# JiaweiXu8/AD-GS

Measured on AMD Instinct MI355X. Metric: fwd+bwd frames/s, higher is better.
Workload: dtype f32; 1 GPU; C3: 1000000 Gaussians, 1920x1280, SH deg 3, 8 dynamic objects, flow+semantic outputs, 1 camera/GPU/step; P=1000000, camera_pool=16 cameras / time stamps per GPU, cycled one per step (train.py:55-61), settle_steps=75, capacity_reruns=0, launch=eager, parallelism=single GPU, gradient_exchange=none, camera_streams=1

## Files before the change

### ad-gs_amd/csrc/api.hip

```cpp
#include "common.h"
#include "kernels.h"
#include "../../include/adgs_rasterizer.h"
#include "../../include/adgs_optim.h"

#include <atomic>
#include <chrono>
#include <mutex>
#include <vector>
#include <cstdlib>
#include <algorithm>
#include <cmath>
#include <cstring>

namespace adgs {

static thread_local std::string g_last_error;
struct FrameContext {
	adgs_frame_stats stats;
	size_t hint_cells, hint_fine;
	unsigned hint_max_cell_chunks;
	bool bucket_frame_pending;
	long long reruns;
	int last_order_hint;
	uint32_t* slab_bounds;
// ... 106 lines not shown
		s.tile_scanned = c.take<uint32_t>(ntiles);
		s.tile_batches = c.take<uint32_t>(ntiles);
		if (bytes) *bytes = c.size();
		return s;
	}
};
struct BinStateV2 {
	uint32_t* pool_cursor; uint32_t* pool;
	uint64_t* keys_unsorted; uint64_t* keys; uint32_t* list_unsorted; uint32_t* list; char* sort_temp;
	uint32_t* rec_key; uint2* rec_im; uint2* entries; uint32_t* slow_list;
	static size_t slab_grid(size_t R_cells, size_t ncells) { return std::max<size_t>(2 * R_cells / SLAB_TARGET_FOREIGN + ncells + 1, ncells << forced_lg()); }
	static int forced_lg() { const char* v = getenv("ADGS_SLABS_LG"); return (v && *v) ? std::min(std::max(atoi(v), 0), (int)MAX_SLAB_LG) : 0; }
	static size_t pool_chunks(size_t R_fine, size_t ntiles) { return R_fine / WAVE + (2 * (size_t)POOL_BLOCK + 1) * ntiles + 1; }
	static BinStateV2 carve_buckets(char* chunk, size_t R_cells, size_t R_fine, size_t ntiles, size_t* bytes, size_t ncells = 0) {
		Carver c(chunk); BinStateV2 b;
		b.pool_cursor = c.take<uint32_t>(64);
		b.pool = c.take<uint32_t>(pool_chunks(R_fine, ntiles) * CHUNK_WORDS);
		b.entries = c.take<uint2>(R_cells + 1);
		b.rec_im = c.take<uint2>(R_cells);
		b.rec_key = c.take<uint32_t>(R_cells);
		b.slow_list = c.take<uint32_t>(1 + slab_grid(R_cells, ncells));
		b.keys = nullptr; b.keys_unsorted = nullptr; b.sort_temp = nullptr; b.list = nullptr; b.list_unsorted = nullptr;
		if (bytes) *bytes = c.size();
		return b;
	}
	static BinStateV2 carve(char* chunk, size_t R_cells, size_t R_fine, size_t ntiles, size_t* bytes) {
		Carver c(chunk); BinStateV2 b;
		b.pool_cursor = c.take<uint32_t>(64);
		b.pool = c.take<uint32_t>(pool_chunks(R_fine, ntiles) * CHUNK_WORDS);
		b.list = c.take<uint32_t>(R_cells);
		b.list_unsorted = c.take<uint32_t>(R_cells);
		b.keys = c.take<uint64_t>(R_cells);
		b.keys_unsorted = c.take<uint64_t>(R_cells);
		b.sort_temp = c.take<char>(sort_temp_bytes(R_cells));
		b.rec_key = nullptr; b.rec_im = nullptr; b.entries = nullptr; b.slow_list = nullptr;
		if (bytes) *bytes = c.size();
		return b;
	}
};

static std::atomic<unsigned long long> g_env_reads{0};
static const char* env_str(const char* name) { g_env_reads.fetch_add(1, std::memory_order_relaxed); return getenv(name); }
static int env_int(const char* name, int dflt) {
	const char* v = env_str(name);
	return (v && *v) ? atoi(v) : dflt;
}
static bool use_v2(int D_S, bool env = true) {
	if (!env) return D_S <= (int)MAX_SEMANTIC;
	const char* m = env_str("ADGS_RASTER_MODE");
	if (m && std::string(m) == "classic") return false;
	return D_S <= std::min(env_int("ADGS_V2_MAX_SEMANTIC", 32), (int)MAX_SEMANTIC);
}

static bool v2_keys_fit(int gx, int gy, int c) { return 2 * c + (int)higher_msb((uint32_t)(((gx + c - 1) / c) * ((gy + c - 1) / c))) <= 32; }
static int v2_cell_tiles(int gx, int gy, bool fit_keys, bool env = true) {
	const size_t ntiles16 = (size_t)gx * gy;
	const int small = std::min(8, std::max(3, (int)std::lround(std::sqrt((double)ntiles16 / 110.0))));
	const int dflt = ntiles16 >= 4096 ? 12 : small;
	int c = std::max(1, env ? env_int("ADGS_CELL_TILES", dflt) : dflt);
	while (fit_keys && c > 1 && !v2_keys_fit(gx, gy, c)) c--;
	return c;
}
static int v2_pixels_per_lane(size_t ntiles16, bool env = true) {
	const int e = env ? env_int("ADGS_V2_PPL", 0) : 0;
	if (e == 1 || e == 2 || e == 4) return e;
	return ntiles16 < 4096 ? 2 : 4;
}


static const char* const kStageNames[ST_COUNT] = { "preprocess_fwd", "scan", "duplicate_keys", "radix_sort", "tile_ranges",
	"render_fwd", "render_bwd", "preprocess_bwd", "deform_fwd", "deform_bwd", "grad_expand" };
struct ProfRec { int stage; hipEvent_t a, b; };
static std::atomic<unsigned> g_prof_mask{0};
static std::mutex g_prof_mu;
static std::vector<ProfRec> g_prof_recs;
static std::vector<hipEvent_t> g_prof_pool;
static hipEvent_t prof_event() {
	std::lock_guard<std::mutex> lk(g_prof_mu);
	if (!g_prof_pool.empty()) { hipEvent_t e = g_prof_pool.back(); g_prof_pool.pop_back(); return e; }
	hipEvent_t e = nullptr; (void)hipEventCreate(&e); return e;
}
StageTimer::StageTimer(int stage_, hipStream_t stream) : on((g_prof_mask.load(std::memory_order_relaxed) >> stage_) & 1u), stage(stage_), a(nullptr), b(nullptr), s(stream) {
	if (on) { a = prof_event(); b = prof_event(); (void)hipEventRecord(a, s); }
}
StageTimer::~StageTimer() {
	if (on) { (void)hipEventRecord(b, s); std::lock_guard<std::mutex> lk(g_prof_mu); g_prof_recs.push_back(ProfRec{ stage, a, b }); }
}

static uint32_t* pinned_word() {
	static thread_local uint32_t* p = nullptr;
	if (!p) { if (hipHostMalloc((void**)&p, 1024, hipHostMallocDefault) != hipSuccess) p = nullptr; }
	return p;
}

struct MailboxRef { Mailbox* host; Mailbox* dev; uint32_t next_seq; size_t cap_cells, cap_fine;
	long long repaired; };
static MailboxRef* mailbox() {
	constexpr int MAX_DEV = 64;
	static thread_local MailboxRef boxes[MAX_DEV] = {};
	int dev = 0;
	if (hipGetDevice(&dev) != hipSuccess || dev < 0 || dev >= MAX_DEV) return nullptr;
	MailboxRef& m = boxes[dev];
	if (!m.host) {
		void* h = nullptr; void* d = nullptr;
		if (hipHostMalloc(&h, 256, hipHostMallocMapped | hipHostMallocCoherent | hipHostMallocPortable) != hipSuccess) return nullptr;
		if (hipHostGetDevicePointer(&d, h, 0) != hipSuccess) { (void)hipHostFree(h); return nullptr; }
		memset(h, 0, 256);
		m.host = (Mailbox*)h; m.dev = (Mailbox*)d; m.next_seq = 1; m.cap_cells = m.cap_fine = 0;
	}
	return &m;
}
struct OrderHints {
	struct Entry { const void* view; const void* proj; int W, H; size_t tiles; hipStream_t stream; bool captured; uint32_t* buf; unsigned long long used; bool written; size_t extra; };
	std::vector<Entry> entries;
	unsigned long long clock = 0, lookups = 0, hits = 0;
	hipStream_t service = nullptr;
	static constexpr size_t MAX_ENTRIES = 1024;
	Entry* find(const void* view, const void* proj, int W, int H, size_t tiles, hipStream_t stream, bool captured) {
		for (Entry& e : entries)
			if (e.view == view && e.proj == proj && e.W == W && e.H == H && e.tiles == tiles && e.captured == captured && (captured || e.stream == stream)) { e.used = ++clock; return &e; }
		return nullptr;
	}
	bool reset_signature(uint32_t* buf, size_t tiles, size_t extra) {
		if (!service && hipStreamCreateWithFlags(&service, hipStreamNonBlocking) != hipSuccess) { service = nullptr; return false; }
		return hipMemsetAsync(buf + tiles, 0, 16 * sizeof(uint32_t), service) == hipSuccess &&
		       (extra == 0 || hipMemsetAsync(buf + tiles + 16, 0xff, extra * sizeof(uint32_t), service) == hipSuccess) && hipStreamSynchronize(service) == hipSuccess;
	}
	Entry* create(const void* view, const void* proj, int W, int H, size_t tiles, hipStream_t stream, bool captured, size_t extra) {
		Entry* e = nullptr;
		if (entries.size() >= MAX_ENTRIES) {
			if (captured) return nullptr;
			for (Entry& c : entries) if (!c.captured && (!e || c.used < e->used)) e = &c;
			if (!e) return nullptr;
			(void)hipStreamSynchronize(e->stream);
			if (e->tiles != tiles || e->extra != extra) { (void)hipFree(e->buf); e->buf = nullptr; e->tiles = 0; e->view = nullptr; if (hipMalloc((void**)&e->buf, (tiles + 16 + extra) * sizeof(uint32_t)) != hipSuccess) { e->buf = nullptr; return nullptr; } }
		} else {
			Entry fresh{ nullptr, nullptr, 0, 0, 0, nullptr, false, nullptr, 0, false, 0 };
			if (hipMalloc((void**)&fresh.buf, (tiles + 16 + extra) * sizeof(uint32_t)) != hipSuccess) return nullptr;
			entries.push_back(fresh);
			e = &entries.back();
		}
		e->view = view; e->proj = proj; e->W = W; e->H = H; e->tiles = tiles; e->stream = stream; e->captured = captured; e->used = ++clock; e->written = false; e->extra = extra;
		if (!reset_signature(e->buf, tiles, extra)) { e->view = nullptr; e->tiles = 0; (void)hipFree(e->buf); e->buf = nullptr; return nullptr; }
		return e;
	}
};
static OrderHints* order_hints() {
	constexpr int MAX_DEV = 64;
	static thread_local OrderHints hints[MAX_DEV];
	int dev = 0;
	if (hipGetDevice(&dev) != hipSuccess || dev < 0 || dev >= MAX_DEV) return nullptr;
	return &hints[dev];
}
struct FrameCfg { int v2; int cell_tiles; int ppl; int tile_order = 1; int sh_staging = 1; int timeline = 0; int order_ready = 0; int backwards = 0; int antialiasing = 0; int published = 0; };
static uint32_t frame_cfg_word(const FrameCfg& c) {
	return 0xAD600000u | ((uint32_t)(c.v2 & 1) << 19) | ((uint32_t)(c.tile_order & 1) << 18) | ((uint32_t)(c.sh_staging & 1) << 17) | ((uint32_t)(c.timeline & 1) << 16) |
	       ((uint32_t)(c.order_ready & 1) << 15) | ((uint32_t)(c.antialiasing & 1) << 14) | ((uint32_t)(c.published & 1) << 13) |
	       ((uint32_t)(c.ppl & 0x1f) << 8) | (uint32_t)(c.cell_tiles & 0xff);
}
static bool frame_cfg_from_word(uint32_t w, FrameCfg* c) {
	if ((w & 0xFFF00000u) != 0xAD600000u) return false;
	*c = FrameCfg{ (int)((w >> 19) & 1u), (int)(w & 0xffu), (int)((w >> 8) & 0x1fu) };
	c->tile_order = (int)((w >> 18) & 1u); c->sh_staging = (int)((w >> 17) & 1u); c->timeline = (int)((w >> 16) & 1u); c->order_ready = (int)((w >> 15) & 1u);
	c->antialiasing = (int)((w >> 14) & 1u); c->published = (int)((w >> 13) & 1u);
	return c->cell_tiles >= 1 && (c->ppl == 1 || c->ppl == 2 || c->ppl == 4);
}
struct FrameKey {
	const void* img; const void* geom; int W, H, P;
	bool operator==(const FrameKey& o) const { return img == o.img && geom == o.geom && W == o.W && H == o.H && P == o.P; }
};
static std::mutex g_cfg_mu;
static std::vector<std::pair<FrameKey, FrameCfg>> g_cfg_table;
static void remember_frame(const FrameKey& k, const FrameCfg& c) {
	std::lock_guard<std::mutex> lk(g_cfg_mu);
	for (auto it = g_cfg_table.begin(); it != g_cfg_table.end();) it = (it->first.img == k.img || it->first.geom == k.geom) ? g_cfg_table.erase(it) : it + 1;
	if (g_cfg_table.size() >= 256) g_cfg_table.erase(g_cfg_table.begin());
	g_cfg_table.emplace_back(k, c);
}
static int note_backward(const FrameKey& k) {
	std::lock_guard<std::mutex> lk(g_cfg_mu);
	for (auto it = g_cfg_table.rbegin(); it != g_cfg_table.rend(); ++it) if (it->first == k) return it->second.backwards++;
	return -1;
}
static bool lookup_frame(const FrameKey& k, FrameCfg* c) {
	std::lock_guard<std::mutex> lk(g_cfg_mu);
	for (auto it = g_cfg_table.rbegin(); it != g_cfg_table.rend(); ++it) if (it->first == k) { *c = it->second; return true; }
	return false;
}
static bool lookup_frame_by_image(const void* img, int W, int H, FrameCfg* c) {
	std::lock_guard<std::mutex> lk(g_cfg_mu);
	for (auto it = g_cfg_table.rbegin(); it != g_cfg_table.rend(); ++it)
		if (it->first.img == img && it->first.W == W && it->first.H == H) { *c = it->second; return true; }
	return false;
}
__global__ void publish_counts_kernel(const uint32_t* __restrict__ total_cells, const unsigned long long* __restrict__ fine_slots, Mailbox* box, uint32_t seq,
	uint32_t cap_cells, unsigned long long cap_fine, uint32_t* __restrict__ overflow_flag) {
	unsigned long long f = threadIdx.x < SCAN_AUX_SLOTS ? fine_slots[threadIdx.x] : 0ull;
#pragma unroll
	for (int off = WAVE / 2; off > 0; off >>= 1) f += __shfl_xor(f, off, WAVE);
	if (threadIdx.x == 0) {
		const uint32_t total = *total_cells;
		const uint32_t over = (total > cap_cells || f > cap_fine) ? 1u : 0u;
		*overflow_flag = over;
		box->r_cells = total; box->r_fine = f; box->oversize = 0u; box->n_groups = 0u; box->overflow = over; box->max_cell_chunks = 0u;
		if (over) box->overflow_count = box->overflow_count + 1u;
		box->cap_cells = cap_cells; box->cap_fine = cap_fine;
		__threadfence_system();
		box->seq = seq;
	}
}
static int wait_mailbox(const MailboxRef* m, uint32_t seq, hipStream_t stream) {
	const auto t0 = std::chrono::steady_clock::now();
	for (unsigned spin = 0;; spin++) {
		if (m->host->seq == seq) return 0;
		if ((spin & 0xFFFF) == 0xFFFF && std::chrono::steady_clock::now() - t0 > std::chrono::seconds(10)) break;
	}
	ADGS_HIP_CHECK(hipStreamSynchronize(stream));
	if (m->host->seq == seq) return 0;
	set_error("the device never published the binning counts"); return -1;
}

}

using namespace adgs;

extern "C" const char* adgs_last_error(void) { return g_last_error.c_str(); }

extern "C" void adgs_get_frame_stats(adgs_frame_stats* out) { if (out) *out = frame_context()->stats; }

extern "C" int adgs_get_frame_status(adgs_frame_status* out) {
	if (!out) return -1;
	memset(out, 0, sizeof(*out));
	MailboxRef* mb = mailbox();
	if (!mb) { set_error("hipHostMalloc (mapped) failed"); return -1; }
	out->pairs = (int64_t)mb->host->r_cells; out->fine_pairs = (int64_t)mb->host->r_fine;
	out->capacity_pairs = mb->host->cap_cells == 0xffffffffu ? (int64_t)mb->host->r_cells : (int64_t)mb->host->cap_cells;
	out->capacity_fine_pairs = mb->host->cap_fine == ~0ull ? (int64_t)mb->host->r_fine : (int64_t)mb->host->cap_fine;
	out->overflow = (int32_t)mb->host->overflow; out->overflow_count = (int64_t)mb->host->overflow_count;
	out->eager_reruns = (int64_t)frame_context()->reruns;
	out->order_hint = frame_context()->last_order_hint;
	out->fullest_slab_units = (int64_t)mb->host->max_cell_chunks;
	if (OrderHints* oh = order_hints()) { out->order_hint_lookups = (int64_t)oh->lookups; out->order_hint_hits = (int64_t)oh->hits; }
	out->unrepaired_overflow_count = (int64_t)mb->host->overflow_count - (int64_t)mb->repaired;
	return 0;
}

extern "C" int adgs_raster_needs_zero_init(int D_S) { return use_v2(D_S) ? 0 : 1; }
extern "C" int adgs_raster_backward_needs_zero_init(const char* geom_buffer, const char* img_buffer, int width, int height, int P) {
	FrameCfg cfg;
	if (!lookup_frame(FrameKey{ img_buffer, geom_buffer, width, height, P }, &cfg)) return 1;
	return cfg.v2 ? 0 : 1;
}

extern "C" void adgs_profile_enable(int stage_mask) { g_prof_mask.store((unsigned)stage_mask); }
extern "C" int adgs_profile_reserve(int n_events) {
	std::vector<hipEvent_t> fresh;
	for (int i = 0; i < n_events; i++) { hipEvent_t e = nullptr; if (hipEventCreate(&e) != hipSuccess) break; fresh.push_back(e); }
	std::lock_guard<std::mutex> lk(g_prof_mu);
	g_prof_pool.insert(g_prof_pool.end(), fresh.begin(), fresh.end());
	return (int)fresh.size();
}
extern "C" int adgs_profile_num_stages(void) { return ST_COUNT; }
extern "C" const char* adgs_profile_stage_name(int i) { return (i >= 0 && i < ST_COUNT) ? kStageNames[i] : ""; }
extern "C" int adgs_profile_collect(double* total_ms, int64_t* counts) {
	std::lock_guard<std::mutex> lk(g_prof_mu);
	for (auto& r : g_prof_recs) {
		float ms = 0.f;
		if (hipEventElapsedTime(&ms, r.a, r.b) == hipSuccess) { total_ms[r.stage] += ms; counts[r.stage] += 1; }
		g_prof_pool.push_back(r.a); g_prof_pool.push_back(r.b);
	}
	g_prof_recs.clear();
	return 0;
}

extern "C" int adgs_device_check(void) {
	int n = 0;
	if (hipGetDeviceCount(&n) != hipSuccess || n == 0) { set_error("no HIP device"); return -1; }
	hipDeviceProp_t prop;
	int dev = 0;
	ADGS_HIP_CHECK(hipGetDevice(&dev));
	ADGS_HIP_CHECK(hipGetDeviceProperties(&prop, dev));
	if (std::string(prop.gcnArchName).find("gfx950") == std::string::npos) {
		set_error(std::string("device is ") + prop.gcnArchName + ", this library is built for gfx950 only");
		return -2;
	}
	return 0;
}

static int raster_forward_impl(const ShSource* sh_src, bool training, int antialiasing,
	adgs_alloc_fn geometryBuffer, void* geometryUser,
	adgs_alloc_fn binningBuffer, void* binningUser,
	adgs_alloc_fn imageBuffer, void* imageUser,
	int P, int D, int M, int D_S,
	const float* background, int width, int height,
	const float* means3D, const float* shs, const float* colors_precomp, const float* flow_points, const float* semantic,
	const float* opacities, const float* scales, float scale_modifier, const float* rotations, const float* cov3D_precomp,
	const float* viewmatrix, const float* projmatrix, const float* cam_pos, float tan_fovx, float tan_fovy, int prefiltered,
	float* out_color, float* out_depth, float* img_opacity, float* img_flow, float* img_semantic,
	int inv_depth, int* radii, int debug, void* stream_) {
	(void)prefiltered;
	hipStream_t stream = (hipStream_t)stream_;
	FrameContext* fc = frame_context();
	if (P <= 0) return 0;
	if (D_S > MAX_SEMANTIC) { set_error("D_S exceeds 32 semantic channels"); return -1; }
	if (!means3D || !opacities || (!cov3D_precomp && (!scales || !rotations)) || !radii) { set_error("missing required input pointer"); return -1; }
	const int gx = (width + TILE_X - 1) / TILE_X, gy = (height + TILE_Y - 1) / TILE_Y;
	const size_t ntiles = (size_t)gx * gy, npix = (size_t)width * height;
	if (gx > 65535 || gy > 65535) { set_error("image too large"); return -1; }
	if (ntiles * 4 * (2 * (size_t)POOL_BLOCK + 1) > 0xffffffffull) { set_error("image too large: chunk slots are 32-bit"); return -1; }

	if (D_S > 1) training = true;
	if (use_v2(D_S)) {
		int cell_tiles = v2_cell_tiles(gx, gy, false);
		int cgx = (gx + cell_tiles - 1) / cell_tiles, cgy = (gy + cell_tiles - 1) / cell_tiles;
		size_t ncells = (size_t)cgx * cgy;
		const char* binning_env = env_str("ADGS_BINNING");
		const std::string binning_mode = binning_env ? binning_env : "";
		{
			const MailboxRef* mbp = mailbox();
			const unsigned old_m = fc->hint_max_cell_chunks;
			const unsigned seen = (mbp && fc->bucket_frame_pending) ? mbp->host->max_cell_chunks : 0u;
			fc->hint_max_cell_chunks = std::max(seen, old_m - std::max(1u, old_m / 16) * (old_m ? 1u : 0u));
			fc->bucket_frame_pending = false;
		}
		bool buckets = ncells <= (size_t)MAX_CELLS && cell_tiles <= 16 && binning_mode != "sort" &&
			(binning_mode == "bucket" || (fc->hint_cells <= (size_t)std::max(1, env_int("ADGS_BUCKET_MAX_CHUNKS", 4)) * GS_NMAX * (ncells << MAX_SLAB_LG) &&
			                              fc->hint_max_cell_chunks <= (unsigned)std::max(1, env_int("ADGS_BUCKET_MAX_CELL_CHUNKS", 16))));
		if (!buckets && !v2_keys_fit(gx, gy, cell_tiles)) {
			cell_tiles = v2_cell_tiles(gx, gy, true);
			cgx = (gx + cell_tiles - 1) / cell_tiles; cgy = (gy + cell_tiles - 1) / cell_tiles; ncells = (size_t)cgx * cgy;
		}
		const bool sort_fallback_fits = v2_keys_fit(gx, gy, cell_tiles);
		size_t gb = 0, ib = 0;
		const size_t count_cells = buckets ? ncells : 0;
		const bool with_ddir = training && sh_src && M == 16;
		GeomStateV2::carve(nullptr, P, &gb, with_ddir, count_cells);
		char* gch = geometryBuffer(geometryUser, gb);
		const int ppl = v2_pixels_per_lane(ntiles), sub = TILE_Y / (4 * ppl);
		const int wgy = (height + 4 * ppl - 1) / (4 * ppl);
		const size_t wtiles = (size_t)gx * wgy;
		ImgStateV2::carve(nullptr, npix, wtiles, ncells, &ib);
		char* ich = imageBuffer(imageUser, ib);
		if (!gch || !ich) { set_error("buffer allocator returned NULL"); return -1; }
		GeomStateV2 geom = GeomStateV2::carve(gch, P, nullptr, with_ddir, count_cells);
		ImgStateV2 img = ImgStateV2::carve(ich, npix, wtiles, ncells, nullptr);
		uint32_t frame_word = 0; bool order_tiles = false;
		{
			FrameCfg fcfg{ 1, cell_tiles, ppl };
			fcfg.antialiasing = antialiasing ? 1 : 0;
			fcfg.tile_order = env_int("ADGS_TILE_ORDER", 1) != 0; fcfg.sh_staging = env_str("ADGS_NO_SH_STAGING") == nullptr; fcfg.timeline = env_int("ADGS_TIMELINE_BWD", 0) != 0;
			order_tiles = wtiles >= 2048 && fcfg.tile_order;
			if (!training) order_tiles = false;
			fcfg.order_ready = order_tiles ? 1 : 0;
			fcfg.published = (training && env_int("ADGS_PUBLISHED_MASK", 1) != 0) ? 1 : 0;
			if (training) remember_frame(FrameKey{ ich, gch, width, height, P }, fcfg);
			frame_word = frame_cfg_word(fcfg);
		}
		const int fwd_order_mode = env_int("ADGS_FWD_ORDER", 2);
		OrderHints::Entry* hint = nullptr;
		const uint32_t* hint_read = nullptr;
		const bool fwd_hint_wanted = wtiles >= 2048 && env_int("ADGS_TILE_ORDER", 1) != 0 && fwd_order_mode == 2;
		if (fwd_hint_wanted) {
			hipStreamCaptureStatus cs0 = hipStreamCaptureStatusNone;
			(void)hipStreamIsCapturing(stream, &cs0);
			if (OrderHints* oh = order_hints()) {
				const bool cap0 = cs0 == hipStreamCaptureStatusActive;
				hint = oh->find(viewmatrix, projmatrix, width, height, wtiles, stream, cap0);
				if (!hint && training) {
					hipStreamCaptureMode mode = hipStreamCaptureModeRelaxed;
					if (cap0) (void)hipThreadExchangeStreamCaptureMode(&mode);
					hint = oh->create(viewmatrix, projmatrix, width, height, wtiles, stream, cap0, std::min<size_t>(ncells, (size_t)MAX_CELLS) * SLAB_ROW);
					if (cap0) (void)hipThreadExchangeStreamCaptureMode(&mode);
					(void)hipGetLastError();
				}
				oh->lookups++;
				if (hint && hint->buf) { hint_read = hint->buf; if (hint->written) oh->hits++; fc->last_order_hint = hint->written ? 1 : 0; } else { hint = nullptr; fc->last_order_hint = 0; }
			}
		}

		PreprocessArgs pa;
		pa.P = P; pa.D = D; pa.M = M; pa.D_S = D_S;
		pa.means3D = means3D; pa.scales = scales; pa.scale_modifier = scale_modifier; pa.rotations = rotations;
		pa.opacities = opacities; pa.shs = shs; pa.cov3D_precomp = cov3D_precomp; pa.colors_precomp = colors_precomp;
		pa.flow_points = flow_points; pa.semantic = semantic;
		pa.view = viewmatrix; pa.proj = projmatrix; pa.campos = cam_pos;
		pa.W = width; pa.H = height; pa.gx = gx; pa.gy = gy;
		pa.tan_fovx = tan_fovx; pa.tan_fovy = tan_fovy;
		pa.focal_y = height / (2.0f * tan_fovy); pa.focal_x = width / (2.0f * tan_fovx);
		pa.inv_depth = inv_depth;
		pa.radii = radii; pa.splats = geom.splats; pa.cov3D = nullptr; pa.clamped = geom.clamped; pa.tiles_touched = geom.cells_touched;
		pa.v2 = 1; pa.dupinfo = geom.dupinfo; pa.fine_touched = geom.fine_touched; pa.cell_tiles = cell_tiles; pa.cgx = cgx; pa.cgy = cgy;
		memset(&pa.sh_src, 0, sizeof(pa.sh_src));
		pa.sh0 = geom.sh0; pa.gacc = training ? geom.gacc : nullptr; pa.fine_total = geom.fine_total;
		pa.bucket_count = nullptr;
		pa.cfg_word = img.header; pa.cfg_value = frame_word;
		pa.ddir = geom.ddir;
		pa.published = training ? geom.published : nullptr;
		pa.antialias = antialiasing ? 1 : 0;
		FramePrologue pro{ nullptr, 0, nullptr, nullptr, 0 };
		bool own_bounds = false, sample_bounds = false;
		if (buckets) {
			if (!fc->slab_bounds) {
				hipStreamCaptureStatus csb = hipStreamCaptureStatusNone;
				(void)hipStreamIsCapturing(stream, &csb);
				hipStreamCaptureMode mode = hipStreamCaptureModeRelaxed;
				if (csb == hipStreamCaptureStatusActive) (void)hipThreadExchangeStreamCaptureMode(&mode);
				bool ok = hipMalloc((void**)&fc->slab_bounds, (size_t)MAX_CELLS * SLAB_ROW * sizeof(uint32_t)) == hipSuccess;
				ok = ok && (fc->service || hipStreamCreateWithFlags(&fc->service, hipStreamNonBlocking) == hipSuccess);
				ok = ok && hipMemsetAsync(fc->slab_bounds, 0xff, (size_t)MAX_CELLS * SLAB_ROW * sizeof(uint32_t), fc->service) == hipSuccess && hipStreamSynchronize(fc->service) == hipSuccess;
				if (csb == hipStreamCaptureStatusActive) (void)hipThreadExchangeStreamCaptureMode(&mode);
				if (!ok) { if (fc->slab_bounds) (void)hipFree(fc->slab_bounds); fc->slab_bounds = nullptr; (void)hipGetLastError(); }
			}
			pro.zero = reinterpret_cast<uint32_t*>(geom.bucket_fine_total()); pro.n_zero = 2 * SCAN_AUX_SLOTS + 8;
			if (fc->slab_bounds) {
				const bool own = training && hint && (hint->written || hint->captured) && hint->extra >= ncells * SLAB_ROW;
				own_bounds = own;
				sample_bounds = !own && fwd_hint_wanted && env_int("ADGS_SLAB_SAMPLE", 1) != 0;
				pro.copy_dst = geom.bounds; pro.copy_src = own ? hint->buf + wtiles + 16 : fc->slab_bounds; pro.n_copy = (int)(ncells * SLAB_ROW);
			}
			if (!sh_src && launch_bin_prepare(pro, stream) != 0) return -1;
			pa.bucket_count = geom.counts; pa.fine_total = geom.bucket_fine_total();
		}
		if (sh_src) { pa.sh_src = *sh_src; StageTimer t(ST_PREPROCESS, stream); if (launch_sh0(P, *sh_src, geom.sh0, stream, buckets ? &pro : nullptr) != 0) return -1; }
		if (const int evict_mb = env_int("ADGS_DBG_EVICT_MB", 0)) {
			static thread_local void* scratch = nullptr; static thread_local size_t scratch_bytes = 0;
			const size_t want = (size_t)evict_mb << 20;
			if (scratch_bytes < want) { if (scratch) (void)hipFree(scratch); scratch = nullptr; scratch_bytes = 0; if (hipMalloc(&scratch, want) == hipSuccess) scratch_bytes = want; }
			if (scratch) ADGS_HIP_CHECK(hipMemsetAsync(scratch, 0, want, stream));
		}
		{ StageTimer t(ST_PREPROCESS, stream); if (launch_preprocess_fwd(pa, stream) != 0) return -1; }
		ADGS_LAUNCH_CHECK(debug, stream);
		MailboxRef* mb = mailbox();
		if (!mb) { set_error("hipHostMalloc (mapped) failed"); return -1; }
		const uint32_t seq = mb->next_seq++;
		hipStreamCaptureStatus cap_status = hipStreamCaptureStatusNone;
		(void)hipStreamIsCapturing(stream, &cap_status);
		const bool capturing = cap_status == hipStreamCaptureStatusActive;
		const bool speculate = capturing || env_int("ADGS_NO_SPECULATION", 0) == 0;
		const size_t cap_cells = std::min<size_t>(std::max<size_t>(fc->hint_cells, (size_t)P + 4096), 0x7fffffffu);
		const size_t cap_fine = std::max<size_t>(fc->hint_fine, (size_t)8 * P + 4096);
		mb->cap_cells = cap_cells; mb->cap_fine = cap_fine;
		uint32_t* overflow_flag = geom.d_counts() + 3;
		CellScanArgs sa;
		sa.cell_count = geom.cell_count(); sa.cell_start = geom.cell_start; sa.cell_ranges = img.cell_ranges; sa.ncells = (int)ncells;
		sa.max_chunks = (uint32_t)std::min(MAX_CHUNKS, std::max(1, env_int("ADGS_MAX_CHUNKS", MAX_CHUNKS))); sa.d_counts = geom.d_counts();
		sa.fine_total = geom.bucket_fine_total(); sa.cell_work = geom.cell_work; sa.force_lg = buckets ? env_int("ADGS_SLABS_LG", -1) : -1;
		sa.slab_target = own_bounds ? (uint32_t)SLAB_TARGET : (uint32_t)SLAB_TARGET_FOREIGN;
		sa.cap_cells = speculate ? (uint32_t)cap_cells : 0xffffffffu; sa.cap_fine = speculate ? (unsigned long long)cap_fine : ~0ull;
		sa.box = mb->dev; sa.seq = seq;
		if (buckets) {
			StageTimer t(ST_SCAN, stream);
			if (launch_cell_colscan(geom.counts, (P + 255) / 256, (int)ncells, geom.cell_count(), stream) != 0) return -1;
			if (launch_cell_scan(sa, stream) != 0) return -1;
		} else {
			{
				StageTimer t(ST_SCAN, stream);
				if (exclusive_scan_u32_sum(geom.cells_touched, geom.offsets, (size_t)P + 1, geom.scan_temp, geom.fine_touched, geom.fine_total, stream) != 0) return -1;
			}
			hipLaunchKernelGGL(publish_counts_kernel, dim3(1), dim3(WAVE), 0, stream, (const uint32_t*)(geom.offsets + P), (const unsigned long long*)geom.fine_total, mb->dev, seq,
				speculate ? (uint32_t)cap_cells : 0xffffffffu, speculate ? (unsigned long long)cap_fine : ~0ull, overflow_flag);
			ADGS_HIP_CHECK(hipGetLastError());
		}
		ADGS_LAUNCH_CHECK(debug, stream);
		const int bit = (int)higher_msb((uint32_t)ncells);
		BinStateV2 bin;
		const int mask_shift = 32 + bit;
		auto enqueue_binning = [&](size_t cells, size_t fine, const uint32_t* d_count) -> int {
			size_t bb = 0;
			if (buckets) {
				BinStateV2::carve_buckets(nullptr, cells, training ? fine * sub : 0, training ? wtiles : 0, &bb, ncells);
				char* bch = binningBuffer(binningUser, bb);
				if (!bch) { set_error("binning allocator returned NULL"); return -1; }
				bin = BinStateV2::carve_buckets(bch, cells, training ? fine * sub : 0, training ? wtiles : 0, nullptr, ncells);
				if (cells == 0) { ADGS_HIP_CHECK(hipMemsetAsync(bin.pool_cursor, 0, sizeof(uint32_t), stream)); return 0; }
				const uint32_t cap = (uint32_t)std::min<size_t>(cells, 0xffffffffu);
				{ StageTimer t(ST_DUPLICATE, stream);
				  if (launch_cell_scatter(P, geom.dupinfo, geom.cell_start, geom.counts, bin.rec_key, bin.rec_im, cap, cell_tiles, cgx, (int)ncells, bin.pool_cursor, bin.slow_list, stream) != 0) return -1; }
				ADGS_LAUNCH_CHECK(debug, stream);
				SlabSortArgs ga;
				ga.cell_ranges = img.cell_ranges; ga.ncells = (int)ncells; ga.cell_work = geom.cell_work; ga.grid = (uint32_t)BinStateV2::slab_grid(cells, ncells); ga.rec_key = bin.rec_key; ga.rec_im = bin.rec_im; ga.ent_f = bin.entries; ga.cap = cap;
				ga.bounds = geom.bounds; ga.bounds_out = fc->slab_bounds; ga.d_counts = geom.d_counts(); ga.slow_list = bin.slow_list;
				ga.bounds_out2 = (training && hint && hint->extra >= ncells * SLAB_ROW) ? hint->buf + wtiles + 16 : nullptr;
				ga.box = mb->dev;
				{ StageTimer t(ST_SORT, stream);
				  if (sample_bounds && launch_cell_sample(ga, geom.bounds, stream) != 0) return -1;
				  if (launch_slab_sort(ga, stream) != 0) return -1; }
				ADGS_LAUNCH_CHECK(debug, stream);
				return 0;
			}
			BinStateV2::carve(nullptr, cells, training ? fine * sub : 0, training ? wtiles : 0, &bb);
			char* bch = binningBuffer(binningUser, bb);
			if (!bch) { set_error("binning allocator returned NULL"); return -1; }
			bin = BinStateV2::carve(bch, cells, training ? fine * sub : 0, training ? wtiles : 0, nullptr);
			if (cells == 0) {
				ADGS_HIP_CHECK(hipMemsetAsync(img.cell_ranges, 0, ncells * sizeof(uint2), stream));
				ADGS_HIP_CHECK(hipMemsetAsync(bin.pool_cursor, 0, sizeof(uint32_t), stream));
				return 0;
			}
			{ StageTimer t(ST_DUPLICATE, stream);
			  if (launch_duplicate_cells(P, geom.dupinfo, geom.offsets, bin.keys_unsorted, bin.list_unsorted, (uint32_t)std::min<size_t>(cells, 0xffffffffu),
			        cell_tiles, cgx, img.cell_ranges, (int)ncells, bin.pool_cursor, mask_shift, stream) != 0) return -1; }
			ADGS_LAUNCH_CHECK(debug, stream);
			{ StageTimer t(ST_SORT, stream);
			  if (radix_sort_pairs_u64_dn(bin.keys_unsorted, bin.keys, bin.list_unsorted, bin.list, cells, d_count, 32 + bit, bin.sort_temp, stream) != 0) return -1; }
			ADGS_LAUNCH_CHECK(debug, stream);
			{ StageTimer t(ST_RANGES, stream);
			  if (launch_tile_ranges((int)cells, d_count, bin.keys, img.cell_ranges, bit >= 32 ? 0xffffffffu : ((1u << bit) - 1u), stream) != 0) return -1;
// ... 73 lines not shown
		fc->stats.num_rendered = (int64_t)R_cells; fc->stats.tiles = (int32_t)ntiles; fc->stats.sort_bits = buckets ? 32 : 32 + bit;
		fc->stats.sort_passes = buckets ? 4 : (32 + bit + 7) / 8;
		fc->stats.reserved = buckets ? 1 : 0; fc->stats.fine_pairs = (int64_t)R_fine;
		return (int)R_cells;
	}

	size_t gbytes = 0, ibytes = 0;
	GeomState::carve(nullptr, P, &gbytes);
	char* gchunk = geometryBuffer(geometryUser, gbytes);
	ImgState::carve(nullptr, npix, ntiles, &ibytes);
	char* ichunk = imageBuffer(imageUser, ibytes);
	if (!gchunk || !ichunk) { set_error("buffer allocator returned NULL"); return -1; }
	GeomState geom = GeomState::carve(gchunk, P, nullptr);
	ImgState img = ImgState::carve(ichunk, npix, ntiles, nullptr);
	uint32_t frame_word = 0;
	{
		FrameCfg fcfg{ 0, 1, 4 };
		fcfg.antialiasing = antialiasing ? 1 : 0;
		fcfg.sh_staging = env_str("ADGS_NO_SH_STAGING") == nullptr;
		remember_frame(FrameKey{ ichunk, gchunk, width, height, P }, fcfg);
		frame_word = frame_cfg_word(fcfg);
	}

	PreprocessArgs pa;
	pa.P = P; pa.D = D; pa.M = M; pa.D_S = D_S;
	pa.means3D = means3D; pa.scales = scales; pa.scale_modifier = scale_modifier; pa.rotations = rotations;
	pa.opacities = opacities; pa.shs = shs; pa.cov3D_precomp = cov3D_precomp; pa.colors_precomp = colors_precomp;
	pa.flow_points = flow_points; pa.semantic = semantic;
	pa.view = viewmatrix; pa.proj = projmatrix; pa.campos = cam_pos;
	pa.W = width; pa.H = height; pa.gx = gx; pa.gy = gy;
	pa.tan_fovx = tan_fovx; pa.tan_fovy = tan_fovy;
	pa.focal_y = height / (2.0f * tan_fovy);
	pa.focal_x = width / (2.0f * tan_fovx);
	pa.inv_depth = inv_depth;
	pa.radii = radii; pa.splats = geom.splats; pa.cov3D = geom.cov3D; pa.clamped = geom.clamped; pa.tiles_touched = geom.tiles_touched;
	pa.v2 = 0; pa.dupinfo = nullptr; pa.fine_touched = nullptr; pa.cell_tiles = 1; pa.cgx = gx; pa.cgy = gy;
	memset(&pa.sh_src, 0, sizeof(pa.sh_src)); pa.sh0 = nullptr; pa.gacc = nullptr; pa.fine_total = nullptr;
	pa.bucket_count = nullptr;
	pa.cfg_word = img.header; pa.cfg_value = frame_word; pa.ddir = nullptr; pa.published = nullptr;
	pa.antialias = antialiasing ? 1 : 0;
	if (sh_src) { set_error("the raw-SH entry points need the default (v2) pipeline (not ADGS_RASTER_MODE=classic, D_S <= ADGS_V2_MAX_SEMANTIC)"); return -1; }
	{ StageTimer t(ST_PREPROCESS, stream); if (launch_preprocess_fwd(pa, stream) != 0) return -1; }
	ADGS_LAUNCH_CHECK(debug, stream);

	{
		StageTimer t(ST_SCAN, stream);
		if (exclusive_scan_u32(geom.tiles_touched, geom.offsets, (size_t)P + 1, geom.scan_temp, stream) != 0) return -1;
	}
	ADGS_LAUNCH_CHECK(debug, stream);

	uint32_t* host_word = pinned_word();
	if (!host_word) { set_error("hipHostMalloc failed"); return -1; }
	ADGS_HIP_CHECK(hipMemcpyAsync(host_word, geom.offsets + P, sizeof(uint32_t), hipMemcpyDeviceToHost, stream));
	ADGS_HIP_CHECK(hipStreamSynchronize(stream));
	const int num_rendered = (int)*host_word;

	size_t bbytes = 0;
	BinState::carve(nullptr, (size_t)num_rendered, &bbytes);
	char* bchunk = binningBuffer(binningUser, bbytes);
	if (!bchunk) { set_error("binning allocator returned NULL"); return -1; }
	BinState bin = BinState::carve(bchunk, (size_t)num_rendered, nullptr);

	{ StageTimer t(ST_DUPLICATE, stream);
	  if (launch_duplicate_keys(P, geom.splats, geom.offsets, radii, bin.keys_unsorted, bin.list_unsorted, gx, gy, stream) != 0) return -1; }
	ADGS_LAUNCH_CHECK(debug, stream);
	const int bit = (int)higher_msb((uint32_t)ntiles);
	{ StageTimer t(ST_SORT, stream);
	  if (radix_sort_pairs_u64(bin.keys_unsorted, bin.keys, bin.list_unsorted, bin.list, (size_t)num_rendered, 32 + bit, bin.sort_temp, stream) != 0) return -1; }
	ADGS_LAUNCH_CHECK(debug, stream);
	{ StageTimer t(ST_RANGES, stream);
	  ADGS_HIP_CHECK(hipMemsetAsync(img.ranges, 0, ntiles * sizeof(uint2), stream));
	  if (launch_tile_ranges(num_rendered, nullptr, bin.keys, img.ranges, 0xffffffffu, stream) != 0) return -1; }
	ADGS_LAUNCH_CHECK(debug, stream);

	RenderFwdArgs ra;
	ra.ranges = img.ranges; ra.point_list = bin.list; ra.splats = geom.splats;
	ra.W = width; ra.H = height; ra.gx = gx; ra.gy = gy; ra.D_S = D_S;
	ra.has_color = (colors_precomp != nullptr) || (shs != nullptr);
	ra.has_flow = flow_points != nullptr; ra.has_sem = (semantic != nullptr) && D_S > 0; ra.inv_depth = inv_depth != 0;
	ra.semantic = semantic; ra.bg = background;
	ra.final_T = img_opacity; ra.n_contrib = img.n_contrib;
	ra.out_color = out_color; ra.out_depth = out_depth; ra.out_flow = img_flow; ra.out_semantic = img_semantic;
	{ StageTimer t(ST_RENDER_FWD, stream); if (launch_render_fwd(ra, stream) != 0) return -1; }
	ADGS_LAUNCH_CHECK(debug, stream);

	fc->stats.num_rendered = num_rendered; fc->stats.tiles = (int32_t)ntiles; fc->stats.sort_bits = 32 + bit; fc->stats.sort_passes = (32 + bit + 7) / 8;
	fc->stats.fine_pairs = num_rendered;
	return num_rendered;
}

static int raster_backward_impl(const ShSource* sh_src, const ShGradDst* sh_dst,
	int P, int D, int M, int R, int D_S,
	const float* background, int width, int height,
	const float* means3D, const float* shs, const float* colors_precomp, const float* flow_points, const float* semantic,
	const float* scales, float scale_modifier, const float* rotations, const float* cov3D_precomp,
	const float* viewmatrix, const float* projmatrix, const float* campos, float tan_fovx, float tan_fovy,
	const int* radii, char* geom_buffer, char* binning_buffer, char* img_buffer,
	const float* dL_dpix, const float* dL_dpix_depth, const float* dL_dpix_flow, const float* dL_dpix_semantic,
	float* dL_dmean2D, float* dL_dconic, float* dL_dopacity, float* dL_dcolor, float* dL_ddepth, float* dL_dmean3D,
	float* dL_dcov3D, float* dL_dsh, float* dL_dscale, float* dL_drot, float* dL_dflow, float* dL_dsemantic,
	const float* grad_img_opacity, const float* img_opacity, int inv_depth, int debug, void* stream_, float* dL_dmean2D_abs = nullptr) {
	hipStream_t stream = (hipStream_t)stream_;
	if (P <= 0) return 0;
	if (!geom_buffer || !img_buffer || (R > 0 && !binning_buffer)) { set_error("backward called without forward state buffers"); return -1; }
	if (dL_dmean2D_abs && dL_dpix_semantic && semantic && D_S > 1) {
		set_error("backward: dL_dmean2D_abs cannot be computed with D_S > 1 semantic channels and a semantic gradient (the extra channels are separate replays: "
		          "their per-pass absolute sums are not the absolute of the pair's term)");
		return -1;
	}
	const int gx = (width + TILE_X - 1) / TILE_X, gy = (height + TILE_Y - 1) / TILE_Y;
	const size_t ntiles = (size_t)gx * gy, npix = (size_t)width * height;
	FrameCfg cfg;
	const FrameKey fkey{ img_buffer, geom_buffer, width, height, P };
	if (!lookup_frame(fkey, &cfg)) {
		hipStreamCaptureStatus cs = hipStreamCaptureStatusNone;
		(void)hipStreamIsCapturing(stream, &cs);
		if (cs == hipStreamCaptureStatusActive) { set_error("backward over state buffers the captured forward did not allocate: their configuration cannot be read back inside a stream capture"); return -1; }
		uint32_t word = 0;
		ADGS_HIP_CHECK(hipMemcpyAsync(&word, img_buffer, sizeof(word), hipMemcpyDeviceToHost, stream));
		ADGS_HIP_CHECK(hipStreamSynchronize(stream));
		if (!frame_cfg_from_word(word, &cfg)) { set_error("backward: the image state buffer does not carry a forward's configuration word (not written by adgs_raster_forward?)"); return -1; }
	}
	if (dL_dmean2D_abs && !cfg.v2) {
		set_error("backward: dL_dmean2D_abs needs a forward of the default (v2) pipeline; this frame's forward ran the classic pipeline "
		          "(ADGS_RASTER_MODE=classic, or D_S above ADGS_V2_MAX_SEMANTIC), which does not form the absolute sums");
		return -1;
	}
	if (cfg.v2) {
		const int cell_tiles = cfg.cell_tiles;
		const size_t ncells = (size_t)((gx + cell_tiles - 1) / cell_tiles) * ((gy + cell_tiles - 1) / cell_tiles);
		GeomStateV2 geom = GeomStateV2::carve(geom_buffer, P, nullptr, sh_src && M == 16);
		const int ppl = cfg.ppl;
		const int wgy = (height + 4 * ppl - 1) / (4 * ppl);
		const size_t wtiles = (size_t)gx * wgy;
		ImgStateV2 img = ImgStateV2::carve(img_buffer, npix, wtiles, ncells, nullptr);
		BinStateV2 bin = BinStateV2::carve(binning_buffer, 0, 0, wtiles, nullptr);
		const bool has_color = (colors_precomp != nullptr) || (shs != nullptr) || (sh_src != nullptr);
		RenderV2BwdArgs ra;
		ra.splats = geom.splats; ra.pool = bin.pool; ra.tile_last_chunk = img.tile_last_chunk; ra.tile_consumed = img.tile_consumed;
		ra.W = width; ra.H = height; ra.gx = gx; ra.gy = wgy; ra.ppl = ppl;
		ra.bg = background; ra.final_T = img_opacity; ra.n_contrib = img.n_contrib;
		ra.bg_image = sh_src ? sh_src->bg_image : nullptr; ra.dL_dbg_image = (sh_src && sh_dst && ra.bg_image && dL_dpix) ? sh_dst->bg_image : nullptr;
		ra.dL_dpix = dL_dpix; ra.dL_dpix_depth = dL_dpix_depth; ra.dL_dpix_flow = dL_dpix_flow; ra.dL_dpix_sem = dL_dpix_semantic;
		ra.dL_dpix_opacity = grad_img_opacity;
		ra.do_color = dL_dpix && has_color;
		ra.do_flow = dL_dpix_flow && flow_points;
		ra.do_sem = dL_dpix_semantic && semantic && D_S > 0;
		ra.do_depth = dL_dpix_depth != nullptr;
		ra.do_opacity = grad_img_opacity != nullptr || (ra.bg_image != nullptr && ra.do_color);
		ra.absgrad = dL_dmean2D_abs != nullptr;
		ra.gacc = geom.gacc;
		ra.tile_order = nullptr;
		ra.tl_start = cfg.timeline ? img.tile_scanned : nullptr; ra.tl_end = img.tile_batches;
		{
			StageTimer t(ST_RENDER_BWD, stream);
			if (wtiles >= 2048 && cfg.tile_order) {
				if (!cfg.order_ready && launch_tile_order((int)wtiles, img.tile_consumed, img.tile_order, stream) != 0) return -1;
				ra.tile_order = img.tile_order;
			}
			if (note_backward(fkey) != 0) ADGS_HIP_CHECK(hipMemsetAsync(geom.gacc, 0, (size_t)P * GACC_STRIDE * sizeof(float), stream));
			ra.sem_src = nullptr; ra.sem_dst = nullptr; ra.sem_stride = 0;
			if (binning_buffer && launch_render_bwd_v2(ra, stream) != 0) return -1;
			if (binning_buffer && ra.do_sem && D_S > 1) {
				ADGS_HIP_CHECK(hipMemsetAsync(dL_dsemantic, 0, (size_t)P * D_S * sizeof(float), stream));
				RenderV2BwdArgs rc = ra;
				rc.do_color = rc.do_flow = rc.do_depth = rc.do_opacity = false; rc.do_sem = true; rc.absgrad = false;
				rc.dL_dpix = nullptr; rc.dL_dpix_depth = nullptr; rc.dL_dpix_flow = nullptr; rc.dL_dpix_opacity = nullptr;
				rc.bg_image = nullptr; rc.dL_dbg_image = nullptr; rc.sem_stride = D_S;
				for (int c = 1; c < D_S; c++) {
					rc.dL_dpix_sem = dL_dpix_semantic + (size_t)c * npix; rc.sem_src = semantic + c; rc.sem_dst = dL_dsemantic + c;
					if (launch_render_bwd_v2(rc, stream) != 0) return -1;
				}
			}
		}
		ADGS_LAUNCH_CHECK(debug, stream);
		PreprocessBwdArgs pa;
		pa.P = P; pa.D = D; pa.M = M;
		pa.means3D = means3D; pa.radii = radii; pa.shs = shs; pa.clamped = geom.clamped;
		pa.scales = scales; pa.rotations = rotations; pa.scale_modifier = scale_modifier;
		pa.cov3D = cov3D_precomp;
		pa.view = viewmatrix; pa.proj = projmatrix; pa.campos = campos;
		pa.focal_y = height / (2.0f * tan_fovy); pa.focal_x = width / (2.0f * tan_fovx);
		pa.tan_fovx = tan_fovx; pa.tan_fovy = tan_fovy; pa.inv_depth = inv_depth;
		pa.dL_dmean2D = nullptr; pa.dL_dconic = nullptr; pa.dL_dcolor = nullptr; pa.dL_ddepth = nullptr;
		pa.dL_dmean3D = dL_dmean3D; pa.dL_dcov3D = dL_dcov3D; pa.dL_dsh = dL_dsh; pa.dL_dscale = dL_dscale; pa.dL_drot = dL_drot;
		pa.gacc = geom.gacc; pa.splats = geom.splats; pa.W = width; pa.H = height;
		memset(&pa.sh_src, 0, sizeof(pa.sh_src)); pa.sh_dst = ShGradDst{};
		if (sh_src) { pa.sh_src = *sh_src; if (sh_dst) pa.sh_dst = *sh_dst; }
		pa.out_mean2D = dL_dmean2D; pa.out_conic = dL_dconic; pa.out_opacity = dL_dopacity; pa.out_color = dL_dcolor; pa.out_depth = dL_ddepth;
		pa.out_flow = ra.do_flow ? dL_dflow : nullptr; pa.out_sem = ra.do_sem ? dL_dsemantic : nullptr; pa.D_S = D_S;
		pa.out_mean2D_abs = dL_dmean2D_abs;
		pa.sh_staging = cfg.sh_staging;
		pa.ddir = geom.ddir;
		pa.antialias = cfg.antialiasing;
		pa.published = cfg.published ? geom.published : nullptr;
		{ StageTimer t(ST_PREPROCESS_BWD, stream); if (launch_preprocess_bwd(pa, stream) != 0) return -1; }
		ADGS_LAUNCH_CHECK(debug, stream);
		return 0;
	}
	GeomState geom = GeomState::carve(geom_buffer, P, nullptr);
	ImgState img = ImgState::carve(img_buffer, npix, ntiles, nullptr);
	BinState bin = BinState::carve(binning_buffer, (size_t)R, nullptr);

	const bool has_color = (colors_precomp != nullptr) || (shs != nullptr);
	RenderBwdArgs ra;
	ra.ranges = img.ranges; ra.point_list = bin.list; ra.splats = geom.splats;
	ra.W = width; ra.H = height; ra.gx = gx; ra.gy = gy; ra.D_S = D_S;
	ra.semantic = semantic; ra.bg = background;
	ra.final_T = img_opacity; ra.n_contrib = img.n_contrib;
	ra.dL_dpix = dL_dpix; ra.dL_dpix_depth = dL_dpix_depth; ra.dL_dpix_flow = dL_dpix_flow; ra.dL_dpix_sem = dL_dpix_semantic;
	ra.dL_dpix_opacity = grad_img_opacity;
	ra.do_color = dL_dpix && has_color;
	ra.do_flow = dL_dpix_flow && flow_points;
	ra.do_sem = dL_dpix_semantic && semantic && D_S > 0;
	ra.do_depth = dL_dpix_depth != nullptr;
	ra.do_opacity = grad_img_opacity != nullptr;
	ra.dL_dmean2D = dL_dmean2D; ra.dL_dconic = dL_dconic; ra.dL_dopacity = dL_dopacity; ra.dL_dcolor = dL_dcolor;
	ra.dL_ddepth = dL_ddepth; ra.dL_dflow = dL_dflow; ra.dL_dsem = dL_dsemantic;
	if (R > 0) {
		{ StageTimer t(ST_RENDER_BWD, stream); if (launch_render_bwd(ra, stream) != 0) return -1; }
		ADGS_LAUNCH_CHECK(debug, stream);
	}

	PreprocessBwdArgs pa;
	pa.P = P; pa.D = D; pa.M = M;
	pa.means3D = means3D; pa.radii = radii; pa.shs = shs; pa.clamped = geom.clamped;
	pa.scales = scales; pa.rotations = rotations; pa.scale_modifier = scale_modifier;
	pa.cov3D = cov3D_precomp ? cov3D_precomp : geom.cov3D;
	pa.view = viewmatrix; pa.proj = projmatrix; pa.campos = campos;
	pa.focal_y = height / (2.0f * tan_fovy); pa.focal_x = width / (2.0f * tan_fovx);
	pa.tan_fovx = tan_fovx; pa.tan_fovy = tan_fovy; pa.inv_depth = inv_depth;
	pa.dL_dmean2D = dL_dmean2D; pa.dL_dconic = dL_dconic; pa.dL_dcolor = dL_dcolor; pa.dL_ddepth = dL_ddepth;
	pa.dL_dmean3D = dL_dmean3D; pa.dL_dcov3D = dL_dcov3D; pa.dL_dsh = dL_dsh; pa.dL_dscale = dL_dscale; pa.dL_drot = dL_drot;
	if (sh_src) { set_error("the raw-SH entry points need the default (v2) pipeline (not ADGS_RASTER_MODE=classic, D_S <= ADGS_V2_MAX_SEMANTIC)"); return -1; }
	memset(&pa.sh_src, 0, sizeof(pa.sh_src)); pa.sh_dst = ShGradDst{};
	pa.gacc = nullptr; pa.splats = nullptr; pa.W = width; pa.H = height; pa.out_mean2D = nullptr; pa.out_conic = nullptr; pa.out_opacity = nullptr; pa.out_color = nullptr; pa.out_depth = nullptr;
	pa.out_flow = nullptr; pa.out_sem = nullptr; pa.D_S = D_S; pa.out_mean2D_abs = nullptr;
	pa.sh_staging = cfg.sh_staging; pa.ddir = nullptr; pa.published = nullptr;
	pa.antialias = cfg.antialiasing;
	if (cfg.antialiasing) { pa.out_opacity = dL_dopacity; pa.splats = geom.splats; }
	{ StageTimer t(ST_PREPROCESS_BWD, stream); if (launch_preprocess_bwd(pa, stream) != 0) return -1; }
	ADGS_LAUNCH_CHECK(debug, stream);
	return 0;
}

static int read_raster_options(const adgs_raster_options* o, const char* who, int* antialiasing) {
	*antialiasing = 0;
	if (!o) return 0;
	if (o->struct_bytes < offsetof(adgs_raster_options, antialiasing) + sizeof(int32_t) || o->struct_bytes > 4096) {
		set_error(std::string(who) + ": adgs_raster_options.struct_bytes must be sizeof(adgs_raster_options) of the caller's header"); return -1;
	}
	adgs_raster_options full;
	memset(&full, 0, sizeof(full));
	memcpy(&full, o, std::min<size_t>((size_t)o->struct_bytes, sizeof(full)));
	if (full.antialiasing != 0 && full.antialiasing != 1) { set_error(std::string(who) + ": adgs_raster_options.antialiasing must be 0 or 1"); return -1; }
	*antialiasing = full.antialiasing;
	return 0;
}

extern "C" int adgs_raster_forward_opts(
	adgs_alloc_fn geometryBuffer, void* geometryUser, adgs_alloc_fn binningBuffer, void* binningUser, adgs_alloc_fn imageBuffer, void* imageUser,
	int P, int D, int M, int D_S, const float* background, int width, int height,
	const float* means3D, const float* shs, const float* colors_precomp, const float* flow_points, const float* semantic,
	const float* opacities, const float* scales, float scale_modifier, const float* rotations, const float* cov3D_precomp,
	const float* viewmatrix, const float* projmatrix, const float* cam_pos, float tan_fovx, float tan_fovy, int prefiltered,
	float* out_color, float* out_depth, float* img_opacity, float* img_flow, float* img_semantic,
	int inv_depth, int* radii, int debug, void* stream, const adgs_raster_options* options) {
	int aa = 0;
	if (read_raster_options(options, "adgs_raster_forward_opts", &aa) != 0) return -1;
	return raster_forward_impl(nullptr, true, aa, geometryBuffer, geometryUser, binningBuffer, binningUser, imageBuffer, imageUser, P, D, M, D_S, background,
		width, height, means3D, shs, colors_precomp, flow_points, semantic, opacities, scales, scale_modifier, rotations, cov3D_precomp,
		viewmatrix, projmatrix, cam_pos, tan_fovx, tan_fovy, prefiltered, out_color, out_depth, img_opacity, img_flow, img_semantic,
		inv_depth, radii, debug, stream);
}

extern "C" int adgs_raster_forward(
	adgs_alloc_fn geometryBuffer, void* geometryUser, adgs_alloc_fn binningBuffer, void* binningUser, adgs_alloc_fn imageBuffer, void* imageUser,
	int P, int D, int M, int D_S, const float* background, int width, int height,
	const float* means3D, const float* shs, const float* colors_precomp, const float* flow_points, const float* semantic,
	const float* opacities, const float* scales, float scale_modifier, const float* rotations, const float* cov3D_precomp,
	const float* viewmatrix, const float* projmatrix, const float* cam_pos, float tan_fovx, float tan_fovy, int prefiltered,
	float* out_color, float* out_depth, float* img_opacity, float* img_flow, float* img_semantic,
	int inv_depth, int* radii, int debug, void* stream) {
	return adgs_raster_forward_opts(geometryBuffer, geometryUser, binningBuffer, binningUser, imageBuffer, imageUser, P, D, M, D_S, background, width, height, means3D, shs, colors_precomp, flow_points, semantic, opacities, scales, scale_modifier, rotations, cov3D_precomp, viewmatrix, projmatrix, cam_pos, tan_fovx, tan_fovy, prefiltered, out_color, out_depth, img_opacity, img_flow, img_semantic, inv_depth, radii, debug, stream, nullptr);
}

extern "C" int adgs_raster_render_opts(
	adgs_alloc_fn geometryBuffer, void* geometryUser, adgs_alloc_fn binningBuffer, void* binningUser, adgs_alloc_fn imageBuffer, void* imageUser,
	int P, int D, int M, int D_S, const float* background, int width, int height,
	const float* means3D, const float* shs, const float* colors_precomp, const float* flow_points, const float* semantic,
	const float* opacities, const float* scales, float scale_modifier, const float* rotations, const float* cov3D_precomp,
	const float* viewmatrix, const float* projmatrix, const float* cam_pos, float tan_fovx, float tan_fovy, int prefiltered,
	float* out_color, float* out_depth, float* img_opacity, float* img_flow, float* img_semantic,
	int inv_depth, int* radii, int debug, void* stream, const adgs_raster_options* options) {
	int aa = 0;
	if (read_raster_options(options, "adgs_raster_render_opts", &aa) != 0) return -1;
	return raster_forward_impl(nullptr, false, aa, geometryBuffer, geometryUser, binningBuffer, binningUser, imageBuffer, imageUser, P, D, M, D_S, background,
		width, height, means3D, shs, colors_precomp, flow_points, semantic, opacities, scales, scale_modifier, rotations, cov3D_precomp,
		viewmatrix, projmatrix, cam_pos, tan_fovx, tan_fovy, prefiltered, out_color, out_depth, img_opacity, img_flow, img_semantic,
		inv_depth, radii, debug, stream);
}

extern "C" int adgs_raster_render(
	adgs_alloc_fn geometryBuffer, void* geometryUser, adgs_alloc_fn binningBuffer, void* binningUser, adgs_alloc_fn imageBuffer, void* imageUser,
	int P, int D, int M, int D_S, const float* background, int width, int height,
	const float* means3D, const float* shs, const float* colors_precomp, const float* flow_points, const float* semantic,
	const float* opacities, const float* scales, float scale_modifier, const float* rotations, const float* cov3D_precomp,
	const float* viewmatrix, const float* projmatrix, const float* cam_pos, float tan_fovx, float tan_fovy, int prefiltered,
	float* out_color, float* out_depth, float* img_opacity, float* img_flow, float* img_semantic,
	int inv_depth, int* radii, int debug, void* stream) {
	return adgs_raster_render_opts(geometryBuffer, geometryUser, binningBuffer, binningUser, imageBuffer, imageUser, P, D, M, D_S, background, width, height, means3D, shs, colors_precomp, flow_points, semantic, opacities, scales, scale_modifier, rotations, cov3D_precomp, viewmatrix, projmatrix, cam_pos, tan_fovx, tan_fovy, prefiltered, out_color, out_depth, img_opacity, img_flow, img_semantic, inv_depth, radii, debug, stream, nullptr);
}

static int read_backward_options(const adgs_raster_backward_options* o, const char* who, float** dL_dmean2D_abs) {
	*dL_dmean2D_abs = nullptr;
	if (!o) return 0;
	if (o->struct_bytes < offsetof(adgs_raster_backward_options, dL_dmean2D_abs) + sizeof(float*) || o->struct_bytes > 4096) {
		set_error(std::string(who) + ": adgs_raster_backward_options.struct_bytes must be sizeof(adgs_raster_backward_options) of the caller's header"); return -1;
	}
	adgs_raster_backward_options full;
	memset(&full, 0, sizeof(full));
	memcpy(&full, o, std::min<size_t>((size_t)o->struct_bytes, sizeof(full)));
	*dL_dmean2D_abs = full.dL_dmean2D_abs;
	return 0;
}

extern "C" int adgs_raster_backward_opts(
	int P, int D, int M, int R, int D_S, const float* background, int width, int height,
	const float* means3D, const float* shs, const float* colors_precomp, const float* flow_points, const float* semantic,
	const float* scales, float scale_modifier, const float* rotations, const float* cov3D_precomp,
	const float* viewmatrix, const float* projmatrix, const float* campos, float tan_fovx, float tan_fovy,
	const int* radii, char* geom_buffer, char* binning_buffer, char* img_buffer,
	const float* dL_dpix, const float* dL_dpix_depth, const float* dL_dpix_flow, const float* dL_dpix_semantic,
	float* dL_dmean2D, float* dL_dconic, float* dL_dopacity, float* dL_dcolor, float* dL_ddepth, float* dL_dmean3D,
	float* dL_dcov3D, float* dL_dsh, float* dL_dscale, float* dL_drot, float* dL_dflow, float* dL_dsemantic,
	const float* grad_img_opacity, const float* img_opacity, int inv_depth, int debug, void* stream, const adgs_raster_backward_options* options) {
	float* abs_dst = nullptr;
	if (read_backward_options(options, "adgs_raster_backward_opts", &abs_dst) != 0) return -1;
	return raster_backward_impl(nullptr, nullptr, P, D, M, R, D_S, background, width, height, means3D, shs, colors_precomp, flow_points, semantic,
		scales, scale_modifier, rotations, cov3D_precomp, viewmatrix, projmatrix, campos, tan_fovx, tan_fovy, radii, geom_buffer, binning_buffer,
		img_buffer, dL_dpix, dL_dpix_depth, dL_dpix_flow, dL_dpix_semantic, dL_dmean2D, dL_dconic, dL_dopacity, dL_dcolor, dL_ddepth, dL_dmean3D,
		dL_dcov3D, dL_dsh, dL_dscale, dL_drot, dL_dflow, dL_dsemantic, grad_img_opacity, img_opacity, inv_depth, debug, stream, abs_dst);
}

extern "C" int adgs_raster_backward(
	int P, int D, int M, int R, int D_S, const float* background, int width, int height,
	const float* means3D, const float* shs, const float* colors_precomp, const float* flow_points, const float* semantic,
	const float* scales, float scale_modifier, const float* rotations, const float* cov3D_precomp,
	const float* viewmatrix, const float* projmatrix, const float* campos, float tan_fovx, float tan_fovy,
	const int* radii, char* geom_buffer, char* binning_buffer, char* img_buffer,
	const float* dL_dpix, const float* dL_dpix_depth, const float* dL_dpix_flow, const float* dL_dpix_semantic,
	float* dL_dmean2D, float* dL_dconic, float* dL_dopacity, float* dL_dcolor, float* dL_ddepth, float* dL_dmean3D,
	float* dL_dcov3D, float* dL_dsh, float* dL_dscale, float* dL_drot, float* dL_dflow, float* dL_dsemantic,
	const float* grad_img_opacity, const float* img_opacity, int inv_depth, int debug, void* stream) {
	return adgs_raster_backward_opts(P, D, M, R, D_S, background, width, height, means3D, shs, colors_precomp, flow_points, semantic,
		scales, scale_modifier, rotations, cov3D_precomp, viewmatrix, projmatrix, campos, tan_fovx, tan_fovy, radii, geom_buffer, binning_buffer,
		img_buffer, dL_dpix, dL_dpix_depth, dL_dpix_flow, dL_dpix_semantic, dL_dmean2D, dL_dconic, dL_dopacity, dL_dcolor, dL_ddepth, dL_dmean3D,
		dL_dcov3D, dL_dsh, dL_dscale, dL_drot, dL_dflow, dL_dsemantic, grad_img_opacity, img_opacity, inv_depth, debug, stream, nullptr);
}

static ShSource to_sh_source(const adgs_sh_source* s) {
	ShSource r;
	r.Ns = s->Ns; r.scene_dc = s->scene_dc; r.obj_dc = s->obj_dc; r.scene_rest = s->scene_rest; r.obj_rest = s->obj_rest;
	r.scene_sp = s->scene_deform; r.obj_sp = s->obj_deform; r.f = s->f;
	const bool raw_geo = s->Ns > 0 && s->scene_xyz && s->scene_scaling && s->scene_rotation && s->scene_opacity;
	r.scene_xyz = raw_geo ? s->scene_xyz : nullptr; r.scene_scaling = raw_geo ? s->scene_scaling : nullptr;
	r.scene_rotation = raw_geo ? s->scene_rotation : nullptr; r.scene_opacity = raw_geo ? s->scene_opacity : nullptr;
	r.bg_image = s->bg_image;
	if (!r.scene_dc) { r.scene_dc = r.obj_dc; r.scene_rest = r.obj_rest; }
	if (!r.obj_dc) { r.obj_dc = r.scene_dc; r.obj_rest = r.scene_rest; }
	return r;
}
static int check_sh_source(const adgs_sh_source* sh, int P, int M, const char* who) {
	const bool need_scene = sh && sh->Ns > 0, need_obj = sh && sh->Ns < P;
	if (sh && (sh->scene_xyz || sh->scene_scaling || sh->scene_rotation || sh->scene_opacity) &&
	    !(sh->scene_xyz && sh->scene_scaling && sh->scene_rotation && sh->scene_opacity)) {
		set_error(std::string(who) + ": raw scene geometry needs all four tensors"); return -1;
	}
	if (!sh || sh->Ns < 0 || sh->Ns > P || (need_scene && (!sh->scene_dc || (M > 1 && !sh->scene_rest))) || (need_obj && (!sh->obj_dc || (M > 1 && !sh->obj_rest)))) {
		set_error(std::string(who) + ": incomplete SH source"); return -1;
	}
	return 0;
}

extern "C" int adgs_raster_forward_rawsh_opts(
	adgs_alloc_fn geometryBuffer, void* geometryUser, adgs_alloc_fn binningBuffer, void* binningUser, adgs_alloc_fn imageBuffer, void* imageUser,
	int P, int D, int M, int D_S, const float* background, int width, int height,
	const float* means3D, const adgs_sh_source* sh, const float* flow_points, const float* semantic,
	const float* opacities, const float* scales, float scale_modifier, const float* rotations,
	const float* viewmatrix, const float* projmatrix, const float* cam_pos, float tan_fovx, float tan_fovy,
	float* out_color, float* out_depth, float* img_opacity, float* img_flow, float* img_semantic,
// ... 279 lines not shown
```

### ad-gs_amd/csrc/deform_sh.hip

```cpp
#include "common.h"
#include "kernels.h"
#include <cstring>

namespace adgs {
namespace {

struct ShsFwdArgs {
	int Ns, N, M;
	const float *scene_dc, *obj_dc, *scene_rest, *obj_rest, *sp_scene, *sp_obj;
	adgs_func_eval fs;
	float* out;
};
__global__ void __launch_bounds__(256) deform_shs_fwd_kernel(ShsFwdArgs a) {
	const size_t i = (size_t)blockIdx.x * blockDim.x + threadIdx.x;
	const int row = a.M * 3;
	const size_t total = (size_t)a.N * row;
	const size_t e0 = i * 4;
	if (e0 >= total) return;
	float v[4];
#pragma unroll
	for (int k = 0; k < 4; k++) {
		const size_t e = e0 + k;
		if (e >= total) { v[k] = 0.f; continue; }
		const int n = (int)(e / row), c = (int)(e % row);
		const bool is_obj = n >= a.Ns;
		const int m = is_obj ? n - a.Ns : n;
		if (c < 3) {
			float x = (is_obj ? a.obj_dc : a.scene_dc)[3 * (size_t)m + c];
			const float* sp = is_obj ? a.sp_obj : a.sp_scene;
			if (sp && has_lin(a.fs)) x = x + lin_eval(sp + ((size_t)m * 3 + c) * a.fs.n_params, a.fs);
			v[k] = x;
		} else {
			v[k] = (is_obj ? a.obj_rest : a.scene_rest)[(size_t)m * (row - 3) + (c - 3)];
		}
	}
	if (e0 + 4 <= total && (row & 3) == 0) *reinterpret_cast<float4*>(a.out + e0) = make_float4(v[0], v[1], v[2], v[3]);
	else { for (int k = 0; k < 4; k++) if (e0 + k < total) a.out[e0 + k] = v[k]; }
}

__global__ void __launch_bounds__(256) shs_rest_interleave_kernel(int Ns, int N, const float* __restrict__ scene_rest, const float* __restrict__ obj_rest, float* __restrict__ out) {
	const size_t i = (size_t)blockIdx.x * blockDim.x + threadIdx.x;
	if (i >= (size_t)N * 12) return;
	const int n = (int)(i / 12), q = (int)(i - (size_t)n * 12);
	const bool is_obj = n >= Ns;
	const float* r = (is_obj ? obj_rest : scene_rest) + (size_t)(is_obj ? n - Ns : n) * 45;
	float* o = out + (size_t)n * 48 + 4 * q;
	if (q == 0) { o[3] = r[0]; return; }
	const float a = r[4 * q - 3], b = r[4 * q - 2], c = r[4 * q - 1], d = r[4 * q];
	*reinterpret_cast<float4*>(o) = make_float4(a, b, c, d);
}
__global__ void __launch_bounds__(256) shs_grad_split_kernel(int Ns, int N, const float* __restrict__ g, float* __restrict__ g_scene_dc, float* __restrict__ g_obj_dc,
	float* __restrict__ g_scene_rest, float* __restrict__ g_obj_rest) {
	const size_t i = (size_t)blockIdx.x * blockDim.x + threadIdx.x;
	if (i >= (size_t)N * 12) return;
	const int n = (int)(i / 12), q = (int)(i - (size_t)n * 12);
	const bool is_obj = n >= Ns;
	const size_t m = is_obj ? n - Ns : n;
	const float4 v = *reinterpret_cast<const float4*>(g + (size_t)n * 48 + 4 * q);
	float* rest = is_obj ? g_obj_rest : g_scene_rest;
	if (q == 0) {
		float* dc = is_obj ? g_obj_dc : g_scene_dc;
		if (dc) { dc[3 * m] = v.x; dc[3 * m + 1] = v.y; dc[3 * m + 2] = v.z; }
		if (rest) rest[m * 45] = v.w;
		return;
	}
	if (rest) { float* r = rest + m * 45 + 4 * q - 3; r[0] = v.x; r[1] = v.y; r[2] = v.z; r[3] = v.w; }
}

struct ShsBwdArgs {
	int Ns, N, M;
	const float* g;
	float *g_scene_dc, *g_obj_dc, *g_scene_rest, *g_obj_rest;
};
__global__ void __launch_bounds__(256) deform_shs_bwd_copy_kernel(ShsBwdArgs a) {
	const size_t e = (size_t)blockIdx.x * blockDim.x + threadIdx.x;
	const int row = a.M * 3;
	if (e >= (size_t)a.N * row) return;
	const int n = (int)(e / row), c = (int)(e % row);
	const bool is_obj = n >= a.Ns;
	const int m = is_obj ? n - a.Ns : n;
	const float v = a.g[e];
	if (c < 3) { float* d = is_obj ? a.g_obj_dc : a.g_scene_dc; if (d) d[3 * (size_t)m + c] = v; }
	else { float* d = is_obj ? a.g_obj_rest : a.g_scene_rest; if (d) d[(size_t)m * (row - 3) + (c - 3)] = v; }
}
struct ParamGradArgs {
	int count, D, gstride;
	const float* g;
	float* out;
	adgs_func_eval f;
	int nb0, count_b; const float* g_b; float* out_b;
	AdamSlot adam = { nullptr, nullptr, nullptr, 0.f, 0.f }, adam_b = { nullptr, nullptr, nullptr, 0.f, 0.f };
	float beta1 = 0.f, beta2 = 0.f, eps = 0.f;
};
constexpr int PG_ITEMS = 8;
template <bool ADAM>
__global__ void __launch_bounds__(256) deform_lin_param_grad_kernel(ParamGradArgs a) {
	extern __shared__ float s_w[];
	const int np = a.f.n_params;
	const bool second = a.nb0 > 0 && (int)blockIdx.x >= a.nb0;
	const int seg_count = second ? a.count_b : a.count;
	const float* __restrict__ seg_g = second ? a.g_b : a.g;
	float* __restrict__ seg_out = second ? a.out_b : a.out;
	const size_t tot = (size_t)seg_count * a.D * np;
	const size_t blk0 = (size_t)(blockIdx.x - (second ? a.nb0 : 0)) * 256 * PG_ITEMS;
	constexpr int HALVES = PG_ITEMS / 4;
	size_t e0[HALVES], m0[HALVES]; int k0[HALVES], d0[HALVES]; float gv0[HALVES];
#pragma unroll
	for (int half = 0; half < HALVES; half++) {
		e0[half] = blk0 + ((size_t)half * 256 + threadIdx.x) * 4;
		const size_t e = min(e0[half], tot - 1);
		size_t row;
		if (tot <= 0xffffffffull) { const uint32_t r32 = (uint32_t)e / (uint32_t)np; row = r32; k0[half] = (int)((uint32_t)e - r32 * (uint32_t)np); }
		else { row = e / np; k0[half] = (int)(e - row * np); }
		m0[half] = row / a.D; d0[half] = (int)(row - m0[half] * a.D);
		gv0[half] = seg_g[m0[half] * (size_t)a.gstride + d0[half]];
	}
	float* const ad_p = ADAM ? (second ? a.adam_b.p : a.adam.p) : nullptr;
	float* const ad_m = ADAM ? (second ? a.adam_b.m : a.adam.m) : nullptr;
	float* const ad_v = ADAM ? (second ? a.adam_b.v : a.adam.v) : nullptr;
	const float ad_step = ADAM ? (second ? a.adam_b.step_size : a.adam.step_size) : 0.f, ad_ibc2 = ADAM ? (second ? a.adam_b.inv_bc2_sqrt : a.adam.inv_bc2_sqrt) : 0.f;
	float4 p4[HALVES], m4[HALVES], v4[HALVES];
	if (ADAM && ad_p) {
		const size_t last4 = tot >= 4 ? (tot - 4) & ~(size_t)3 : 0;
#pragma unroll
		for (int half = 0; half < HALVES; half++) {
			const size_t e = tot >= 4 ? min(e0[half], last4) : 0;
			if (tot >= 4) { p4[half] = ld_stream4(reinterpret_cast<const float4*>(ad_p + e)); m4[half] = ld_stream4(reinterpret_cast<const float4*>(ad_m + e)); v4[half] = ld_stream4(reinterpret_cast<const float4*>(ad_v + e)); }
		}
	}
	for (int k = threadIdx.x; k < np; k += blockDim.x) s_w[k] = 0.f;
	__syncthreads();
	const int total = a.f.n_terms[0] + a.f.n_terms[1] + a.f.n_terms[2];
	for (int i = threadIdx.x; i < total; i += blockDim.x) s_w[a.f.index[i]] = a.f.weight[i];
	__syncthreads();
#pragma unroll
	for (int half = 0; half < HALVES; half++) {
		if (e0[half] >= tot) return;
		size_t m = m0[half]; int k = k0[half], d = d0[half];
		float gv = gv0[half];
		float v[4];
#pragma unroll
		for (int it = 0; it < 4; it++) {
			v[it] = __fmul_rn(s_w[k], gv);
			if (++k == np) {
				k = 0;
				if (++d == a.D) { d = 0; m++; }
				if (e0[half] + it + 1 < tot) gv = seg_g[m * (size_t)a.gstride + d];
			}
		}
		if (ADAM && ad_p) {
			if (e0[half] + 4 <= tot) {
				adam_update4(p4[half], m4[half], v4[half], make_float4(v[0], v[1], v[2], v[3]), a.beta1, a.beta2, a.eps, ad_step, ad_ibc2);
				st_stream4(reinterpret_cast<float4*>(ad_p + e0[half]), p4[half]); st_stream4(reinterpret_cast<float4*>(ad_m + e0[half]), m4[half]); st_stream4(reinterpret_cast<float4*>(ad_v + e0[half]), v4[half]);
			} else for (int it = 0; it < 4 && e0[half] + it < tot; it++) {
				const size_t e = e0[half] + it;
				float pp = ad_p[e], mm = ad_m[e], vv = ad_v[e];
				adam_update(pp, mm, vv, v[it], a.beta1, a.beta2, a.eps, ad_step, ad_ibc2);
				ad_p[e] = pp; ad_m[e] = mm; ad_v[e] = vv;
			}
			continue;
		}
		if (e0[half] + 4 <= tot) st_stream4(reinterpret_cast<float4*>(seg_out + e0[half]), make_float4(v[0], v[1], v[2], v[3]));
		else for (int it = 0; it < 4 && e0[half] + it < tot; it++) seg_out[e0[half] + it] = v[it];
	}
}

template <int NV4>
__global__ void __launch_bounds__(256) sh0_rows_kernel(int N, ShSource s, float* __restrict__ out, FramePrologue pro, int ostride) {
	__shared__ float s_w[NV4 * 4];
	run_frame_prologue(pro);
	__shared__ float s_part[256 * NV4 + 4];
	const int e0 = blockIdx.x * 256;
	const int rows = min(256, N * 3 - e0);
	const int split = 3 * s.Ns;
	const bool one_side = (e0 >= split) || (e0 + rows <= split);
	const bool ob = e0 >= split;
	const float* sp = ob ? s.obj_sp : s.scene_sp;
	const bool fast = rows > 0 && one_side && sp != nullptr;
	const size_t r0 = ob ? (size_t)e0 - split : (size_t)e0;
	float4 q[NV4];
	float dc = 0.f;
	if (fast) {
		const float4* src = reinterpret_cast<const float4*>(sp + r0 * (NV4 * 4));
		const int words = rows * NV4;
#pragma unroll
		for (int k = 0; k < NV4; k++) { const int wd = k * 256 + threadIdx.x; q[k] = ld_stream4(src + min(wd, words - 1)); }
		dc = (ob ? s.obj_dc : s.scene_dc)[r0 + min((int)threadIdx.x, rows - 1)];
	}
	for (int k = threadIdx.x; k < NV4 * 4; k += 256) s_w[k] = 0.f;
	__syncthreads();
	const int total = s.f.n_terms[0] + s.f.n_terms[1] + s.f.n_terms[2];
	for (int i = threadIdx.x; i < total; i += 256) s_w[s.f.index[i]] = s.f.weight[i];
	__syncthreads();
	if (rows <= 0) return;
	if (fast) {
#pragma unroll
		for (int k = 0; k < NV4; k++) {
			const int wd = k * 256 + threadIdx.x, part = wd % NV4;
			s_part[wd] = q[k].x * s_w[4 * part] + q[k].y * s_w[4 * part + 1] + q[k].z * s_w[4 * part + 2] + q[k].w * s_w[4 * part + 3];
		}
		__syncthreads();
		if ((int)threadIdx.x < rows) {
			float acc = 0.f;
#pragma unroll
			for (int k = 0; k < NV4; k++) acc += s_part[threadIdx.x * NV4 + k];
			const int e = e0 + threadIdx.x, n = e / 3;
			out[(size_t)n * ostride + (e - 3 * n)] = dc + acc;
		}
		return;
	}
	const int e = e0 + threadIdx.x;
	if (e >= N * 3) return;
	const int n = e / 3;
	const bool tob = n >= s.Ns;
	const size_t r = tob ? (size_t)e - 3 * (size_t)s.Ns : (size_t)e;
	float v = (tob ? s.obj_dc : s.scene_dc)[r];
	const float* tsp = tob ? s.obj_sp : s.scene_sp;
	if (tsp) {
		const float4* row = reinterpret_cast<const float4*>(tsp + r * (NV4 * 4));
		float4 q[NV4];
#pragma unroll
		for (int k = 0; k < NV4; k++) q[k] = row[k];
		float acc = 0.f;
#pragma unroll
		for (int k = 0; k < NV4; k++) acc += q[k].x * s_w[4 * k] + q[k].y * s_w[4 * k + 1] + q[k].z * s_w[4 * k + 2] + q[k].w * s_w[4 * k + 3];
		v = v + acc;
	}
	out[(size_t)n * ostride + (e - 3 * n)] = v;
}
__global__ void __launch_bounds__(256) sh0_kernel(int N, ShSource s, float* __restrict__ out, FramePrologue pro, int ostride) {
	extern __shared__ float s_rows[];
	run_frame_prologue(pro);
	const int tid = threadIdx.x, B = blockDim.x, base = blockIdx.x * B, count = min(B, N - base);
	const int np = s.f.n_params, L = 3 * np, stride = L | 1;
	const bool lin = (s.scene_sp || s.obj_sp) && has_lin(s.f);
	if (lin) {
		stage_rows<true>(s_rows, stride, L, base, count, s.Ns, s.scene_sp, s.obj_sp, tid, B);
		__syncthreads();
	}
	if (tid >= count) return;
	const int n = base + tid;
	const bool ob = n >= s.Ns;
	const size_t m = ob ? n - s.Ns : n;
	const float* dc = (ob ? s.obj_dc : s.scene_dc) + 3 * m;
	const bool has_row = lin && (ob ? s.obj_sp : s.scene_sp) != nullptr;
#pragma unroll
	for (int c = 0; c < 3; c++) {
		float v = dc[c];
		if (has_row) v = v + lin_eval(s_rows + tid * stride + c * np, s.f);
		out[(size_t)ostride * n + c] = v;
	}
}
}

int launch_sh0(int N, const ShSource& s, float* out, hipStream_t stream, const FramePrologue* prologue, int ostride) {
	if (N <= 0) return 0;
	const FramePrologue pro = prologue ? *prologue : FramePrologue{ nullptr, 0, nullptr, nullptr, 0 };
	const int np = s.f.n_params;
	const bool lin = (s.scene_sp || s.obj_sp) && (s.f.n_terms[0] + s.f.n_terms[1] + s.f.n_terms[2]) > 0 && np > 0;
	const bool aligned = ((reinterpret_cast<uintptr_t>(s.scene_sp) | reinterpret_cast<uintptr_t>(s.obj_sp)) & 15) == 0;
	if (lin && np % 4 == 0 && np <= 32 && aligned) {
		using RowsKernel = void (*)(int, ShSource, float*, FramePrologue, int);
		static const RowsKernel rows[8] = { sh0_rows_kernel<1>, sh0_rows_kernel<2>, sh0_rows_kernel<3>, sh0_rows_kernel<4>,
			sh0_rows_kernel<5>, sh0_rows_kernel<6>, sh0_rows_kernel<7>, sh0_rows_kernel<8> };
		hipLaunchKernelGGL(rows[np / 4 - 1], dim3((unsigned)(((size_t)N * 3 + 255) / 256)), dim3(256), 0, stream, N, s, out, pro, ostride);
		ADGS_HIP_CHECK(hipGetLastError());
		return 0;
	}
	size_t lds = 0;
	const int B = pick_block((3 * np) | 1, &lds);
	if (lds > MAX_STAGING_LDS) { set_error("launch_sh0: SH deformation rows too large for the LDS staging buffer (more than 207 parameters per channel)"); return -1; }
	if (lds > 48 * 1024) ADGS_HIP_CHECK(hipFuncSetAttribute(reinterpret_cast<const void*>(&sh0_kernel), hipFuncAttributeMaxDynamicSharedMemorySize, (int)lds));
	hipLaunchKernelGGL(sh0_kernel, dim3((unsigned)((N + B - 1) / B)), dim3(B), lds, stream, N, s, out, pro, ostride);
	ADGS_HIP_CHECK(hipGetLastError());
	return 0;
}
int launch_lin_param_grad2(int count_a, const float* g_a, float* out_a, int count_b, const float* g_b, float* out_b, int D, int gstride,
	const adgs_func_eval& f, hipStream_t stream, const AdamSlot* adam_a, const AdamSlot* adam_b, float beta1, float beta2, float eps) {
	if (f.n_params <= 0) return 0;
	const AdamSlot off = { nullptr, nullptr, nullptr, 0.f, 0.f };
	const AdamSlot sa = adam_a ? *adam_a : off, sb = adam_b ? *adam_b : off;
	const bool on_a = (out_a || sa.p) && count_a > 0, on_b = (out_b || sb.p) && count_b > 0;
	if (!on_a && !on_b) return 0;
	if ((on_a && !g_a) || (on_b && !g_b)) { set_error("launch_lin_param_grad2: NULL gradient buffer"); return -1; }
	if ((on_a && out_a && sa.p) || (on_b && out_b && sb.p)) { set_error("launch_lin_param_grad2: a side takes the gradient store OR the Adam step"); return -1; }
	ParamGradArgs pg;
	pg.D = D; pg.gstride = gstride; pg.f = f; pg.beta1 = beta1; pg.beta2 = beta2; pg.eps = eps;
	const size_t per_block = (size_t)256 * PG_ITEMS;
	const size_t nb_a = on_a ? ((size_t)count_a * D * f.n_params + per_block - 1) / per_block : 0, nb_b = on_b ? ((size_t)count_b * D * f.n_params + per_block - 1) / per_block : 0;
	const bool two = on_a && on_b;
	pg.count = on_a ? count_a : count_b; pg.g = on_a ? g_a : g_b; pg.out = on_a ? out_a : out_b; pg.adam = on_a ? sa : sb;
	pg.nb0 = two ? (int)nb_a : 0; pg.count_b = two ? count_b : 0; pg.g_b = two ? g_b : nullptr; pg.out_b = two ? out_b : nullptr; pg.adam_b = two ? sb : off;
	if (sa.p || sb.p) hipLaunchKernelGGL(deform_lin_param_grad_kernel<true>, dim3((unsigned)(nb_a + nb_b)), dim3(256), f.n_params * sizeof(float), stream, pg);
	else hipLaunchKernelGGL(deform_lin_param_grad_kernel<false>, dim3((unsigned)(nb_a + nb_b)), dim3(256), f.n_params * sizeof(float), stream, pg);
	ADGS_HIP_CHECK(hipGetLastError());
	return 0;
}
int launch_lin_param_grad(int count, int D, const float* g, int gstride, float* out, const adgs_func_eval& f, hipStream_t stream) {
	if (count <= 0 || f.n_params <= 0) return 0;
	if (!g || !out) { set_error("launch_lin_param_grad: NULL gradient buffer"); return -1; }
	return launch_lin_param_grad2(count, g, out, 0, nullptr, nullptr, D, gstride, f, stream, nullptr, nullptr, 0.f, 0.f, 0.f);
}

int launch_deform_shs_fwd(const adgs_deform_params& p, const adgs_func_eval& fs, float* shs_out, hipStream_t stream) {
	const int N = p.Ns + p.No;
	if (p.sh_coeffs == 16 && (reinterpret_cast<uintptr_t>(shs_out) & 15) == 0 && (p.scene_shs_dc || p.obj_shs_dc)) {
		ShSource src;
		memset(&src, 0, sizeof(src));
		src.Ns = p.Ns; src.scene_dc = p.scene_shs_dc ? p.scene_shs_dc : p.obj_shs_dc; src.obj_dc = p.obj_shs_dc ? p.obj_shs_dc : p.scene_shs_dc;
		src.scene_sp = p.shs_deform_param_scene; src.obj_sp = p.shs_deform_param_obj; src.f = fs;
		if (launch_sh0(N, src, shs_out, stream, nullptr, 48) != 0) return -1;
		hipLaunchKernelGGL(shs_rest_interleave_kernel, dim3((unsigned)(((size_t)N * 12 + 255) / 256)), dim3(256), 0, stream, p.Ns, N, p.scene_shs_rest, p.obj_shs_rest, shs_out);
	} else {
		const ShsFwdArgs sa = { p.Ns, N, p.sh_coeffs, p.scene_shs_dc, p.obj_shs_dc, p.scene_shs_rest, p.obj_shs_rest, p.shs_deform_param_scene, p.shs_deform_param_obj, fs, shs_out };
		const size_t quads = ((size_t)N * p.sh_coeffs * 3 + 3) / 4;
		hipLaunchKernelGGL(deform_shs_fwd_kernel, dim3((unsigned)((quads + 255) / 256)), dim3(256), 0, stream, sa);
	}
	ADGS_HIP_CHECK(hipGetLastError());
	return 0;
}
int launch_deform_shs_bwd(const adgs_deform_params& p, const adgs_func_eval& fs, const float* dL_dshs, const adgs_deform_grads& grads, hipStream_t stream) {
	const int N = p.Ns + p.No, M = p.sh_coeffs;
	const ShsBwdArgs sb = { p.Ns, N, M, dL_dshs, grads.scene_shs_dc, grads.obj_shs_dc, grads.scene_shs_rest, grads.obj_shs_rest };
	if (M == 16 && (reinterpret_cast<uintptr_t>(dL_dshs) & 15) == 0)
		hipLaunchKernelGGL(shs_grad_split_kernel, dim3((unsigned)(((size_t)N * 12 + 255) / 256)), dim3(256), 0, stream, sb.Ns, N, dL_dshs, sb.g_scene_dc, sb.g_obj_dc, sb.g_scene_rest, sb.g_obj_rest);
	else
		hipLaunchKernelGGL(deform_shs_bwd_copy_kernel, dim3((unsigned)(((size_t)N * M * 3 + 255) / 256)), dim3(256), 0, stream, sb);
	ADGS_HIP_CHECK(hipGetLastError());
	return launch_lin_param_grad2(p.Ns, dL_dshs, grads.shs_deform_param_scene, p.No, dL_dshs + (size_t)p.Ns * M * 3, grads.shs_deform_param_obj,
		3, M * 3, fs, stream);
}
}
```

### ad-gs_amd/csrc/kernels.h

```cpp
#pragma once
#include "common.h"
#include "func_eval.h"

namespace adgs {

struct PreprocessArgs {
	int P, D, M, D_S;
	const float* means3D; const float* scales; float scale_modifier; const float* rotations;
	const float* opacities; const float* shs; const float* cov3D_precomp; const float* colors_precomp;
	const float* flow_points; const float* semantic;
	const float* view; const float* proj; const float* campos;
	int W, H, gx, gy;
	float tan_fovx, tan_fovy, focal_x, focal_y;
	int inv_depth;
	int* radii; Splat* splats; float* cov3D; uint8_t* clamped; uint32_t* tiles_touched;
	int v2;
	uint32_t* fine_touched;
	uint4* dupinfo;
	int cell_tiles, cgx, cgy;
	ShSource sh_src;
	const float* sh0;
	float* gacc;
	unsigned long long* fine_total;
	uint32_t* bucket_count;
	uint32_t* cfg_word; uint32_t cfg_value;
	float* ddir;
	int antialias;
	uint8_t* published;
};

int launch_preprocess_fwd(const PreprocessArgs& a, hipStream_t stream);
int launch_mark_visible(int P, const float* means, const float* view, uint8_t* present, hipStream_t stream);
int launch_duplicate_keys(int P, const Splat* splats, const uint32_t* offsets, const int* radii, uint64_t* keys, uint32_t* vals,
	int gx, int gy, hipStream_t stream);
int launch_tile_ranges(int L, const uint32_t* d_L, const uint64_t* keys, uint2* ranges, uint32_t id_mask, hipStream_t stream);

struct RenderFwdArgs {
	const uint2* ranges; const uint32_t* point_list; const Splat* splats;
	int W, H, gx, gy, D_S;
	bool has_color, has_flow, has_sem, inv_depth;
	const float* semantic;
	const float* bg;
	float* final_T;
	uint32_t* n_contrib;
	float* out_color; float* out_depth; float* out_flow; float* out_semantic;
	int order_mode;
};
int launch_render_fwd(const RenderFwdArgs& a, hipStream_t stream);

struct RenderBwdArgs {
	const uint2* ranges; const uint32_t* point_list; const Splat* splats;
	int W, H, gx, gy, D_S;
	const float* semantic; const float* bg;
	const float* final_T; const uint32_t* n_contrib;
	const float* dL_dpix; const float* dL_dpix_depth; const float* dL_dpix_flow; const float* dL_dpix_sem; const float* dL_dpix_opacity;
	bool do_color, do_flow, do_sem, do_depth, do_opacity;
	float* dL_dmean2D;
	float* dL_dconic;
	float* dL_dopacity;
	float* dL_dcolor;
	float* dL_ddepth;
	float* dL_dflow;
	float* dL_dsem;
};
int launch_render_bwd(const RenderBwdArgs& a, hipStream_t stream);

struct PreprocessBwdArgs {
	int P, D, M;
	const float* means3D; const int* radii; const float* shs; const uint8_t* clamped;
	const float* scales; const float* rotations; float scale_modifier;
	const float* cov3D;
	const float* view; const float* proj; const float* campos;
	float focal_x, focal_y, tan_fovx, tan_fovy;
	int inv_depth;
	const float* dL_dmean2D; const float* dL_dconic; const float* dL_dcolor; const float* dL_ddepth;
	float* dL_dmean3D; float* dL_dcov3D; float* dL_dsh; float* dL_dscale; float* dL_drot;
	float* gacc; const Splat* splats; int W, H;
	ShSource sh_src; ShGradDst sh_dst;
	float* out_mean2D; float* out_conic; float* out_opacity; float* out_color; float* out_depth; float* out_flow; float* out_sem;
	float* out_mean2D_abs;
	int D_S;
	int sh_staging;
	const float* ddir;
	int antialias;
	const uint8_t* published;
};
int launch_preprocess_bwd(const PreprocessBwdArgs& a, hipStream_t stream);

constexpr int CHUNK_WORDS = 2 + WAVE;
constexpr int CHUNK_PREV = WAVE, CHUNK_COUNT = WAVE + 1;
constexpr int POOL_BLOCK = 4;
constexpr int GACC_STRIDE = 16;
constexpr int GACC_USED = 14;

constexpr int MAX_CELLS = 1024;
constexpr int SLAB_ROW = 128;
constexpr int MAX_SLAB_LG = 7;
constexpr int SLAB_TARGET = 3072;
constexpr int SLAB_TARGET_FOREIGN = 2048;
constexpr int GS_NMAX = 4096;
constexpr int MAX_CHUNKS = 16384;
constexpr size_t count_row_stride(int nblocks) { return ((size_t)nblocks + 3u) & ~(size_t)3u; }
struct Mailbox { volatile uint32_t seq; uint32_t r_cells; unsigned long long r_fine; uint32_t oversize, n_groups, overflow, overflow_count, max_cell_chunks;
	uint32_t cap_cells; unsigned long long cap_fine; };
int launch_bin_prepare(const FramePrologue& p, hipStream_t stream);
struct CellScanArgs {
	const uint32_t* cell_count;
	uint32_t* cell_start;
	uint2* cell_ranges; int ncells;
	uint32_t max_chunks;
	uint2* cell_work;
	int force_lg;
	uint32_t slab_target;
	uint32_t* d_counts;
	const unsigned long long* fine_total;
	uint32_t cap_cells; unsigned long long cap_fine;
	Mailbox* box; uint32_t seq;
};
int launch_cell_scan(const CellScanArgs& a, hipStream_t stream);
int launch_cell_colscan(uint32_t* counts , int nblocks, int ncells, uint32_t* cell_count, hipStream_t stream);
int launch_cell_scatter(int P, const uint4* dupinfo, const uint32_t* cell_start, const uint32_t* counts, uint32_t* rec_key, uint2* rec_im, uint32_t cap,
	int cell_tiles, int cgx, int ncells, uint32_t* pool_cursor, uint32_t* slow_list, hipStream_t stream);
struct SlabSortArgs {
	const uint2* cell_ranges; int ncells;
	const uint2* cell_work;
	uint32_t grid;
	const uint32_t* rec_key; const uint2* rec_im;
	uint2* ent_f;
	uint32_t cap;
	const uint32_t* bounds;
	uint32_t* bounds_out;
	uint32_t* bounds_out2;
	uint32_t* slow_list;
	uint32_t* d_counts;
	Mailbox* box;
};
int launch_slab_sort(const SlabSortArgs& a, hipStream_t stream);
int launch_cell_sample(const SlabSortArgs& a, uint32_t* bounds, hipStream_t stream);
int launch_bounds_from_sorted(const uint64_t* keys, const uint2* cell_ranges, int ncells, const uint32_t* d_total, uint32_t cap, uint32_t* bounds_out, hipStream_t stream);

int launch_duplicate_cells(int P, const uint4* dupinfo, const uint32_t* offsets, uint64_t* keys, uint32_t* vals,
	uint32_t cap, int cell_tiles, int cgx, uint2* cell_ranges, int ncells, uint32_t* pool_cursor, int mask_shift, hipStream_t stream);

struct RenderV2FwdArgs {
	const uint2* cell_ranges; const uint32_t* cell_list; const Splat* splats;
	const uint64_t* cell_keys; int mask_shift;
	const uint2* cell_entries;
	int W, H, gx, gy, cell_tiles, cgx;
	int ppl;
	bool has_color, has_flow, has_sem;
	const float* bg;
	const float* bg_image;
	uint32_t* pool; uint32_t* pool_cursor; uint32_t* tile_last_chunk; uint32_t* tile_consumed; uint32_t* tile_scanned; uint32_t* tile_batches;
	float* final_T; uint32_t* n_contrib;
	float* out_color; float* out_depth; float* out_flow; float* out_semantic;
	int order_mode;
	const uint32_t* fwd_order;
	const float* fwd_view; const float* fwd_sig;
	const uint32_t* overflow_flag;
	bool publish;
	uint8_t* published;
};
int launch_render_fwd_v2(const RenderV2FwdArgs& a, hipStream_t stream);

struct RenderV2BwdArgs {
	const Splat* splats; const uint32_t* pool; const uint32_t* tile_last_chunk; const uint32_t* tile_consumed;
	int W, H, gx, gy, ppl;
	const float* bg; const float* final_T; const uint32_t* n_contrib;
	const float* bg_image; float* dL_dbg_image;
	const float* dL_dpix; const float* dL_dpix_depth; const float* dL_dpix_flow; const float* dL_dpix_sem; const float* dL_dpix_opacity;
	bool do_color, do_flow, do_sem, do_depth, do_opacity;
	bool absgrad;
	float* gacc;
	const uint32_t* tile_order;
	uint32_t* tl_start; uint32_t* tl_end;
	const float* sem_src; float* sem_dst; int sem_stride;
};
int launch_render_bwd_v2(const RenderV2BwdArgs& a, hipStream_t stream);

struct RenderV2SemFwdArgs {
	const Splat* splats; const uint32_t* pool; const uint32_t* tile_last_chunk; const uint32_t* tile_consumed; const uint32_t* n_contrib;
	int W, H, gx, gy, ppl;
	const float* semantic; int D_S, c0, nch;
	float* out_semantic;
};
int launch_render_sem_fwd_v2(const RenderV2SemFwdArgs& a, hipStream_t stream);
int launch_tile_order(int ntiles, const uint32_t* tile_consumed, uint32_t* order, hipStream_t stream, uint32_t* order_copy = nullptr, const float* view = nullptr);

constexpr size_t MAX_STAGING_LDS = 156 * 1024;
inline int pick_block(int row_floats, size_t* lds) {
	int B = 256;
	while (B > 64 && (size_t)B * row_floats * sizeof(float) > 48 * 1024) B >>= 1;
	*lds = (size_t)B * row_floats * sizeof(float);
	return B;
}
int launch_deform_shs_fwd(const adgs_deform_params& p, const adgs_func_eval& fs, float* shs_out, hipStream_t stream);
int launch_deform_shs_bwd(const adgs_deform_params& p, const adgs_func_eval& fs, const float* dL_dshs, const adgs_deform_grads& grads, hipStream_t stream);
int launch_lin_param_grad(int count, int D, const float* g, int gstride, float* out, const adgs_func_eval& f, hipStream_t stream);
int launch_lin_param_grad2(int count_a, const float* g_a, float* out_a, int count_b, const float* g_b, float* out_b, int D, int gstride,
	const adgs_func_eval& f, hipStream_t stream, const AdamSlot* adam_a = nullptr, const AdamSlot* adam_b = nullptr, float beta1 = 0.f, float beta2 = 0.f,
	float eps = 0.f);
void adam_bias_terms(float lr, int step, float beta1, float beta2, float* step_size, float* inv_bc2_sqrt);
int launch_sh0(int N, const ShSource& s, float* out, hipStream_t stream, const FramePrologue* prologue = nullptr, int ostride = 3);
inline bool has_lin_host(const adgs_func_eval& f) { return (f.n_terms[0] + f.n_terms[1] + f.n_terms[2]) > 0 && f.n_params > 0; }

int knn_run(int P, const float* points, float* meanDists, char* workspace, hipStream_t stream);
size_t knn_workspace_bytes(int P);

}
```

### ad-gs_amd/csrc/preprocess_bwd.hip

```cpp
#include "common.h"
#include "kernels.h"
#include "geom.h"
#include "func_eval.h"
#include <cstdlib>

#ifndef ADGS_PREB_STAGE_U4
#define ADGS_PREB_STAGE_U4 12
#endif
namespace adgs {
namespace {

struct M3 { float v[3][3]; };
__device__ __forceinline__ M3 m3mul(const M3& a, const M3& b) {
	M3 r;
#pragma unroll
	for (int c = 0; c < 3; c++)
#pragma unroll
		for (int rr = 0; rr < 3; rr++)
			r.v[c][rr] = a.v[0][rr] * b.v[c][0] + a.v[1][rr] * b.v[c][1] + a.v[2][rr] * b.v[c][2];
	return r;
}
__device__ __forceinline__ M3 m3t(const M3& a) {
	M3 r;
#pragma unroll
	for (int c = 0; c < 3; c++)
#pragma unroll
		for (int rr = 0; rr < 3; rr++) r.v[c][rr] = a.v[rr][c];
	return r;
}

constexpr int BW_THREADS = 256;
constexpr int SH_ROW_FULL = 48, SH_ROW_FULL_LDS = 49, SH_ROW_REST = 45;

struct PreBIn { alignas(16) float q[4]; float4 u0, u1, u2, u3, s0, s1; float p[3], s[3], op; int radius; uint8_t clamped; float dd[9]; };
__device__ __forceinline__ PreBIn load_preb_in(const PreprocessBwdArgs& a, const int idx, const bool gate, const bool pub) {
	PreBIn in;
	const size_t i = (size_t)min(idx, a.P - 1);
	const bool rs = a.sh_src.scene_xyz != nullptr && (int)i < a.sh_src.Ns;
	in.radius = gate ? 0 : a.radii[i];
	if (!pub) return in;
	const float* pos = rs ? a.sh_src.scene_xyz : a.means3D;
	in.p[0] = pos[3 * i]; in.p[1] = pos[3 * i + 1]; in.p[2] = pos[3 * i + 2];
	const float* sc = rs ? a.sh_src.scene_scaling : a.scales;
	const float* rt = rs ? a.sh_src.scene_rotation : a.rotations;
	in.s[0] = sc[3 * i]; in.s[1] = sc[3 * i + 1]; in.s[2] = sc[3 * i + 2];
	const float4 r = *reinterpret_cast<const float4*>(rt + 4 * i);
	in.q[0] = r.x; in.q[1] = r.y; in.q[2] = r.z; in.q[3] = r.w;
	in.op = rs ? a.sh_src.scene_opacity[i] : 0.f;
	const float4* ga = reinterpret_cast<const float4*>(a.gacc + i * GACC_STRIDE);
	in.u0 = ld_stream4(ga); in.u1 = ld_stream4(ga + 1); in.u2 = ld_stream4(ga + 2); in.u3 = ld_stream4(ga + 3);
	const float4* sp = reinterpret_cast<const float4*>(a.splats + i);
	in.s0 = ld_stream4(sp); in.s1 = ld_stream4(sp + 1);
	in.clamped = a.clamped[i];
	if (a.ddir) {
#pragma unroll
		for (int k = 0; k < 9; k++) in.dd[k] = ld_stream(a.ddir + (size_t)k * a.P + i);
	}
	return in;
}

template <bool STAGED, bool AA>
__global__ void __launch_bounds__(BW_THREADS) preprocess_bwd_kernel(PreprocessBwdArgs a) {
	extern __shared__ float s_sh[];
	const int tid = threadIdx.x;
	const int base = blockIdx.x * BW_THREADS;
	const int idx = base + tid;
	const bool raw = a.sh_src.scene_dc != nullptr;
	const int nvalid = min(BW_THREADS, a.P - base);
	const bool pf = STAGED && a.gacc != nullptr && a.cov3D == nullptr && a.scales != nullptr && a.rotations != nullptr;
	const bool adam_rest = STAGED && raw && (a.sh_dst.adam.scene_rest.p != nullptr || a.sh_dst.adam.obj_rest.p != nullptr);
	const bool gate = a.gacc != nullptr && a.published != nullptr;
	bool pub = true;
	if (gate) pub = idx < a.P && a.published[idx] != 0;
	PreBIn in;
	const bool have_ddir = STAGED && raw && pf && a.ddir != nullptr && a.D == 3;
	if (STAGED) {
		if (raw && have_ddir) {
			in = load_preb_in(a, idx, gate, pub);
		} else if (raw) {
			stage_rows<true, ADGS_PREB_STAGE_U4>(s_sh, SH_ROW_REST, SH_ROW_REST, base, nvalid, a.sh_src.Ns, a.sh_src.scene_rest, a.sh_src.obj_rest, tid, BW_THREADS,
				[&]() { if (pf) in = load_preb_in(a, idx, gate, pub); });
		} else {
			const float4* src = reinterpret_cast<const float4*>(a.shs + (size_t)base * SH_ROW_FULL);
			constexpr int NQ4 = SH_ROW_FULL / 4;
			const int total4 = nvalid * NQ4;
			float4 v[NQ4];
#pragma unroll
			for (int u = 0; u < NQ4; u++) v[u] = ld_stream4(src + min(tid + u * BW_THREADS, total4 - 1));
			if (pf) in = load_preb_in(a, idx, gate, pub);
#pragma unroll
			for (int u = 0; u < NQ4; u++) {
				const int q = tid + u * BW_THREADS;
				if (q < total4) {
					const int g = q / NQ4, c = (q - g * NQ4) * 4;
					float* d = s_sh + g * SH_ROW_FULL_LDS + c;
					d[0] = v[u].x; d[1] = v[u].y; d[2] = v[u].z; d[3] = v[u].w;
				}
			}
		}
		if (!have_ddir) __syncthreads();
	}
	const bool valid = idx < a.P;
	const bool vis = valid && (gate ? pub : (pf ? in.radius : a.radii[idx]) > 0);
	const bool rs = a.sh_src.scene_xyz != nullptr && idx < a.sh_src.Ns;
	if (valid && !vis) {
		if (a.gacc) {
			a.out_mean2D[3 * (size_t)idx] = 0.f; a.out_mean2D[3 * (size_t)idx + 1] = 0.f; a.out_mean2D[3 * (size_t)idx + 2] = 0.f;
			if (a.out_mean2D_abs) { a.out_mean2D_abs[3 * (size_t)idx] = 0.f; a.out_mean2D_abs[3 * (size_t)idx + 1] = 0.f; a.out_mean2D_abs[3 * (size_t)idx + 2] = 0.f; }
			if (a.out_conic) *reinterpret_cast<float4*>(a.out_conic + 4 * (size_t)idx) = make_float4(0.f, 0.f, 0.f, 0.f);
			if (!rs) a.out_opacity[idx] = 0.f;
			if (a.out_depth) a.out_depth[idx] = 0.f;
			if (a.out_color) { a.out_color[3 * (size_t)idx] = 0.f; a.out_color[3 * (size_t)idx + 1] = 0.f; a.out_color[3 * (size_t)idx + 2] = 0.f; }
			if (a.out_flow && !rs) { a.out_flow[3 * (size_t)idx] = 0.f; a.out_flow[3 * (size_t)idx + 1] = 0.f; a.out_flow[3 * (size_t)idx + 2] = 0.f; }
			if (a.out_sem && a.D_S >= 1) a.out_sem[(size_t)idx * a.D_S] = 0.f;
			if (rs) {
				float* gx = a.sh_dst.scene_xyz + 3 * (size_t)idx; gx[0] = 0.f; gx[1] = 0.f; gx[2] = 0.f;
				float* gs = a.sh_dst.scene_scaling + 3 * (size_t)idx; gs[0] = 0.f; gs[1] = 0.f; gs[2] = 0.f;
				*reinterpret_cast<float4*>(a.sh_dst.scene_rotation + 4 * (size_t)idx) = make_float4(0.f, 0.f, 0.f, 0.f);
				a.sh_dst.scene_opacity[idx] = 0.f;
			} else {
				a.dL_dmean3D[3 * (size_t)idx] = 0.f; a.dL_dmean3D[3 * (size_t)idx + 1] = 0.f; a.dL_dmean3D[3 * (size_t)idx + 2] = 0.f;
			}
			if (a.dL_dcov3D) for (int i = 0; i < 6; i++) a.dL_dcov3D[6 * (size_t)idx + i] = 0.f;
			if (raw) {
				const bool is_obj = idx >= a.sh_src.Ns;
				const size_t m = is_obj ? idx - a.sh_src.Ns : idx;
				float* gdc = (is_obj ? a.sh_dst.obj_dc : a.sh_dst.scene_dc);
				float* gre = (is_obj ? a.sh_dst.obj_rest : a.sh_dst.scene_rest);
				if (gdc) { gdc[3 * m] = 0.f; gdc[3 * m + 1] = 0.f; gdc[3 * m + 2] = 0.f; }
				if (a.sh_dst.rgb_factor) { float* rf = a.sh_dst.rgb_factor + 3 * (size_t)idx; rf[0] = 0.f; rf[1] = 0.f; rf[2] = 0.f; }
				if (STAGED) { if (gre || adam_rest) for (int i = 0; i < SH_ROW_REST; i++) s_sh[tid * SH_ROW_REST + i] = 0.f; }
				else if (gre) for (int i = 0; i < (a.M - 1) * 3; i++) gre[m * (size_t)(a.M - 1) * 3 + i] = 0.f;
			} else if (a.shs) {
				if (STAGED) { for (int i = 0; i < SH_ROW_FULL; i++) s_sh[tid * SH_ROW_FULL_LDS + i] = 0.f; }
				else { float* dsh = a.dL_dsh + (size_t)idx * a.M * 3; for (int i = 0; i < a.M * 3; i++) dsh[i] = 0.f; }
			}
			if (a.scales && !rs) {
				a.dL_dscale[3 * (size_t)idx] = 0.f; a.dL_dscale[3 * (size_t)idx + 1] = 0.f; a.dL_dscale[3 * (size_t)idx + 2] = 0.f;
				*reinterpret_cast<float4*>(a.dL_drot + 4 * (size_t)idx) = make_float4(0.f, 0.f, 0.f, 0.f);
			}
		}
	}
	if (vis) {
	const float* V = a.view; const float* PJ = a.proj;
	const float* pos = rs ? a.sh_src.scene_xyz : a.means3D;
	const float mx = pf ? in.p[0] : pos[3 * (size_t)idx], my = pf ? in.p[1] : pos[3 * (size_t)idx + 1], mz = pf ? in.p[2] : pos[3 * (size_t)idx + 2];
	SceneAct act;
	if (rs) act = pf ? scene_activations(in.s, in.q, &in.op, (size_t)0)
	                 : scene_activations(a.sh_src.scene_scaling, a.sh_src.scene_rotation, a.sh_src.scene_opacity, (size_t)idx);
	float gflow[3] = { 0.f, 0.f, 0.f };

	float dcon_x, dcon_y, dcon_z, g2x, g2y, gd, gcol[3];
	float aa_g = 0.f, aa_op = 0.f;
	if (a.gacc) {
		const float4* ga = reinterpret_cast<const float4*>(a.gacc + (size_t)idx * GACC_STRIDE);
		const float4 u0 = pf ? in.u0 : ga[0], u1 = pf ? in.u1 : ga[1], u2 = pf ? in.u2 : ga[2], u3 = pf ? in.u3 : ga[3];
		const float4* sp = reinterpret_cast<const float4*>(a.splats + idx);
		const float4 s0 = pf ? in.s0 : sp[0], s1 = pf ? in.s1 : sp[1];
		const float op = s1.y, qa = s0.z, qb = s0.w, qc = s1.x;
		g2x = -op * (qa * u0.y + qb * u0.z) * (float)(0.5 * a.W);
		g2y = -op * (qc * u0.z + qb * u0.y) * (float)(0.5 * a.H);
		dcon_x = -0.5f * op * u0.w; dcon_y = -0.5f * op * u1.x; dcon_z = -0.5f * op * u1.y;
		gcol[0] = u1.z; gcol[1] = u1.w; gcol[2] = u2.x; gd = u2.y;
		st_stream(a.out_mean2D + 3 * (size_t)idx, g2x); st_stream(a.out_mean2D + 3 * (size_t)idx + 1, g2y); st_stream(a.out_mean2D + 3 * (size_t)idx + 2, 0.f);
		if (a.out_mean2D_abs) {
			st_stream(a.out_mean2D_abs + 3 * (size_t)idx, op * (float)(0.5 * a.W) * u3.z); st_stream(a.out_mean2D_abs + 3 * (size_t)idx + 1, op * (float)(0.5 * a.H) * u3.w);
			st_stream(a.out_mean2D_abs + 3 * (size_t)idx + 2, 0.f);
		}
		if (a.out_conic) *reinterpret_cast<float4*>(a.out_conic + 4 * (size_t)idx) = make_float4(dcon_x, dcon_y, 0.f, dcon_z);
		if (AA) { aa_g = u0.x; aa_op = op; }
		else if (rs) st_stream(a.sh_dst.scene_opacity + idx, u0.x * act.op * (1.f - act.op));
		else st_stream(a.out_opacity + idx, u0.x);
		if (a.out_color) { a.out_color[3 * (size_t)idx] = gcol[0]; a.out_color[3 * (size_t)idx + 1] = gcol[1]; a.out_color[3 * (size_t)idx + 2] = gcol[2]; }
		if (a.out_depth) a.out_depth[idx] = gd;
		if (a.out_flow && rs) { gflow[0] = u2.z; gflow[1] = u2.w; gflow[2] = u3.x; }
		else if (a.out_flow) { a.out_flow[3 * (size_t)idx] = u2.z; a.out_flow[3 * (size_t)idx + 1] = u2.w; a.out_flow[3 * (size_t)idx + 2] = u3.x; }
		if (a.out_sem && a.D_S >= 1) a.out_sem[(size_t)idx * a.D_S] = u3.y;
	} else {
		dcon_x = a.dL_dconic[4 * (size_t)idx]; dcon_y = a.dL_dconic[4 * (size_t)idx + 1]; dcon_z = a.dL_dconic[4 * (size_t)idx + 3];
		g2x = a.dL_dmean2D[3 * (size_t)idx]; g2y = a.dL_dmean2D[3 * (size_t)idx + 1];
		gd = a.dL_ddepth[idx];
		gcol[0] = a.dL_dcolor[3 * (size_t)idx]; gcol[1] = a.dL_dcolor[3 * (size_t)idx + 1]; gcol[2] = a.dL_dcolor[3 * (size_t)idx + 2];
		if (AA) { aa_g = a.out_opacity[idx]; aa_op = a.splats[idx].opacity; }
	}
	float c3[6];
	if (a.cov3D) {
#pragma unroll
		for (int i = 0; i < 6; i++) c3[i] = a.cov3D[6 * (size_t)idx + i];
	} else if (rs) {
		cov3d_from_values(act.s[0], act.s[1], act.s[2], a.scale_modifier, act.q[0], act.q[1], act.q[2], act.q[3], c3);
	} else if (pf) {
		cov3d_from_scale_rot(in.s, a.scale_modifier, in.q, c3);
	} else {
		cov3d_from_scale_rot(a.scales + 3 * (size_t)idx, a.scale_modifier, a.rotations + 4 * (size_t)idx, c3);
	}
	float tx = V[0] * mx + V[4] * my + V[8] * mz + V[12];
	float ty = V[1] * mx + V[5] * my + V[9] * mz + V[13];
	const float tz = V[2] * mx + V[6] * my + V[10] * mz + V[14];
	const float h_x = a.focal_x, h_y = a.focal_y;
	const float limx = 1.3f * a.tan_fovx, limy = 1.3f * a.tan_fovy;
	const float txtz = tx / tz, tytz = ty / tz;
	tx = fminf(limx, fmaxf(-limx, txtz)) * tz;
	ty = fminf(limy, fmaxf(-limy, tytz)) * tz;
	const float x_grad_mul = (txtz < -limx || txtz > limx) ? 0.f : 1.f;
	const float y_grad_mul = (tytz < -limy || tytz > limy) ? 0.f : 1.f;
	M3 J = { { { h_x / tz, 0.0f, -(h_x * tx) / (tz * tz) }, { 0.0f, h_y / tz, -(h_y * ty) / (tz * tz) }, { 0.f, 0.f, 0.f } } };
	M3 Wm = { { { V[0], V[4], V[8] }, { V[1], V[5], V[9] }, { V[2], V[6], V[10] } } };
	M3 Vrk = { { { c3[0], c3[1], c3[2] }, { c3[1], c3[3], c3[4] }, { c3[2], c3[4], c3[5] } } };
	M3 T = m3mul(Wm, J);
	M3 cov2D = m3mul(m3mul(m3t(T), m3t(Vrk)), T);
	const float ca = cov2D.v[0][0] + 0.3f, cb = cov2D.v[0][1], cc = cov2D.v[1][1] + 0.3f;
	const float denom = ca * cc - cb * cb;
	float dL_da = 0.f, dL_db = 0.f, dL_dc = 0.f;
	float aa_drho = 0.f;
	if (AA) {
		const float rho = (cov2D.v[0][0] * cov2D.v[1][1] - cb * cb) / denom;
		const float k = sqrtf(fmaxf(rho, 2.5e-5f));
		const float op_in = rs ? act.op : aa_op / k;
		aa_drho = rho > 2.5e-5f ? aa_g * op_in / (2.f * k) : 0.f;
		if (rs) st_stream(a.sh_dst.scene_opacity + idx, aa_g * k * act.op * (1.f - act.op));
		else if (a.gacc) st_stream(a.out_opacity + idx, aa_g * k);
		else a.out_opacity[idx] = aa_g * k;
	}
	const float denom2inv = 1.0f / ((denom * denom) + 0.0000001f);
	float dcov[6];
	if (denom2inv != 0) {
		dL_da = denom2inv * (-cc * cc * dcon_x + 2 * cb * cc * dcon_y + (denom - ca * cc) * dcon_z);
		dL_dc = denom2inv * (-ca * ca * dcon_z + 2 * ca * cb * dcon_y + (denom - ca * cc) * dcon_x);
		dL_db = denom2inv * 2 * (cb * cc * dcon_x - (denom + 2 * cb * cb) * dcon_y + ca * cb * dcon_z);
		if (AA) {
			const float q = aa_drho * 0.3f / (denom * denom);
			dL_da += q * (cov2D.v[1][1] * cc + cb * cb);
			dL_dc += q * (cov2D.v[0][0] * ca + cb * cb);
			dL_db += q * (-2.f * cb * (ca + cov2D.v[1][1]));
		}
		dcov[0] = (T.v[0][0] * T.v[0][0] * dL_da + T.v[0][0] * T.v[1][0] * dL_db + T.v[1][0] * T.v[1][0] * dL_dc);
		dcov[3] = (T.v[0][1] * T.v[0][1] * dL_da + T.v[0][1] * T.v[1][1] * dL_db + T.v[1][1] * T.v[1][1] * dL_dc);
		dcov[5] = (T.v[0][2] * T.v[0][2] * dL_da + T.v[0][2] * T.v[1][2] * dL_db + T.v[1][2] * T.v[1][2] * dL_dc);
		dcov[1] = 2 * T.v[0][0] * T.v[0][1] * dL_da + (T.v[0][0] * T.v[1][1] + T.v[0][1] * T.v[1][0]) * dL_db + 2 * T.v[1][0] * T.v[1][1] * dL_dc;
		dcov[2] = 2 * T.v[0][0] * T.v[0][2] * dL_da + (T.v[0][0] * T.v[1][2] + T.v[0][2] * T.v[1][0]) * dL_db + 2 * T.v[1][0] * T.v[1][2] * dL_dc;
		dcov[4] = 2 * T.v[0][2] * T.v[0][1] * dL_da + (T.v[0][1] * T.v[1][2] + T.v[0][2] * T.v[1][1]) * dL_db + 2 * T.v[1][1] * T.v[1][2] * dL_dc;
	} else {
#pragma unroll
		for (int i = 0; i < 6; i++) dcov[i] = 0.f;
	}
	if (a.dL_dcov3D) {
#pragma unroll
		for (int i = 0; i < 6; i++) a.dL_dcov3D[6 * (size_t)idx + i] = dcov[i];
	}

	const float tv0 = T.v[0][0] * Vrk.v[0][0] + T.v[0][1] * Vrk.v[0][1] + T.v[0][2] * Vrk.v[0][2];
	const float tv1 = T.v[0][0] * Vrk.v[1][0] + T.v[0][1] * Vrk.v[1][1] + T.v[0][2] * Vrk.v[1][2];
	const float tv2 = T.v[0][0] * Vrk.v[2][0] + T.v[0][1] * Vrk.v[2][1] + T.v[0][2] * Vrk.v[2][2];
	const float uv0 = T.v[1][0] * Vrk.v[0][0] + T.v[1][1] * Vrk.v[0][1] + T.v[1][2] * Vrk.v[0][2];
	const float uv1 = T.v[1][0] * Vrk.v[1][0] + T.v[1][1] * Vrk.v[1][1] + T.v[1][2] * Vrk.v[1][2];
	const float uv2 = T.v[1][0] * Vrk.v[2][0] + T.v[1][1] * Vrk.v[2][1] + T.v[1][2] * Vrk.v[2][2];
	const float dL_dT00 = 2 * tv0 * dL_da + uv0 * dL_db;
	const float dL_dT01 = 2 * tv1 * dL_da + uv1 * dL_db;
// ... 13 lines not shown
	float gmy = V[4] * dL_dtx + V[5] * dL_dty + V[6] * dL_dtz;
	float gmz = V[8] * dL_dtx + V[9] * dL_dty + V[10] * dL_dtz;

	{
		const float hw = PJ[3] * mx + PJ[7] * my + PJ[11] * mz + PJ[15];
		const float m_w = 1.0f / (hw + 0.0000001f);
		const float mul1 = (PJ[0] * mx + PJ[4] * my + PJ[8] * mz + PJ[12]) * m_w * m_w;
		const float mul2 = (PJ[1] * mx + PJ[5] * my + PJ[9] * mz + PJ[13]) * m_w * m_w;
		gmx += (PJ[0] * m_w - PJ[3] * mul1) * g2x + (PJ[1] * m_w - PJ[3] * mul2) * g2y;
		gmy += (PJ[4] * m_w - PJ[7] * mul1) * g2x + (PJ[5] * m_w - PJ[7] * mul2) * g2y;
		gmz += (PJ[8] * m_w - PJ[11] * mul1) * g2x + (PJ[9] * m_w - PJ[11] * mul2) * g2y;
	}
	{
		const float mul3 = V[2] * mx + V[6] * my + V[10] * mz + V[14];
		const float demon = a.inv_depth ? (-1.0f / (mul3 * mul3 + 0.0000001f)) : 1.0f;
		gmx += (V[2] - V[3] * mul3) * gd * demon;
		gmy += (V[6] - V[7] * mul3) * gd * demon;
		gmz += (V[10] - V[11] * mul3) * gd * demon;
	}
	if (a.shs || a.sh_src.scene_dc) {
		const float ox = mx - a.campos[0], oy = my - a.campos[1], oz = mz - a.campos[2];
		const float len = sqrtf(ox * ox + oy * oy + oz * oz);
		const float x = ox / len, y = oy / len, z = oz / len;
		const float* sh; float* dsh; float* dsh0;
		bool want_rows = true;
		if (raw) {
			const bool is_obj = idx >= a.sh_src.Ns;
			const size_t m = is_obj ? idx - a.sh_src.Ns : idx;
			float* gdc = is_obj ? a.sh_dst.obj_dc : a.sh_dst.scene_dc;
			float* gre = is_obj ? a.sh_dst.obj_rest : a.sh_dst.scene_rest;
			dsh0 = gdc ? gdc + 3 * m : nullptr;
			want_rows = gre != nullptr || adam_rest;
			if (STAGED) { dsh = s_sh + tid * SH_ROW_REST - 3; sh = dsh; }
			else {
				sh = (is_obj ? a.sh_src.obj_rest : a.sh_src.scene_rest) + m * (size_t)(a.M - 1) * 3 - 3;
				dsh = gre + m * (size_t)(a.M - 1) * 3 - 3;
			}
		} else if (STAGED) {
			dsh = s_sh + tid * SH_ROW_FULL_LDS; sh = dsh; dsh0 = dsh;
		} else {
			sh = a.shs + (size_t)idx * a.M * 3;
			dsh = a.dL_dsh + (size_t)idx * a.M * 3;
			dsh0 = dsh;
		}
		const uint8_t cl = pf ? in.clamped : a.clamped[idx];
		float g[3];
#pragma unroll
		for (int c = 0; c < 3; c++) g[c] = ((cl >> c) & 1) ? 0.f : gcol[c];
		float dx3[3] = { 0.f, 0.f, 0.f }, dy3[3] = { 0.f, 0.f, 0.f }, dz3[3] = { 0.f, 0.f, 0.f };
		const float C0 = 0.28209479177387814f, C1 = 0.4886025119029199f;
		const float C2[5] = { 1.0925484305920792f, -1.0925484305920792f, 0.31539156525252005f, -1.0925484305920792f, 0.5462742152960396f };
		const float C3[7] = { -0.5900435899266435f, 2.890611442640554f, -0.4570457994644658f, 0.3731763325901154f,
			-0.4570457994644658f, 1.445305721320277f, -0.5900435899266435f };
		const int deg = a.D;
		float xx = 0.f, yy = 0.f, zz = 0.f, xy = 0.f, yz = 0.f, xz = 0.f;
		if (have_ddir) {
#pragma unroll
			for (int c = 0; c < 3; c++) { dx3[c] = in.dd[3 * c]; dy3[c] = in.dd[3 * c + 1]; dz3[c] = in.dd[3 * c + 2]; }
		} else if (deg > 0) {
#pragma unroll
			for (int c = 0; c < 3; c++) { dx3[c] = -C1 * sh[3 * 3 + c]; dy3[c] = -C1 * sh[1 * 3 + c]; dz3[c] = C1 * sh[2 * 3 + c]; }
			if (deg > 1) {
				xx = x * x; yy = y * y; zz = z * z; xy = x * y; yz = y * z; xz = x * z;
#pragma unroll
				for (int c = 0; c < 3; c++) {
					dx3[c] += C2[0] * y * sh[4 * 3 + c] + C2[2] * 2.f * -x * sh[6 * 3 + c] + C2[3] * z * sh[7 * 3 + c] + C2[4] * 2.f * x * sh[8 * 3 + c];
					dy3[c] += C2[0] * x * sh[4 * 3 + c] + C2[1] * z * sh[5 * 3 + c] + C2[2] * 2.f * -y * sh[6 * 3 + c] + C2[4] * 2.f * -y * sh[8 * 3 + c];
					dz3[c] += C2[1] * y * sh[5 * 3 + c] + C2[2] * 2.f * 2.f * z * sh[6 * 3 + c] + C2[3] * x * sh[7 * 3 + c];
				}
				if (deg > 2) {
#pragma unroll
					for (int c = 0; c < 3; c++) {
						dx3[c] += (C3[0] * sh[9 * 3 + c] * 3.f * 2.f * xy + C3[1] * sh[10 * 3 + c] * yz + C3[2] * sh[11 * 3 + c] * -2.f * xy +
							C3[3] * sh[12 * 3 + c] * -3.f * 2.f * xz + C3[4] * sh[13 * 3 + c] * (-3.f * xx + 4.f * zz - yy) +
							C3[5] * sh[14 * 3 + c] * 2.f * xz + C3[6] * sh[15 * 3 + c] * 3.f * (xx - yy));
						dy3[c] += (C3[0] * sh[9 * 3 + c] * 3.f * (xx - yy) + C3[1] * sh[10 * 3 + c] * xz + C3[2] * sh[11 * 3 + c] * (-3.f * yy + 4.f * zz - xx) +
							C3[3] * sh[12 * 3 + c] * -3.f * 2.f * yz + C3[4] * sh[13 * 3 + c] * -2.f * xy + C3[5] * sh[14 * 3 + c] * -2.f * yz +
							C3[6] * sh[15 * 3 + c] * -3.f * 2.f * xy);
						dz3[c] += (C3[1] * sh[10 * 3 + c] * xy + C3[2] * sh[11 * 3 + c] * 4.f * 2.f * yz + C3[3] * sh[12 * 3 + c] * 3.f * (2.f * zz - xx - yy) +
							C3[4] * sh[13 * 3 + c] * 4.f * 2.f * xz + C3[5] * sh[14 * 3 + c] * (xx - yy));
					}
				}
			}
		}
		if (dsh0) { dsh0[0] = C0 * g[0]; dsh0[1] = C0 * g[1]; dsh0[2] = C0 * g[2]; }
		if (raw && a.sh_dst.rgb_factor) { float* rf = a.sh_dst.rgb_factor + 3 * (size_t)idx; rf[0] = g[0]; rf[1] = g[1]; rf[2] = g[2]; }
		if (want_rows) {
			float coef[16];
			sh_coef_factors(deg, x, y, z, coef);
#pragma unroll
			for (int k = 1; k < 16; k++)
				if (k < a.M) { dsh[k * 3] = coef[k] * g[0]; dsh[k * 3 + 1] = coef[k] * g[1]; dsh[k * 3 + 2] = coef[k] * g[2]; }
		}
		const float ddx = dx3[0] * g[0] + dx3[1] * g[1] + dx3[2] * g[2];
		const float ddy = dy3[0] * g[0] + dy3[1] * g[1] + dy3[2] * g[2];
		const float ddz = dz3[0] * g[0] + dz3[1] * g[1] + dz3[2] * g[2];
		const float sum2 = ox * ox + oy * oy + oz * oz;
		const float invsum32 = 1.0f / sqrtf(sum2 * sum2 * sum2);
		gmx += ((+sum2 - ox * ox) * ddx - oy * ox * ddy - oz * ox * ddz) * invsum32;
		gmy += (-ox * oy * ddx + (sum2 - oy * oy) * ddy - oz * oy * ddz) * invsum32;
		gmz += (-ox * oz * ddx - oy * oz * ddy + (sum2 - oz * oz) * ddz) * invsum32;
	}
	if (rs) { float* gx = a.sh_dst.scene_xyz + 3 * (size_t)idx; st_stream(gx, gmx + gflow[0]); st_stream(gx + 1, gmy + gflow[1]); st_stream(gx + 2, gmz + gflow[2]); }
	else { st_stream(a.dL_dmean3D + 3 * (size_t)idx, gmx); st_stream(a.dL_dmean3D + 3 * (size_t)idx + 1, gmy); st_stream(a.dL_dmean3D + 3 * (size_t)idx + 2, gmz); }

	if (a.scales) {
		float r, x, y, z;
		if (rs) { r = act.q[0]; x = act.q[1]; y = act.q[2]; z = act.q[3]; }
		else if (pf) { r = in.q[0]; x = in.q[1]; y = in.q[2]; z = in.q[3]; }
		else { const float* q = a.rotations + 4 * (size_t)idx; r = q[0]; x = q[1]; y = q[2]; z = q[3]; }
		const float sc0 = rs ? act.s[0] : (pf ? in.s[0] : a.scales[3 * (size_t)idx]), sc1 = rs ? act.s[1] : (pf ? in.s[1] : a.scales[3 * (size_t)idx + 1]),
			sc2 = rs ? act.s[2] : (pf ? in.s[2] : a.scales[3 * (size_t)idx + 2]);
		M3 R = { { { 1.f - 2.f * (y * y + z * z), 2.f * (x * y - r * z), 2.f * (x * z + r * y) },
		           { 2.f * (x * y + r * z), 1.f - 2.f * (x * x + z * z), 2.f * (y * z - r * x) },
		           { 2.f * (x * z - r * y), 2.f * (y * z + r * x), 1.f - 2.f * (x * x + y * y) } } };
		const float s0 = a.scale_modifier * sc0, s1 = a.scale_modifier * sc1, s2 = a.scale_modifier * sc2;
		M3 S = { { { s0, 0.f, 0.f }, { 0.f, s1, 0.f }, { 0.f, 0.f, s2 } } };
		M3 Mm = m3mul(S, R);
		M3 dSig = { { { dcov[0], 0.5f * dcov[1], 0.5f * dcov[2] }, { 0.5f * dcov[1], dcov[3], 0.5f * dcov[4] }, { 0.5f * dcov[2], 0.5f * dcov[4], dcov[5] } } };
		M3 twoM;
#pragma unroll
		for (int c = 0; c < 3; c++)
#pragma unroll
			for (int rr = 0; rr < 3; rr++) twoM.v[c][rr] = Mm.v[c][rr] * 2.0f;
		M3 dL_dM = m3mul(twoM, dSig);
		M3 Rt = m3t(R);
		M3 dMt = m3t(dL_dM);
		const float ds0 = Rt.v[0][0] * dMt.v[0][0] + Rt.v[0][1] * dMt.v[0][1] + Rt.v[0][2] * dMt.v[0][2];
		const float ds1 = Rt.v[1][0] * dMt.v[1][0] + Rt.v[1][1] * dMt.v[1][1] + Rt.v[1][2] * dMt.v[1][2];
		const float ds2 = Rt.v[2][0] * dMt.v[2][0] + Rt.v[2][1] * dMt.v[2][1] + Rt.v[2][2] * dMt.v[2][2];
		if (rs) { float* gs = a.sh_dst.scene_scaling + 3 * (size_t)idx; st_stream(gs, ds0 * sc0); st_stream(gs + 1, ds1 * sc1); st_stream(gs + 2, ds2 * sc2); }
		else { st_stream(a.dL_dscale + 3 * (size_t)idx + 0, ds0); st_stream(a.dL_dscale + 3 * (size_t)idx + 1, ds1); st_stream(a.dL_dscale + 3 * (size_t)idx + 2, ds2); }
#pragma unroll
		for (int k = 0; k < 3; k++) { dMt.v[0][k] *= s0; dMt.v[1][k] *= s1; dMt.v[2][k] *= s2; }
#define MT(i, j) dMt.v[i][j]
		float4 dq;
		dq.x = 2 * z * (MT(0, 1) - MT(1, 0)) + 2 * y * (MT(2, 0) - MT(0, 2)) + 2 * x * (MT(1, 2) - MT(2, 1));
		dq.y = 2 * y * (MT(1, 0) + MT(0, 1)) + 2 * z * (MT(2, 0) + MT(0, 2)) + 2 * r * (MT(1, 2) - MT(2, 1)) - 4 * x * (MT(2, 2) + MT(1, 1));
		dq.z = 2 * x * (MT(1, 0) + MT(0, 1)) + 2 * r * (MT(2, 0) - MT(0, 2)) + 2 * z * (MT(1, 2) + MT(2, 1)) - 4 * y * (MT(2, 2) + MT(0, 0));
		dq.w = 2 * r * (MT(0, 1) - MT(1, 0)) + 2 * x * (MT(2, 0) + MT(0, 2)) + 2 * y * (MT(1, 2) + MT(2, 1)) - 4 * z * (MT(1, 1) + MT(0, 0));
#undef MT
		if (rs) {
			const float qg = r * dq.x + x * dq.y + y * dq.z + z * dq.w;
			st_stream4(reinterpret_cast<float4*>(a.sh_dst.scene_rotation + 4 * (size_t)idx),
				make_float4((dq.x - r * qg) * act.inv_norm, (dq.y - x * qg) * act.inv_norm, (dq.z - y * qg) * act.inv_norm, (dq.w - z * qg) * act.inv_norm));
		} else st_stream4(reinterpret_cast<float4*>(a.dL_drot + 4 * (size_t)idx), dq);
	}
	}
	if (STAGED) {
		__syncthreads();
		if (raw && adam_rest) {
			adam_rows<4>(s_sh, SH_ROW_REST, SH_ROW_REST, base, nvalid, a.sh_src.Ns, a.sh_dst.adam.scene_rest, a.sh_dst.adam.obj_rest, a.sh_dst.adam.beta1, a.sh_dst.adam.beta2, a.sh_dst.adam.eps,
				tid, BW_THREADS);
		} else if (raw) {
			stage_rows<false>(s_sh, SH_ROW_REST, SH_ROW_REST, base, nvalid, a.sh_src.Ns, a.sh_dst.scene_rest, a.sh_dst.obj_rest, tid, BW_THREADS);
		} else {
			float4* dst = reinterpret_cast<float4*>(a.dL_dsh + (size_t)base * SH_ROW_FULL);
			for (int q = tid; q < nvalid * (SH_ROW_FULL / 4); q += BW_THREADS) {
				const int g = q / (SH_ROW_FULL / 4), c = (q - g * (SH_ROW_FULL / 4)) * 4;
				const float* s = s_sh + g * SH_ROW_FULL_LDS + c;
				st_stream4(dst + q, make_float4(s[0], s[1], s[2], s[3]));
			}
		}
	}
}

}

int launch_preprocess_bwd(const PreprocessBwdArgs& a, hipStream_t stream) {
	if (a.P == 0) return 0;
	const bool raw = a.sh_src.scene_dc != nullptr;
	const bool staged = a.M == 16 && (raw || a.shs) && a.gacc != nullptr && a.sh_staging != 0;
	const unsigned grid = (unsigned)((a.P + BW_THREADS - 1) / BW_THREADS);
	const bool adam_rest = a.sh_dst.adam.scene_rest.p || a.sh_dst.adam.obj_rest.p, adam_sp = a.sh_dst.adam.scene_sp.p || a.sh_dst.adam.obj_sp.p;
	if ((adam_rest || adam_sp) && !raw) { set_error("preprocess backward: the in-backward Adam step needs the raw-SH path"); return -1; }
	if (adam_rest && !staged) {
		set_error("preprocess backward: the in-backward Adam step of the SH `rest` tensors needs 16 SH coefficients and the LDS row staging "
		          "(the frame's forward ran with ADGS_NO_SH_STAGING, or M != 16)");
		return -1;
	}
	if (a.out_mean2D_abs && !a.gacc) { set_error("preprocess backward: the absolute mean2D gradient needs the default (v2) pipeline's accumulator lines"); return -1; }
	if (a.antialias && (!a.out_opacity || (!a.gacc && !a.splats))) { set_error("preprocess backward: the anti-aliased frame's opacity gradient has no destination"); return -1; }
	if (staged) {
		const size_t lds = (size_t)BW_THREADS * (raw ? SH_ROW_REST : SH_ROW_FULL_LDS) * sizeof(float);
		if (a.antialias) hipLaunchKernelGGL((preprocess_bwd_kernel<true, true>), dim3(grid), dim3(BW_THREADS), lds, stream, a);
		else hipLaunchKernelGGL((preprocess_bwd_kernel<true, false>), dim3(grid), dim3(BW_THREADS), lds, stream, a);
	} else {
		if (a.antialias) hipLaunchKernelGGL((preprocess_bwd_kernel<false, true>), dim3(grid), dim3(BW_THREADS), 0, stream, a);
		else hipLaunchKernelGGL((preprocess_bwd_kernel<false, false>), dim3(grid), dim3(BW_THREADS), 0, stream, a);
	}
	ADGS_HIP_CHECK(hipGetLastError());
	if (raw && has_lin_host(a.sh_src.f)) {
		const int No = a.P - a.sh_src.Ns;
		if (launch_lin_param_grad2(a.sh_src.Ns, a.sh_dst.scene_dc, a.sh_dst.scene_sp, No, a.sh_dst.obj_dc, a.sh_dst.obj_sp, 3, 3, a.sh_src.f, stream,
		                           &a.sh_dst.adam.scene_sp, &a.sh_dst.adam.obj_sp, a.sh_dst.adam.beta1, a.sh_dst.adam.beta2, a.sh_dst.adam.eps) != 0) return -1;
	}
	return 0;
}

}
```

### ad-gs_amd/csrc/render_v2.hip

```cpp
#include "common.h"
#include "kernels.h"
#include "blend_instrument.h"
#include <cstdlib>

namespace adgs {
namespace {

constexpr float ALPHA_MAX = 0.99f;
constexpr float ALPHA_MIN = 1.0f / 255.0f;
constexpr float T_STOP = 0.0001f;
constexpr float PIXEL_DONE = 3.0e38f;
constexpr uint32_t NO_CHUNK = 0xFFFFFFFFu;
constexpr int SPLAT_ROW = 5;

#ifndef ADGS_PRECISE_EXP
#define ADGS_EXP2(x) __builtin_amdgcn_exp2f(x)
#else
#define ADGS_EXP2(x) exp2f(x)
#endif
constexpr float LOG2E = 1.4426950408889634f;

__device__ __forceinline__ bool tile_may_contribute(const float4 q0, float C, float tau, uint32_t tx, uint32_t row0, int rows) {
	const float A = q0.z, B = q0.w;
	const float x0 = (float)(tx * TILE_X) - q0.x, x1 = x0 + (float)(TILE_X - 1);
// ... 239 lines not shown
		for (uint64_t todo = pm; todo != 0ull; todo &= todo - 1ull) {
			const uint32_t j = (uint32_t)__builtin_ctzll(todo);
			const float4 q0 = s_splat[j * SPLAT_ROW + 0];
			const float4 q1 = s_splat[j * SPLAT_ROW + 1];
			const EntryGeom eg = entry_geom(q0, q1, q0.x - pxf);
			PROBE_EVAL();
			float alpha[PPL]; uint64_t actm[PPL];
			const uint64_t any_m = ((lean_m >> j) & 1ull) ? eval_entry_fwd<true, PPL>(eg, pyf, alpha, actm) : eval_entry_fwd<false, PPL>(eg, pyf, alpha, actm);
			if (any_m == 0ull) continue;

			PROBE_LIVE(actm, PPL);
			uint32_t position = 0u;
			if (PUBLISH) {
				position = consumed + (uint32_t)__popcll(live) + 1u;
				asm volatile("" : "+v"(position));
			}
			live |= 1ull << j;
			const float4 q2 = s_splat[j * SPLAT_ROW + 2];
			const float4 q3 = s_splat[j * SPLAT_ROW + 3];
#pragma unroll
			for (int k = 0; k < PPL; k++) {
				if (actm[k] == 0ull) continue;
				const float test_T = T[k] * (1.f - alpha[k]);
				const uint64_t stopm = actm[k] & __builtin_amdgcn_ballot_w64(test_T < T_STOP);
				const bool stop = __builtin_amdgcn_inverse_ballot_w64(stopm);
				const bool up = __builtin_amdgcn_inverse_ballot_w64(actm[k] & ~stopm);
				pyf[k] = stop ? PIXEL_DONE : pyf[k];
				const float w = up ? alpha[k] * T[k] : 0.f;
				C0[k] = fmaf(q1.z, w, C0[k]); C1[k] = fmaf(q1.w, w, C1[k]); C2[k] = fmaf(q2.x, w, C2[k]);
				F0[k] = fmaf(q2.z, w, F0[k]); F1[k] = fmaf(q2.w, w, F1[k]); F2[k] = fmaf(q3.x, w, F2[k]);
				Dp[k] = fmaf(q2.y, w, Dp[k]); S0[k] = fmaf(q3.y, w, S0[k]);
				T[k] = up ? test_T : T[k];
				if (PUBLISH) last_contrib[k] = up ? position : last_contrib[k];
			}
		}
		PT(t_b1); PT_ACC(3, t_b0, t_b1);
		const uint32_t nlive = (uint32_t)__popcll(live);
		if (PUBLISH) {
			if ((live >> lane) & 1ull) s_pub[pub_n + (uint32_t)__popcll(live & lt_mask)] = myid;
			pub_n += nlive;
		}
		consumed += nlive;
		if (PUBLISH && pub_n >= (uint32_t)WAVE) flush_chunk(WAVE);
	}
	if (PUBLISH && pub_n > 0) flush_chunk(pub_n);

	if (PUBLISH && lane == 0) { a.tile_last_chunk[tile] = prev_chunk; a.tile_consumed[tile] = consumed; a.tile_scanned[tile] = min(pos, range.y) - range.x; a.tile_batches[tile] = entries_in; }
	TL_STORE(lane, a.tile_scanned, a.tile_batches, tile);
	PROBE_FLUSH(0, lane);
	{ PT(t_wave1); PT_ACC(4, t_wave0, t_wave1); PT_ADD(5, 1ull); PT_FLUSH(0, 10, lane); }
	const size_t HW = (size_t)a.H * a.W;
#pragma unroll
	for (int k = 0; k < PPL; k++) {
		if (inside[k]) {
			const size_t pix_id = (size_t)a.W * (py0 + 4 * k) + px;
			a.final_T[pix_id] = (float)(1.0 - (double)T[k]);
			if (PUBLISH) a.n_contrib[pix_id] = last_contrib[k];
			if (a.has_color) {
				const float b0 = a.bg[0] + (a.bg_image ? a.bg_image[0 * HW + pix_id] : 0.f), b1 = a.bg[1] + (a.bg_image ? a.bg_image[1 * HW + pix_id] : 0.f),
					b2 = a.bg[2] + (a.bg_image ? a.bg_image[2 * HW + pix_id] : 0.f);
				st_stream(a.out_color + 0 * HW + pix_id, C0[k] + T[k] * b0);
				st_stream(a.out_color + 1 * HW + pix_id, C1[k] + T[k] * b1);
				st_stream(a.out_color + 2 * HW + pix_id, C2[k] + T[k] * b2);
			}
			if (a.has_flow) { st_stream(a.out_flow + 0 * HW + pix_id, F0[k]); st_stream(a.out_flow + 1 * HW + pix_id, F1[k]); st_stream(a.out_flow + 2 * HW + pix_id, F2[k]); }
			if (a.has_sem) st_stream(a.out_semantic + pix_id, S0[k]);
			st_stream(a.out_depth + pix_id, Dp[k]);
		}
	}
}

constexpr int RED_ROWS = 14, RED_ROWS_ABS = 16, RED_STRIDE = WAVE;
struct RedAddr { const float4* r[4]; };
template <int ROWS>
__device__ __forceinline__ RedAddr red_addresses(const float* s_red, int lane) {
	const int row = (lane >> 2) < ROWS ? (lane >> 2) : (lane >> 2) - 4;
	RedAddr ra;
#pragma unroll
	for (int i = 0; i < 4; i++) ra.r[i] = reinterpret_cast<const float4*>(s_red + row * RED_STRIDE + (lane & 3) * 16 + 4 * ((i + row) & 3));
	return ra;
}
template <bool ABS>
__device__ __forceinline__ float wave_sum14_lds(float* s_red, const RedAddr& ra, int lane, float x0, float x1, float x2, float x3, float x4, float x5, float x6,
	float x7, float x8, float x9, float x10, float x11, float x12, float x13, float x14, float x15) {
	float* w = s_red + lane;
	w[0 * RED_STRIDE] = x0; w[1 * RED_STRIDE] = x1; w[2 * RED_STRIDE] = x2; w[3 * RED_STRIDE] = x3; w[4 * RED_STRIDE] = x4;
	w[5 * RED_STRIDE] = x5; w[6 * RED_STRIDE] = x6; w[7 * RED_STRIDE] = x7; w[8 * RED_STRIDE] = x8; w[9 * RED_STRIDE] = x9;
	w[10 * RED_STRIDE] = x10; w[11 * RED_STRIDE] = x11; w[12 * RED_STRIDE] = x12; w[13 * RED_STRIDE] = x13;
	if (ABS) { w[14 * RED_STRIDE] = x14; w[15 * RED_STRIDE] = x15; }
	const float4 a = *ra.r[0], b = *ra.r[1], c = *ra.r[2], d = *ra.r[3];
	float v = ((a.x + a.y) + (a.z + a.w)) + ((b.x + b.y) + (b.z + b.w));
	v += ((c.x + c.y) + (c.z + c.w)) + ((d.x + d.y) + (d.z + d.w));
	int x = __float_as_int(v);
	v += __int_as_float(__builtin_amdgcn_update_dpp(0, x, 0xB1, 0xF, 0xF, false)); x = __float_as_int(v);
	v += __int_as_float(__builtin_amdgcn_update_dpp(0, x, 0x4E, 0xF, 0xF, false));
	return v;
}

struct BwdSums { float op, mx, my, ca, cb, cc, c0, c1, c2, d, f0, f1, f2, s, ax, ay; };
struct BwdEntry { float r, g, b, dval, fx, fy, fz, sem, dx, adx, bdx, qb, qc; };
struct BwdPixel { float gC0, gC1, gC2, gD, gF0, gF1, gF2, gS, tfo, tfb; };
template <bool INIT>
__device__ __forceinline__ void bwd_acc(float& s, float a, float b) { s = INIT ? a * b : fmaf(a, b, s); }
template <bool INIT, bool ABS>
__device__ __forceinline__ void bwd_strip(BwdSums& v, const BwdEntry& e, const BwdPixel& p, float al, float G, float dy, float& T, float& Bsum,
	bool do_color, bool do_flow, bool do_sem, bool do_depth, bool do_opacity) {
	const float rinv = __builtin_amdgcn_rcpf(1.f - al);
	T = T * rinv;
	const float dch = al * T;
	float cg = 0.f;
	if (do_color) {
		cg += e.r * p.gC0; cg += e.g * p.gC1; cg += e.b * p.gC2;
		bwd_acc<INIT>(v.c0, dch, p.gC0); bwd_acc<INIT>(v.c1, dch, p.gC1); bwd_acc<INIT>(v.c2, dch, p.gC2);
	} else if (INIT) { v.c0 = v.c1 = v.c2 = 0.f; }
	if (do_flow) {
		cg += e.fx * p.gF0; cg += e.fy * p.gF1; cg += e.fz * p.gF2;
		bwd_acc<INIT>(v.f0, dch, p.gF0); bwd_acc<INIT>(v.f1, dch, p.gF1); bwd_acc<INIT>(v.f2, dch, p.gF2);
	} else if (INIT) { v.f0 = v.f1 = v.f2 = 0.f; }
	if (do_sem) { cg += e.sem * p.gS; bwd_acc<INIT>(v.s, dch, p.gS); } else if (INIT) { v.s = 0.f; }
	if (do_depth) { cg += e.dval * p.gD; bwd_acc<INIT>(v.d, dch, p.gD); } else if (INIT) { v.d = 0.f; }
	float dL_dalpha = cg - Bsum;
	Bsum += al * dL_dalpha;
	if (do_opacity) dL_dalpha += p.tfo * rinv;
	dL_dalpha = dL_dalpha * T - p.tfb * rinv;
	const float L = G * dL_dalpha;
	const float Ly = L * dy;
	bwd_acc<INIT>(v.op, G, dL_dalpha); bwd_acc<INIT>(v.my, L, dy); bwd_acc<INIT>(v.cc, Ly, dy);
	if (ABS) {
		const float aL = fabsf(L);
		bwd_acc<INIT>(v.ax, aL, fabsf(fmaf(e.qb, dy, e.adx))); bwd_acc<INIT>(v.ay, aL, fabsf(fmaf(e.qc, dy, e.bdx)));
	}
}
__device__ __forceinline__ void bwd_finish_moments(BwdSums& v, float dx) {
	v.mx = dx * v.op; v.ca = dx * v.mx; v.cb = dx * v.my;
}

template <bool LEAN, int PPL>
__device__ __forceinline__ uint64_t eval_entry_bwd(const EntryGeom& eg, float pyf0, int contributor, const int (&last_contributor)[PPL],
	float (&alpha)[PPL], float (&G)[PPL], float (&dy)[PPL], uint64_t (&actm)[PPL]) {
	uint64_t any_m = 0ull;
#pragma unroll
	for (int k = 0; k < PPL; k++) {
		float power;
		eval_pixel<LEAN>(eg, pyf0 + (float)(4 * k), dy[k], power, G[k], alpha[k]);
		actm[k] = LEAN ? __builtin_amdgcn_ballot_w64(!(alpha[k] < ALPHA_MIN))
		               : (__builtin_amdgcn_ballot_w64(contributor < last_contributor[k]) & __builtin_amdgcn_ballot_w64(!(power > 0.0f)) &
		                  __builtin_amdgcn_ballot_w64(!(alpha[k] < ALPHA_MIN)));
		any_m |= actm[k];
	}
	return any_m;
}

template <int PPL, bool FULL, bool ABS>
__global__ void __launch_bounds__(WAVE) render_bwd_v2_kernel(RenderV2BwdArgs a) {
	constexpr int ROWS = 4 * PPL;
	const bool do_color = FULL || a.do_color, do_flow = FULL || a.do_flow, do_sem = FULL || a.do_sem, do_depth = FULL || a.do_depth, do_opacity = FULL || a.do_opacity;
	constexpr int BROW = PPL == 4 ? SPLAT_ROW : 4;
	__shared__ float4 s_splat[WAVE * BROW];
	constexpr int RROWS = ABS ? RED_ROWS_ABS : RED_ROWS;
	__shared__ __attribute__((aligned(16))) float s_red[RROWS * RED_STRIDE];
	const int lane = threadIdx.x;
	const uint32_t tile = a.tile_order ? a.tile_order[blockIdx.x] : blockIdx.x;
	const uint32_t tx = tile % a.gx, ty = tile / a.gx;
	const uint32_t px = tx * TILE_X + (lane & 15);
	const uint32_t py0 = ty * ROWS + (lane >> 4);
	const float pxf = (float)px;
	const size_t HW = (size_t)a.H * a.W;
	bool inside[PPL];
	const float pyf0 = (float)py0;
	float T[PPL], tfo[PPL], tfb[PPL];
	int last_contributor[PPL];
	float Bsum[PPL];
	float gC0[PPL], gC1[PPL], gC2[PPL], gF0[PPL], gF1[PPL], gF2[PPL], gD[PPL], gS[PPL];
	int max_contrib = 0, min_contrib = 0x7fffffff;
	const int slot = lane >> 2;
	const RedAddr red = red_addresses<RROWS>(s_red, lane);
	const bool writer = (lane & 3) == 0 && slot < (ABS ? GACC_STRIDE : GACC_USED);
#pragma unroll
	for (int k = 0; k < PPL; k++) {
		const uint32_t py = py0 + 4 * k;
		inside[k] = px < (uint32_t)a.W && py < (uint32_t)a.H;
		const size_t pix_id = (size_t)a.W * py + px;
		const float T_final = inside[k] ? (float)(1.0 - (double)a.final_T[pix_id]) : 0.f;
		float gO = 0.f;
		T[k] = T_final;
		last_contributor[k] = inside[k] ? (int)a.n_contrib[pix_id] : 0;
		max_contrib = max(max_contrib, last_contributor[k]);
		min_contrib = min(min_contrib, last_contributor[k]);
		Bsum[k] = 0.f;
		gC0[k] = gC1[k] = gC2[k] = gF0[k] = gF1[k] = gF2[k] = gD[k] = gS[k] = 0.f;
		if (inside[k]) {
			if (do_color) { gC0[k] = ld_stream(a.dL_dpix + 0 * HW + pix_id); gC1[k] = ld_stream(a.dL_dpix + 1 * HW + pix_id); gC2[k] = ld_stream(a.dL_dpix + 2 * HW + pix_id); }
			if (do_flow) { gF0[k] = ld_stream(a.dL_dpix_flow + 0 * HW + pix_id); gF1[k] = ld_stream(a.dL_dpix_flow + 1 * HW + pix_id); gF2[k] = ld_stream(a.dL_dpix_flow + 2 * HW + pix_id); }
			if (do_sem) gS[k] = ld_stream(a.dL_dpix_sem + pix_id);
			if (do_depth) gD[k] = ld_stream(a.dL_dpix_depth + pix_id);
			if (do_opacity && a.dL_dpix_opacity) gO = ld_stream(a.dL_dpix_opacity + pix_id);
		}
		float b = 0.f;
		b += a.bg[0] * gC0[k]; b += a.bg[1] * gC1[k]; b += a.bg[2] * gC2[k];
		if (a.bg_image && inside[k]) {
			gO -= a.bg_image[0 * HW + pix_id] * gC0[k] + a.bg_image[1 * HW + pix_id] * gC1[k] + a.bg_image[2 * HW + pix_id] * gC2[k];
			if (a.dL_dbg_image) {
				st_stream(a.dL_dbg_image + 0 * HW + pix_id, T_final * gC0[k]); st_stream(a.dL_dbg_image + 1 * HW + pix_id, T_final * gC1[k]); st_stream(a.dL_dbg_image + 2 * HW + pix_id, T_final * gC2[k]);
			}
		}
		tfo[k] = gO * T_final; tfb[k] = T_final * b;
	}
#pragma unroll
	for (int off = WAVE / 2; off > 0; off >>= 1) {
		max_contrib = max(max_contrib, __shfl_xor(max_contrib, off, WAVE));
		min_contrib = min(min_contrib, __shfl_xor(min_contrib, off, WAVE));
	}
	max_contrib = __builtin_amdgcn_readfirstlane(max_contrib);
	min_contrib = __builtin_amdgcn_readfirstlane(min_contrib);
	uint32_t chunk = a.tile_last_chunk[tile];
	int base = (int)a.tile_consumed[tile];
	TL_DECL; PROBE_DECL;
	PT_DECL(9); PT(t_wave0);
	{
		float pt_probe = gC0[0] + T[0];
		(void)pt_probe;
#ifdef ADGS_PHASE_TIMING
		asm volatile("s_waitcnt vmcnt(0)" : "+v"(pt_probe) :: "memory");
#endif
		PT(t_p1); PT_ACC(8, t_wave0, t_p1);
	}
	uint32_t my_id = 0, link = 0;
	uint32_t nx_id = 0, nx_link = 0;
	float4 nx0, nx1, nx2, nx3;
	nx0 = nx1 = nx2 = nx3 = make_float4(0.f, 0.f, 0.f, 0.f);
	auto request_rows = [&](uint32_t id, int cnt, float4& r0, float4& r1, float4& r2, float4& r3) {
		if (lane < cnt) {
			const float4* src = reinterpret_cast<const float4*>(a.splats + id);
			r0 = src[0]; r1 = src[1]; r2 = src[2]; r3 = src[3];
			if (!FULL && a.sem_src) r3.y = a.sem_src[(size_t)id * a.sem_stride];
		}
	};
	if (chunk != NO_CHUNK) {
		const uint32_t* c = a.pool + (size_t)chunk * CHUNK_WORDS;
		my_id = c[lane]; link = c[CHUNK_PREV + (lane & 1)];
	}
	bool rows_ready = false;
	while (chunk != NO_CHUNK) {
		PT(t_c0);
		__builtin_amdgcn_s_setprio(2);
		const uint32_t prev = (uint32_t)__builtin_amdgcn_readlane((int)link, 0);
		const int n = __builtin_amdgcn_readlane((int)link, 1);
#ifdef ADGS_PHASE_TIMING
		asm volatile("s_waitcnt vmcnt(0) lgkmcnt(0)" ::: "memory");
#endif
		PT(t_c1); PT_ACC(0, t_c0, t_c1); PT_ADD(6, 1ull);
		base -= n;
		const uint32_t cur_id = my_id;
		float4 c0, c1, c2, c3;
		if (rows_ready) { c0 = nx0; c1 = nx1; c2 = nx2; c3 = nx3; }
		else {
			if (prev != NO_CHUNK) { const uint32_t* cn = a.pool + (size_t)prev * CHUNK_WORDS; nx_id = cn[lane]; nx_link = cn[CHUNK_PREV + (lane & 1)]; }
			c0 = c1 = c2 = c3 = make_float4(0.f, 0.f, 0.f, 0.f);
			request_rows(cur_id, n, c0, c1, c2, c3);
		}
		{
			__syncthreads();
			bool my_lean = false;
			if (lane < n) {
				s_splat[lane * BROW + 0] = c0; s_splat[lane * BROW + 1] = c1; s_splat[lane * BROW + 2] = c2; s_splat[lane * BROW + 3] = c3;
				my_lean = c3.w != 0.f;
			}
			uint32_t nn_id = 0, nn_link = 0;
			if (prev != NO_CHUNK) {
				{
					const uint32_t pprev = (uint32_t)__builtin_amdgcn_readlane((int)nx_link, 0);
					request_rows(nx_id, __builtin_amdgcn_readlane((int)nx_link, 1), nx0, nx1, nx2, nx3);
					if (pprev != NO_CHUNK) { const uint32_t* cp = a.pool + (size_t)pprev * CHUNK_WORDS; nn_id = cp[lane]; nn_link = cp[CHUNK_PREV + (lane & 1)]; }
					rows_ready = true;
				}
			}
			my_id = nx_id; link = nx_link; nx_id = nn_id; nx_link = nn_link;
			const int n_before = min_contrib - base;
			const uint64_t lean_m = __builtin_amdgcn_ballot_w64(my_lean) & (n_before >= WAVE ? ~0ull : n_before <= 0 ? 0ull : ((1ull << n_before) - 1ull));
			__syncthreads();
			__builtin_amdgcn_s_setprio(0);
			PT(t_g1); PT_ACC(1, t_c1, t_g1);
			const int j_first = min(n - 1, max_contrib - base - 1);
			for (int j = j_first; j >= 0; j--) {
				const int contributor = base + j;
				PT_ADD(7, 1ull);
				const float4 q0 = s_splat[j * BROW + 0], q1 = s_splat[j * BROW + 1];
				const float dx = q0.x - pxf;
				const EntryGeom eg = entry_geom(q0, q1, dx);
				const uint32_t gid = (uint32_t)__builtin_amdgcn_readlane((int)cur_id, j);
				PROBE_EVAL();
				float alpha[PPL], G[PPL], dy[PPL]; uint64_t actm[PPL];
				const uint64_t any_m = ((lean_m >> j) & 1ull) ? eval_entry_bwd<true, PPL>(eg, pyf0, contributor, last_contributor, alpha, G, dy, actm)
				                            : eval_entry_bwd<false, PPL>(eg, pyf0, contributor, last_contributor, alpha, G, dy, actm);
				if (any_m == 0ull) continue;
				const float4 q2 = s_splat[j * BROW + 2];
				const float4 q3 = s_splat[j * BROW + 3];
				PROBE_LIVE(actm, PPL);
				BwdSums v;
				const BwdEntry be = { q1.z, q1.w, q2.x, q2.y, q2.z, q2.w, q3.x, q3.y, dx, ABS ? q0.z * dx : 0.f, ABS ? q0.w * dx : 0.f, q0.w, q1.x };
#define ADGS_BWD_PIXEL(k) const BwdPixel bp = { gC0[k], gC1[k], gC2[k], gD[k], gF0[k], gF1[k], gF2[k], gS[k], tfo[k], tfb[k] }
#define ADGS_BWD_INITK(k) { ADGS_BWD_PIXEL(k); const bool act = __builtin_amdgcn_inverse_ballot_w64(actm[k]); \
	bwd_strip<true, ABS>(v, be, bp, act ? alpha[k] : 0.f, act ? G[k] : 0.f, dy[k], T[k], Bsum[k], do_color, do_flow, do_sem, do_depth, do_opacity); }
#define ADGS_BWD_ACCK(k) if (__builtin_amdgcn_inverse_ballot_w64(actm[k])) { ADGS_BWD_PIXEL(k); \
	bwd_strip<false, ABS>(v, be, bp, alpha[k], G[k], dy[k], T[k], Bsum[k], do_color, do_flow, do_sem, do_depth, do_opacity); }
				if (actm[0] != 0ull) { ADGS_BWD_INITK(0) }
				else v.op = v.my = v.cc = v.c0 = v.c1 = v.c2 = v.d = v.f0 = v.f1 = v.f2 = v.s = v.ax = v.ay = 0.f;
#pragma unroll
				for (int k = 1; k < PPL; k++) { ADGS_BWD_ACCK(k) }
				bwd_finish_moments(v, dx);
#undef ADGS_BWD_PIXEL
#undef ADGS_BWD_INITK
#undef ADGS_BWD_ACCK
				PT(t_r0);
				const float out = wave_sum14_lds<ABS>(s_red, red, lane, v.op, v.mx, v.my, v.ca, v.cb, v.cc, v.c0, v.c1, v.c2, v.d, v.f0, v.f1, v.f2, v.s, v.ax, v.ay);
				if (!FULL && a.sem_dst) {
					if (writer && (slot < 6 || slot == GACC_USED - 1)) atomicAdd(slot == GACC_USED - 1 ? a.sem_dst + (size_t)gid * a.sem_stride : a.gacc + (size_t)gid * GACC_STRIDE + slot, out);
				} else if (writer) atomicAdd(a.gacc + (size_t)gid * GACC_STRIDE + slot, out);
				PT(t_r1); PT_ACC(3, t_r0, t_r1);
			}
			PT(t_e1); PT_ACC(2, t_g1, t_e1);
		}
		chunk = prev;
	}
	__builtin_amdgcn_s_setprio(0);
	{ PT(t_wave1); PT_ACC(4, t_wave0, t_wave1); PT_ADD(5, 1ull); PT_FLUSH(16, 9, lane); }
	TL_STORE(lane, a.tl_start, a.tl_end, tile);
	PROBE_FLUSH(8, lane);
}

template <int PPL>
__global__ void __launch_bounds__(WAVE, 8) render_sem_fwd_v2_kernel(RenderV2SemFwdArgs a) {
	constexpr int ROWS = 4 * PPL, NCH = 4;
	__shared__ float4 s_geo[WAVE * 2];
	__shared__ float4 s_sem[WAVE];
	const int lane = threadIdx.x;
	const uint32_t tile = blockIdx.x;
	const uint32_t tx = tile % a.gx, ty = tile / a.gx;
	const uint32_t px = tx * TILE_X + (lane & 15);
	const uint32_t py0 = ty * ROWS + (lane >> 4);
	const float pxf = (float)px, pyf0 = (float)py0;
	const size_t HW = (size_t)a.H * a.W;
	bool inside[PPL]; int last_contributor[PPL]; float S[PPL][NCH];
	int max_contrib = 0;
#pragma unroll
	for (int k = 0; k < PPL; k++) {
		const uint32_t py = py0 + 4 * k;
		inside[k] = px < (uint32_t)a.W && py < (uint32_t)a.H;
		last_contributor[k] = inside[k] ? (int)a.n_contrib[(size_t)a.W * py + px] : 0;
		max_contrib = max(max_contrib, last_contributor[k]);
#pragma unroll
		for (int i = 0; i < NCH; i++) S[k][i] = 0.f;
	}
#pragma unroll
	for (int off = WAVE / 2; off > 0; off >>= 1) max_contrib = max(max_contrib, __shfl_xor(max_contrib, off, WAVE));
	uint32_t chunk = a.tile_last_chunk[tile];
	int base = (int)a.tile_consumed[tile];
	while (chunk != NO_CHUNK) {
		const uint32_t* c = a.pool + (size_t)chunk * CHUNK_WORDS;
		const uint32_t prev = c[CHUNK_PREV];
		const int n = (int)c[CHUNK_COUNT];
		base -= n;
		if (base < max_contrib) {
			__syncthreads();
			if (lane < n) {
				const uint32_t id = c[lane];
				const float4* src = reinterpret_cast<const float4*>(a.splats + id);
				s_geo[lane * 2 + 0] = src[0];
				s_geo[lane * 2 + 1] = src[1];
				const float* sv = a.semantic + (size_t)id * a.D_S + a.c0;
				float4 q = make_float4(sv[0], 0.f, 0.f, 0.f);
				if (a.nch > 1) q.y = sv[1];
				if (a.nch > 2) q.z = sv[2];
				if (a.nch > 3) q.w = sv[3];
				s_sem[lane] = q;
			}
			__syncthreads();
			for (int j = n - 1; j >= 0; j--) {
				const int contributor = base + j;
				if (contributor >= max_contrib) continue;
				const float4 q0 = s_geo[j * 2 + 0], q1 = s_geo[j * 2 + 1];
				const EntryGeom eg = entry_geom(q0, q1, q0.x - pxf);
				const float4 sv = s_sem[j];
#pragma unroll
				for (int k = 0; k < PPL; k++) {
					float dy, power, G, alpha;
					eval_pixel<false>(eg, pyf0 + (float)(4 * k), dy, power, G, alpha);
					const bool act = contributor < last_contributor[k] && !(power > 0.0f) && !(alpha < ALPHA_MIN);
					const float al = act ? alpha : 0.f;
					S[k][0] = fmaf(al, sv.x - S[k][0], S[k][0]); S[k][1] = fmaf(al, sv.y - S[k][1], S[k][1]);
					S[k][2] = fmaf(al, sv.z - S[k][2], S[k][2]); S[k][3] = fmaf(al, sv.w - S[k][3], S[k][3]);
				}
			}
		}
		chunk = prev;
	}
#pragma unroll
	for (int k = 0; k < PPL; k++) {
		if (!inside[k]) continue;
		const size_t pix_id = (size_t)a.W * (py0 + 4 * k) + px;
#pragma unroll
		for (int i = 0; i < NCH; i++) if (i < a.nch) a.out_semantic[(size_t)(a.c0 + i) * HW + pix_id] = S[k][i];
	}
}

__global__ void __launch_bounds__(256) reset_tiles_kernel(uint32_t T, uint32_t* last_chunk, uint32_t* consumed, uint32_t* cursor) {
	const uint32_t i = blockIdx.x * blockDim.x + threadIdx.x;
	if (i < T) { last_chunk[i] = NO_CHUNK; consumed[i] = 0; }
	if (i == 0) *cursor = 0;
}

}

int launch_render_fwd_v2(const RenderV2FwdArgs& a, hipStream_t stream) {
	const uint32_t T = (uint32_t)a.gx * a.gy;
	if (!a.publish) {
		if (a.ppl == 1) hipLaunchKernelGGL((render_fwd_v2_kernel<1, false>), dim3(T), dim3(WAVE), 0, stream, a);
		else if (a.ppl == 2) hipLaunchKernelGGL((render_fwd_v2_kernel<2, false>), dim3(T), dim3(WAVE), 0, stream, a);
		else hipLaunchKernelGGL((render_fwd_v2_kernel<4, false>), dim3(T), dim3(WAVE), 0, stream, a);
	} else if (a.ppl == 1) hipLaunchKernelGGL((render_fwd_v2_kernel<1, true>), dim3(T), dim3(WAVE), 0, stream, a);
	else if (a.ppl == 2) hipLaunchKernelGGL((render_fwd_v2_kernel<2, true>), dim3(T), dim3(WAVE), 0, stream, a);
	else hipLaunchKernelGGL((render_fwd_v2_kernel<4, true>), dim3(T), dim3(WAVE), 0, stream, a);
	ADGS_HIP_CHECK(hipGetLastError());
	return 0;
}
namespace {
constexpr int TO_THREADS = 256;
__global__ void __launch_bounds__(TO_THREADS) tile_order_kernel(int T, int K, const uint32_t* __restrict__ consumed, uint32_t* __restrict__ order, uint32_t* __restrict__ order_copy,
	const float* __restrict__ view) {
	__shared__ __attribute__((aligned(16))) uint32_t s_key[TO_THREADS];
	const int w = blockIdx.x, tid = threadIdx.x;
	if (w == 0 && order_copy && view && tid < 16) reinterpret_cast<float*>(order_copy + T)[tid] = view[tid];
	const int n = (T - w + K - 1) / K;
	const int t = w + tid * K;
	const uint32_t mine = tid < n ? (min(consumed[t], 0xffffffu) << 8) | (uint32_t)(TO_THREADS - 1 - tid) : 0u;
	s_key[tid] = mine;
	__syncthreads();
	if (tid >= n) return;
	uint32_t rank = 0;
#pragma unroll 4
	for (int j = 0; j < TO_THREADS / 4; j++) {
		const uint4 o = reinterpret_cast<const uint4*>(s_key)[j];
		rank += (o.x > mine ? 1u : 0u) + (o.y > mine ? 1u : 0u) + (o.z > mine ? 1u : 0u) + (o.w > mine ? 1u : 0u);
	}
	const uint32_t at = rank * (uint32_t)K + (uint32_t)w;
	order[at] = (uint32_t)t;
	if (order_copy) order_copy[at] = (uint32_t)t;
}
}
int launch_tile_order(int ntiles, const uint32_t* tile_consumed, uint32_t* order, hipStream_t stream, uint32_t* order_copy, const float* view) {
	if (ntiles <= 0) return 0;
	const int K = (ntiles + TO_THREADS - 1) / TO_THREADS;
	hipLaunchKernelGGL(tile_order_kernel, dim3(K), dim3(TO_THREADS), 0, stream, ntiles, K, tile_consumed, order, order_copy, view);
	ADGS_HIP_CHECK(hipGetLastError());
	return 0;
}

int launch_render_sem_fwd_v2(const RenderV2SemFwdArgs& a, hipStream_t stream) {
	const uint32_t T = (uint32_t)a.gx * a.gy;
	if (a.ppl == 1) hipLaunchKernelGGL(render_sem_fwd_v2_kernel<1>, dim3(T), dim3(WAVE), 0, stream, a);
	else if (a.ppl == 2) hipLaunchKernelGGL(render_sem_fwd_v2_kernel<2>, dim3(T), dim3(WAVE), 0, stream, a);
	else hipLaunchKernelGGL(render_sem_fwd_v2_kernel<4>, dim3(T), dim3(WAVE), 0, stream, a);
	ADGS_HIP_CHECK(hipGetLastError());
	return 0;
}

namespace {
template <bool ABS>
void launch_render_bwd_v2_t(const RenderV2BwdArgs& a, uint32_t T, bool full, hipStream_t stream) {
	if (a.ppl == 1) {
		if (full) hipLaunchKernelGGL((render_bwd_v2_kernel<1, true, ABS>), dim3(T), dim3(WAVE), 0, stream, a);
		else hipLaunchKernelGGL((render_bwd_v2_kernel<1, false, ABS>), dim3(T), dim3(WAVE), 0, stream, a);
	} else if (a.ppl == 2) {
		if (full) hipLaunchKernelGGL((render_bwd_v2_kernel<2, true, ABS>), dim3(T), dim3(WAVE), 0, stream, a);
		else hipLaunchKernelGGL((render_bwd_v2_kernel<2, false, ABS>), dim3(T), dim3(WAVE), 0, stream, a);
	} else {
		if (full) hipLaunchKernelGGL((render_bwd_v2_kernel<4, true, ABS>), dim3(T), dim3(WAVE), 0, stream, a);
		else hipLaunchKernelGGL((render_bwd_v2_kernel<4, false, ABS>), dim3(T), dim3(WAVE), 0, stream, a);
	}
}
}
int launch_render_bwd_v2(const RenderV2BwdArgs& a, hipStream_t stream) {
	const uint32_t T = (uint32_t)a.gx * a.gy;
	const bool full = a.do_color && a.do_flow && a.do_sem && a.do_depth && a.do_opacity && a.dL_dpix_opacity != nullptr && !a.sem_src && !a.sem_dst;
	if (a.absgrad && (a.sem_src || a.sem_dst)) { set_error("blend backward: absolute gradient sums cannot be formed by the extra semantic channel replays"); return -1; }
	if (a.absgrad) launch_render_bwd_v2_t<true>(a, T, full, stream);
	else launch_render_bwd_v2_t<false>(a, T, full, stream);
	ADGS_HIP_CHECK(hipGetLastError());
	return 0;
}

}
```

Baseline: 1098 frames/s.

## Prefill zero gradients for unpublished Gaussians inside the render backward grid

Adds a fill plan that zeroes per-Gaussian gradient outputs for sparse groups, meaning groups where fewer than half of the Gaussians were published. These zero-fill workgroups are appended to the render-backward launch grid, so the fill overlaps with the tail of tile rendering. Preprocess-backward then writes only the visible rows for sparse groups, and the linear parameter gradient gets a row-masked variant. The intent is to remove dense zero-writing from the later kernels and hide it behind render-backward. The cost is more complex grid indexing, a large FillPlan passed by value as a kernel argument, and correctness that depends on the fill and the preprocess paths agreeing on which groups are sparse.

After: 1132 frames/s (median of 6 runs). +3.1%, better.

```diff
diff --git a/ad-gs_amd/csrc/api.hip b/ad-gs_amd/csrc/api.hip
--- a/ad-gs_amd/csrc/api.hip
+++ b/ad-gs_amd/csrc/api.hip
@@ -282,17 +282,17 @@
 	if (hipGetDevice(&dev) != hipSuccess || dev < 0 || dev >= MAX_DEV) return nullptr;
 	return &hints[dev];
 }
-struct FrameCfg { int v2; int cell_tiles; int ppl; int tile_order = 1; int sh_staging = 1; int timeline = 0; int order_ready = 0; int backwards = 0; int antialiasing = 0; int published = 0; };
+struct FrameCfg { int v2; int cell_tiles; int ppl; int tile_order = 1; int sh_staging = 1; int timeline = 0; int order_ready = 0; int backwards = 0; int antialiasing = 0; int published = 0; int prefill = 0; };
 static uint32_t frame_cfg_word(const FrameCfg& c) {
 	return 0xAD600000u | ((uint32_t)(c.v2 & 1) << 19) | ((uint32_t)(c.tile_order & 1) << 18) | ((uint32_t)(c.sh_staging & 1) << 17) | ((uint32_t)(c.timeline & 1) << 16) |
 	       ((uint32_t)(c.order_ready & 1) << 15) | ((uint32_t)(c.antialiasing & 1) << 14) | ((uint32_t)(c.published & 1) << 13) |
-	       ((uint32_t)(c.ppl & 0x1f) << 8) | (uint32_t)(c.cell_tiles & 0xff);
+	       ((uint32_t)(c.prefill & 1) << 12) | ((uint32_t)(c.ppl & 0x7) << 8) | (uint32_t)(c.cell_tiles & 0xff);
 }
 static bool frame_cfg_from_word(uint32_t w, FrameCfg* c) {
 	if ((w & 0xFFF00000u) != 0xAD600000u) return false;
-	*c = FrameCfg{ (int)((w >> 19) & 1u), (int)(w & 0xffu), (int)((w >> 8) & 0x1fu) };
+	*c = FrameCfg{ (int)((w >> 19) & 1u), (int)(w & 0xffu), (int)((w >> 8) & 0x7u) };
 	c->tile_order = (int)((w >> 18) & 1u); c->sh_staging = (int)((w >> 17) & 1u); c->timeline = (int)((w >> 16) & 1u); c->order_ready = (int)((w >> 15) & 1u);
-	c->antialiasing = (int)((w >> 14) & 1u); c->published = (int)((w >> 13) & 1u);
+	c->antialiasing = (int)((w >> 14) & 1u); c->published = (int)((w >> 13) & 1u); c->prefill = (int)((w >> 12) & 1u) & c->published;
 	return c->cell_tiles >= 1 && (c->ppl == 1 || c->ppl == 2 || c->ppl == 4);
 }
 struct FrameKey {
@@ -483,6 +483,7 @@
 			if (!training) order_tiles = false;
 			fcfg.order_ready = order_tiles ? 1 : 0;
 			fcfg.published = (training && env_int("ADGS_PUBLISHED_MASK", 1) != 0) ? 1 : 0;
+			fcfg.prefill = (fcfg.published && env_int("ADGS_GRAD_PREFILL", 1) != 0) ? 1 : 0;
 			if (training) remember_frame(FrameKey{ ich, gch, width, height, P }, fcfg);
 			frame_word = frame_cfg_word(fcfg);
 		}
@@ -862,28 +863,6 @@
 		ra.gacc = geom.gacc;
 		ra.tile_order = nullptr;
 		ra.tl_start = cfg.timeline ? img.tile_scanned : nullptr; ra.tl_end = img.tile_batches;
-		{
-			StageTimer t(ST_RENDER_BWD, stream);
-			if (wtiles >= 2048 && cfg.tile_order) {
-				if (!cfg.order_ready && launch_tile_order((int)wtiles, img.tile_consumed, img.tile_order, stream) != 0) return -1;
-				ra.tile_order = img.tile_order;
-			}
-			if (note_backward(fkey) != 0) ADGS_HIP_CHECK(hipMemsetAsync(geom.gacc, 0, (size_t)P * GACC_STRIDE * sizeof(float), stream));
-			ra.sem_src = nullptr; ra.sem_dst = nullptr; ra.sem_stride = 0;
-			if (binning_buffer && launch_render_bwd_v2(ra, stream) != 0) return -1;
-			if (binning_buffer && ra.do_sem && D_S > 1) {
-				ADGS_HIP_CHECK(hipMemsetAsync(dL_dsemantic, 0, (size_t)P * D_S * sizeof(float), stream));
-				RenderV2BwdArgs rc = ra;
-				rc.do_color = rc.do_flow = rc.do_depth = rc.do_opacity = false; rc.do_sem = true; rc.absgrad = false;
-				rc.dL_dpix = nullptr; rc.dL_dpix_depth = nullptr; rc.dL_dpix_flow = nullptr; rc.dL_dpix_opacity = nullptr;
-				rc.bg_image = nullptr; rc.dL_dbg_image = nullptr; rc.sem_stride = D_S;
-				for (int c = 1; c < D_S; c++) {
-					rc.dL_dpix_sem = dL_dpix_semantic + (size_t)c * npix; rc.sem_src = semantic + c; rc.sem_dst = dL_dsemantic + c;
-					if (launch_render_bwd_v2(rc, stream) != 0) return -1;
-				}
-			}
-		}
-		ADGS_LAUNCH_CHECK(debug, stream);
 		PreprocessBwdArgs pa;
 		pa.P = P; pa.D = D; pa.M = M;
 		pa.means3D = means3D; pa.radii = radii; pa.shs = shs; pa.clamped = geom.clamped;
@@ -904,6 +883,31 @@
 		pa.ddir = geom.ddir;
 		pa.antialias = cfg.antialiasing;
 		pa.published = cfg.published ? geom.published : nullptr;
+		pa.prefill = (cfg.prefill && cfg.published) ? 1 : 0;
+		const FillPlan fill = preprocess_bwd_fill_plan(pa);
+		{
+			StageTimer t(ST_RENDER_BWD, stream);
+			if (wtiles >= 2048 && cfg.tile_order) {
+				if (!cfg.order_ready && launch_tile_order((int)wtiles, img.tile_consumed, img.tile_order, stream) != 0) return -1;
+				ra.tile_order = img.tile_order;
+			}
+			if (note_backward(fkey) != 0) ADGS_HIP_CHECK(hipMemsetAsync(geom.gacc, 0, (size_t)P * GACC_STRIDE * sizeof(float), stream));
+			ra.sem_src = nullptr; ra.sem_dst = nullptr; ra.sem_stride = 0;
+			if (binning_buffer && launch_render_bwd_v2(ra, stream, pa.prefill ? &fill : nullptr) != 0) return -1;
+			if (!binning_buffer && pa.prefill && launch_grad_prefill(fill, stream) != 0) return -1;
+			if (binning_buffer && ra.do_sem && D_S > 1) {
+				ADGS_HIP_CHECK(hipMemsetAsync(dL_dsemantic, 0, (size_t)P * D_S * sizeof(float), stream));
+				RenderV2BwdArgs rc = ra;
+				rc.do_color = rc.do_flow = rc.do_depth = rc.do_opacity = false; rc.do_sem = true; rc.absgrad = false;
+				rc.dL_dpix = nullptr; rc.dL_dpix_depth = nullptr; rc.dL_dpix_flow = nullptr; rc.dL_dpix_opacity = nullptr;
+				rc.bg_image = nullptr; rc.dL_dbg_image = nullptr; rc.sem_stride = D_S;
+				for (int c = 1; c < D_S; c++) {
+					rc.dL_dpix_sem = dL_dpix_semantic + (size_t)c * npix; rc.sem_src = semantic + c; rc.sem_dst = dL_dsemantic + c;
+					if (launch_render_bwd_v2(rc, stream) != 0) return -1;
+				}
+			}
+		}
+		ADGS_LAUNCH_CHECK(debug, stream);
 		{ StageTimer t(ST_PREPROCESS_BWD, stream); if (launch_preprocess_bwd(pa, stream) != 0) return -1; }
 		ADGS_LAUNCH_CHECK(debug, stream);
 		return 0;
@@ -946,7 +950,7 @@
 	memset(&pa.sh_src, 0, sizeof(pa.sh_src)); pa.sh_dst = ShGradDst{};
 	pa.gacc = nullptr; pa.splats = nullptr; pa.W = width; pa.H = height; pa.out_mean2D = nullptr; pa.out_conic = nullptr; pa.out_opacity = nullptr; pa.out_color = nullptr; pa.out_depth = nullptr;
 	pa.out_flow = nullptr; pa.out_sem = nullptr; pa.D_S = D_S; pa.out_mean2D_abs = nullptr;
-	pa.sh_staging = cfg.sh_staging; pa.ddir = nullptr; pa.published = nullptr;
+	pa.sh_staging = cfg.sh_staging; pa.ddir = nullptr; pa.published = nullptr; pa.prefill = 0;
 	pa.antialias = cfg.antialiasing;
 	if (cfg.antialiasing) { pa.out_opacity = dL_dopacity; pa.splats = geom.splats; }
 	{ StageTimer t(ST_PREPROCESS_BWD, stream); if (launch_preprocess_bwd(pa, stream) != 0) return -1; }
diff --git a/ad-gs_amd/csrc/deform_sh.hip b/ad-gs_amd/csrc/deform_sh.hip
--- a/ad-gs_amd/csrc/deform_sh.hip
+++ b/ad-gs_amd/csrc/deform_sh.hip
@@ -165,6 +165,86 @@
 	}
 }
 
+struct ParamGradRowsArgs {
+	int Ns, P, D, gstride;
+	const float *g_scene, *g_obj;
+	float *out_scene, *out_obj;
+	const uint8_t* published;
+	adgs_func_eval f;
+};
+__global__ void __launch_bounds__(PREFILL_GROUP) lin_param_grad_rows_kernel(ParamGradRowsArgs a) {
+	extern __shared__ float s_w[];
+	const int tid = threadIdx.x, base = blockIdx.x * PREFILL_GROUP;
+	const bool pub = base + tid < a.P && a.published[base + tid] != 0;
+	const int npub = __syncthreads_count(pub);
+	const bool sparse = prefill_group_sparse(npub, min(PREFILL_GROUP, a.P - base));
+	if (sparse && npub == 0) return;
+	const int np = a.f.n_params, L = a.D * np;
+	for (int k = tid; k < np; k += PREFILL_GROUP) s_w[k] = 0.f;
+	__syncthreads();
+	const int total = a.f.n_terms[0] + a.f.n_terms[1] + a.f.n_terms[2];
+	for (int i = tid; i < total; i += PREFILL_GROUP) s_w[a.f.index[i]] = a.f.weight[i];
+	__syncthreads();
+	if (sparse) {
+		__shared__ int s_list[PREFILL_GROUP];
+		__shared__ int s_wave[PREFILL_GROUP / WAVE];
+		const int lane = tid & (WAVE - 1), w = tid / WAVE;
+		const uint64_t m = __builtin_amdgcn_ballot_w64(pub);
+		if (lane == 0) s_wave[w] = __popcll(m);
+		__syncthreads();
+		int off = 0;
+		for (int i = 0; i < w; i++) off += s_wave[i];
+		if (pub) s_list[off + __popcll(m & ((1ull << lane) - 1ull))] = base + tid;
+		__syncthreads();
+		for (int e = tid; e < npub * L; e += PREFILL_GROUP) {
+			const int j = e / L, c = e - j * L, d = c / np, gi = s_list[j];
+			const bool ob = gi >= a.Ns;
+			float* const out = ob ? a.out_obj : a.out_scene;
+			if (!out) continue;
+			const size_t r = ob ? gi - a.Ns : gi;
+			st_stream(out + r * (size_t)L + c, __fmul_rn(s_w[c - d * np], (ob ? a.g_obj : a.g_scene)[r * (size_t)a.gstride + d]));
+		}
+		return;
+	}
+	const int end = min(base + PREFILL_GROUP, a.P);
+#pragma unroll
+	for (int side = 0; side < 2; side++) {
+		const int first = side ? a.Ns : 0, lo = max(base, first), hi = side ? end : min(end, a.Ns);
+		float* const out = side ? a.out_obj : a.out_scene;
+		if (lo >= hi || !out) continue;
+		float* const dst = out + (size_t)(lo - first) * L;
+		const float* const g = (side ? a.g_obj : a.g_scene) + (size_t)(lo - first) * a.gstride;
+		const int n = (hi - lo) * L;
+		auto elem = [&](int e) {
+			const uint32_t row = (uint32_t)e / (uint32_t)np, m = row / (uint32_t)a.D;
+			return __fmul_rn(s_w[(uint32_t)e - row * (uint32_t)np], g[(size_t)m * a.gstride + (row - m * (uint32_t)a.D)]);
+		};
+		const int head = min(n, (int)((16u - ((uint32_t)reinterpret_cast<uintptr_t>(dst) & 15u)) & 15u) >> 2);
+		if (tid < head) dst[tid] = elem(tid);
+		const int n4 = (n - head) >> 2;
+		for (int q = tid; q < n4; q += PREFILL_GROUP) {
+			const int e = head + 4 * q;
+			const uint32_t row0 = (uint32_t)e / (uint32_t)np;
+			int k = (int)((uint32_t)e - row0 * (uint32_t)np);
+			uint32_t m = row0 / (uint32_t)a.D; int d = (int)(row0 - m * (uint32_t)a.D);
+			float gv = g[(size_t)m * a.gstride + d];
+			float v[4];
+#pragma unroll
+			for (int it = 0; it < 4; it++) {
+				v[it] = __fmul_rn(s_w[k], gv);
+				if (++k == np) {
+					k = 0;
+					if (++d == a.D) { d = 0; m++; }
+					if (e + it + 1 < n) gv = g[(size_t)m * a.gstride + d];
+				}
+			}
+			st_stream4(reinterpret_cast<float4*>(dst + e), make_float4(v[0], v[1], v[2], v[3]));
+		}
+		const int tail0 = head + (n4 << 2);
+		if (tail0 + tid < n) dst[tail0 + tid] = elem(tail0 + tid);
+	}
+}
+
 template <int NV4>
 __global__ void __launch_bounds__(256) sh0_rows_kernel(int N, ShSource s, float* __restrict__ out, FramePrologue pro, int ostride) {
 	__shared__ float s_w[NV4 * 4];
@@ -296,6 +376,17 @@
 	ADGS_HIP_CHECK(hipGetLastError());
 	return 0;
 }
+int launch_lin_param_grad_rows(int Ns, const float* g_scene, float* out_scene, int No, const float* g_obj, float* out_obj, int D, int gstride,
+	const adgs_func_eval& f, const uint8_t* published, hipStream_t stream) {
+	if (f.n_params <= 0) return 0;
+	const bool on_a = out_scene && Ns > 0, on_b = out_obj && No > 0;
+	if (!on_a && !on_b) return 0;
+	if ((on_a && !g_scene) || (on_b && !g_obj) || !published) { set_error("launch_lin_param_grad_rows: NULL gradient buffer or mask"); return -1; }
+	const ParamGradRowsArgs pg = { Ns, Ns + No, D, gstride, g_scene, g_obj, on_a ? out_scene : nullptr, on_b ? out_obj : nullptr, published, f };
+	hipLaunchKernelGGL(lin_param_grad_rows_kernel, dim3((unsigned)((Ns + No + PREFILL_GROUP - 1) / PREFILL_GROUP)), dim3(PREFILL_GROUP), f.n_params * sizeof(float), stream, pg);
+	ADGS_HIP_CHECK(hipGetLastError());
+	return 0;
+}
 int launch_lin_param_grad(int count, int D, const float* g, int gstride, float* out, const adgs_func_eval& f, hipStream_t stream) {
 	if (count <= 0 || f.n_params <= 0) return 0;
 	if (!g || !out) { set_error("launch_lin_param_grad: NULL gradient buffer"); return -1; }
diff --git a/ad-gs_amd/csrc/grad_prefill.h b/ad-gs_amd/csrc/grad_prefill.h
--- /dev/null
+++ b/ad-gs_amd/csrc/grad_prefill.h
@@ -0,0 +1,101 @@
+#pragma once
+#include "common.h"
+#include "stream_access.h"
+
+namespace adgs {
+
+constexpr int PREFILL_GROUP = 256;
+#ifndef ADGS_PREFILL_SPARSE_NUM
+#define ADGS_PREFILL_SPARSE_NUM 1
+#endif
+#ifndef ADGS_PREFILL_SPARSE_DEN
+#define ADGS_PREFILL_SPARSE_DEN 2
+#endif
+constexpr int PREFILL_SPARSE_NUM = ADGS_PREFILL_SPARSE_NUM, PREFILL_SPARSE_DEN = ADGS_PREFILL_SPARSE_DEN;
+__host__ __device__ __forceinline__ bool prefill_group_sparse(int published, int valid) { return published * PREFILL_SPARSE_DEN < valid * PREFILL_SPARSE_NUM; }
+
+#ifndef ADGS_PREFILL_TILES_BEHIND
+#define ADGS_PREFILL_TILES_BEHIND 0u
+#endif
+constexpr uint32_t PREFILL_TILES_BEHIND = ADGS_PREFILL_TILES_BEHIND;
+#ifdef ADGS_PREFILL_AFTER_BLOCKS
+constexpr uint32_t PREFILL_AFTER_BLOCKS = ADGS_PREFILL_AFTER_BLOCKS;
+#endif
+__host__ inline uint32_t prefill_start(uint32_t tiles) {
+#ifdef ADGS_PREFILL_AFTER_BLOCKS
+	return tiles < PREFILL_AFTER_BLOCKS ? tiles : PREFILL_AFTER_BLOCKS;
+#else
+	return tiles > PREFILL_TILES_BEHIND ? tiles - PREFILL_TILES_BEHIND : 0u;
+#endif
+}
+
+struct FillEntry { float* p; int row, stride, first, count; };
+constexpr int PREFILL_MAX_ENTRIES = 26;
+struct FillPlan {
+	const uint8_t* published;
+	int P, n;
+	uint32_t start, groups;
+	FillEntry e[PREFILL_MAX_ENTRIES];
+};
+inline void fill_plan_add(FillPlan& fp, float* p, int row, int stride, int first, int count) {
+	if (!p || row <= 0 || count <= 0 || fp.n >= PREFILL_MAX_ENTRIES) return;
+	fp.e[fp.n++] = FillEntry{ p, row, stride, first, count };
+}
+
+#if defined(__HIPCC__)
+#ifndef ADGS_PREFILL_STREAM
+#define ADGS_PREFILL_STREAM 1
+#endif
+__device__ __forceinline__ void prefill_st(float* p) {
+#if ADGS_PREFILL_STREAM
+	st_stream(p, 0.f);
+#else
+	*p = 0.f;
+#endif
+}
+__device__ __forceinline__ void prefill_st4(float4* p) {
+#if ADGS_PREFILL_STREAM
+	st_stream4(p, make_float4(0.f, 0.f, 0.f, 0.f));
+#else
+	*p = make_float4(0.f, 0.f, 0.f, 0.f);
+#endif
+}
+__device__ __forceinline__ int prefill_wave_count(const uint8_t* __restrict__ published, int base, int P, int lane) {
+	int n = 0;
+#pragma unroll
+	for (int j = 0; j < PREFILL_GROUP / WAVE; j++) {
+		const int i = base + j * WAVE + lane;
+		const bool set = i < P && published[i] != 0;
+		n += __popcll(__builtin_amdgcn_ballot_w64(set));
+	}
+	return n;
+}
+__device__ __forceinline__ void prefill_group(const FillPlan& fp, const uint32_t group, const int lane) {
+	const int base = (int)group * PREFILL_GROUP;
+	if (base >= fp.P) return;
+	const int end = min(base + PREFILL_GROUP, fp.P);
+	if (!prefill_group_sparse(prefill_wave_count(fp.published, base, fp.P, lane), end - base)) return;
+	for (int i = 0; i < fp.n; i++) {
+		float* const p = fp.e[i].p;
+		const int row = fp.e[i].row, stride = fp.e[i].stride, first = fp.e[i].first;
+		const int lo = max(base, first), hi = min(end, first + fp.e[i].count);
+		if (lo >= hi) continue;
+		if (stride != row) {
+			for (int g = lo + lane; g < hi; g += WAVE)
+				for (int c = 0; c < row; c++) prefill_st(p + (size_t)(g - first) * stride + c);
+			continue;
+		}
+		float* const d = p + (size_t)(lo - first) * row;
+		const int n = (hi - lo) * row;
+		const int head = min(n, (int)((16u - ((uint32_t)reinterpret_cast<uintptr_t>(d) & 15u)) & 15u) >> 2);
+		if (lane < head) prefill_st(d + lane);
+		const int n4 = (n - head) >> 2;
+		float4* const d4 = reinterpret_cast<float4*>(d + head);
+		for (int q = lane; q < n4; q += WAVE) prefill_st4(d4 + q);
+		const int tail0 = head + (n4 << 2);
+		if (tail0 + lane < n) prefill_st(d + tail0 + lane);
+	}
+}
+#endif
+
+}
diff --git a/ad-gs_amd/csrc/kernels.h b/ad-gs_amd/csrc/kernels.h
--- a/ad-gs_amd/csrc/kernels.h
+++ b/ad-gs_amd/csrc/kernels.h
@@ -1,6 +1,7 @@
 #pragma once
 #include "common.h"
 #include "func_eval.h"
+#include "grad_prefill.h"
 
 namespace adgs {
 
@@ -84,8 +85,10 @@
 	const float* ddir;
 	int antialias;
 	const uint8_t* published;
+	int prefill;
 };
 int launch_preprocess_bwd(const PreprocessBwdArgs& a, hipStream_t stream);
+FillPlan preprocess_bwd_fill_plan(const PreprocessBwdArgs& a);
 
 constexpr int CHUNK_WORDS = 2 + WAVE;
 constexpr int CHUNK_PREV = WAVE, CHUNK_COUNT = WAVE + 1;
@@ -176,7 +179,8 @@
 	uint32_t* tl_start; uint32_t* tl_end;
 	const float* sem_src; float* sem_dst; int sem_stride;
 };
-int launch_render_bwd_v2(const RenderV2BwdArgs& a, hipStream_t stream);
+int launch_render_bwd_v2(const RenderV2BwdArgs& a, hipStream_t stream, const FillPlan* fill = nullptr);
+int launch_grad_prefill(const FillPlan& plan, hipStream_t stream);
 
 struct RenderV2SemFwdArgs {
 	const Splat* splats; const uint32_t* pool; const uint32_t* tile_last_chunk; const uint32_t* tile_consumed; const uint32_t* n_contrib;
@@ -200,6 +204,8 @@
 int launch_lin_param_grad2(int count_a, const float* g_a, float* out_a, int count_b, const float* g_b, float* out_b, int D, int gstride,
 	const adgs_func_eval& f, hipStream_t stream, const AdamSlot* adam_a = nullptr, const AdamSlot* adam_b = nullptr, float beta1 = 0.f, float beta2 = 0.f,
 	float eps = 0.f);
+int launch_lin_param_grad_rows(int Ns, const float* g_scene, float* out_scene, int No, const float* g_obj, float* out_obj, int D, int gstride,
+	const adgs_func_eval& f, const uint8_t* published, hipStream_t stream);
 void adam_bias_terms(float lr, int step, float beta1, float beta2, float* step_size, float* inv_bc2_sqrt);
 int launch_sh0(int N, const ShSource& s, float* out, hipStream_t stream, const FramePrologue* prologue = nullptr, int ostride = 3);
 inline bool has_lin_host(const adgs_func_eval& f) { return (f.n_terms[0] + f.n_terms[1] + f.n_terms[2]) > 0 && f.n_params > 0; }
diff --git a/ad-gs_amd/csrc/preprocess_bwd.hip b/ad-gs_amd/csrc/preprocess_bwd.hip
--- a/ad-gs_amd/csrc/preprocess_bwd.hip
+++ b/ad-gs_amd/csrc/preprocess_bwd.hip
@@ -72,6 +72,12 @@
 	const bool gate = a.gacc != nullptr && a.published != nullptr;
 	bool pub = true;
 	if (gate) pub = idx < a.P && a.published[idx] != 0;
+	bool sparse = false;
+	if (gate && a.prefill) {
+		const int npub = __syncthreads_count(pub);
+		sparse = prefill_group_sparse(npub, nvalid);
+		if (sparse && npub == 0 && !adam_rest) return;
+	}
 	PreBIn in;
 	const bool have_ddir = STAGED && raw && pf && a.ddir != nullptr && a.D == 3;
 	if (STAGED) {
@@ -103,7 +109,9 @@
 	const bool valid = idx < a.P;
 	const bool vis = valid && (gate ? pub : (pf ? in.radius : a.radii[idx]) > 0);
 	const bool rs = a.sh_src.scene_xyz != nullptr && idx < a.sh_src.Ns;
-	if (valid && !vis) {
+	if (valid && !vis && sparse) {
+		if (STAGED && raw && adam_rest) for (int i = 0; i < SH_ROW_REST; i++) s_sh[tid * SH_ROW_REST + i] = 0.f;
+	} else if (valid && !vis) {
 		if (a.gacc) {
 			a.out_mean2D[3 * (size_t)idx] = 0.f; a.out_mean2D[3 * (size_t)idx + 1] = 0.f; a.out_mean2D[3 * (size_t)idx + 2] = 0.f;
 			if (a.out_mean2D_abs) { a.out_mean2D_abs[3 * (size_t)idx] = 0.f; a.out_mean2D_abs[3 * (size_t)idx + 1] = 0.f; a.out_mean2D_abs[3 * (size_t)idx + 2] = 0.f; }
@@ -423,6 +431,18 @@
 		if (raw && adam_rest) {
 			adam_rows<4>(s_sh, SH_ROW_REST, SH_ROW_REST, base, nvalid, a.sh_src.Ns, a.sh_dst.adam.scene_rest, a.sh_dst.adam.obj_rest, a.sh_dst.adam.beta1, a.sh_dst.adam.beta2, a.sh_dst.adam.eps,
 				tid, BW_THREADS);
+		} else if (sparse) {
+			const int lane = tid & (WAVE - 1), w0 = tid - lane;
+			for (uint64_t m = __builtin_amdgcn_ballot_w64(vis); m != 0ull; m &= m - 1ull) {
+				const int r = w0 + __builtin_ctzll(m), gi = base + r;
+				if (raw) {
+					const bool is_obj = gi >= a.sh_src.Ns;
+					float* const gre = is_obj ? a.sh_dst.obj_rest : a.sh_dst.scene_rest;
+					if (gre && lane < SH_ROW_REST) st_stream(gre + (size_t)(is_obj ? gi - a.sh_src.Ns : gi) * SH_ROW_REST + lane, s_sh[r * SH_ROW_REST + lane]);
+				} else if (lane < SH_ROW_FULL) {
+					st_stream(a.dL_dsh + (size_t)gi * SH_ROW_FULL + lane, s_sh[r * SH_ROW_FULL_LDS + lane]);
+				}
+			}
 		} else if (raw) {
 			stage_rows<false>(s_sh, SH_ROW_REST, SH_ROW_REST, base, nvalid, a.sh_src.Ns, a.sh_dst.scene_rest, a.sh_dst.obj_rest, tid, BW_THREADS);
 		} else {
@@ -436,6 +456,46 @@
 	}
 }
 
+}
+
+FillPlan preprocess_bwd_fill_plan(const PreprocessBwdArgs& a) {
+	FillPlan fp;
+	fp.published = nullptr; fp.P = a.P; fp.n = 0; fp.start = 0u; fp.groups = 0u;
+	if (!a.prefill || !a.gacc || !a.published || a.P <= 0) return fp;
+	fp.published = a.published;
+	const int P = a.P;
+	const bool raw = a.sh_src.scene_dc != nullptr;
+	const int Ns = raw ? max(0, min(a.sh_src.Ns, P)) : 0;
+	const int Nr = a.sh_src.scene_xyz ? max(0, min(a.sh_src.Ns, P)) : 0;
+	auto all = [&](float* p, int row) { fill_plan_add(fp, p, row, row, 0, P); };
+	auto tail = [&](float* p, int row) { if (p) fill_plan_add(fp, p + (size_t)Nr * row, row, row, Nr, P - Nr); };
+	all(a.out_mean2D, 3); all(a.out_mean2D_abs, 3); all(a.out_conic, 4);
+	tail(a.out_opacity, 1);
+	all(a.out_depth, 1); all(a.out_color, 3);
+	tail(a.out_flow, 3);
+	if (a.D_S >= 1) fill_plan_add(fp, a.out_sem, 1, a.D_S, 0, P);
+	if (Nr > 0) {
+		fill_plan_add(fp, a.sh_dst.scene_xyz, 3, 3, 0, Nr); fill_plan_add(fp, a.sh_dst.scene_scaling, 3, 3, 0, Nr);
+		fill_plan_add(fp, a.sh_dst.scene_rotation, 4, 4, 0, Nr); fill_plan_add(fp, a.sh_dst.scene_opacity, 1, 1, 0, Nr);
+	}
+	tail(a.dL_dmean3D, 3);
+	all(a.dL_dcov3D, 6);
+	if (raw) {
+		fill_plan_add(fp, a.sh_dst.scene_dc, 3, 3, 0, Ns); fill_plan_add(fp, a.sh_dst.obj_dc, 3, 3, Ns, P - Ns);
+		all(a.sh_dst.rgb_factor, 3);
+		const bool adam_rest = a.sh_dst.adam.scene_rest.p || a.sh_dst.adam.obj_rest.p;
+		const int rest = (a.M - 1) * 3;
+		if (!adam_rest) { fill_plan_add(fp, a.sh_dst.scene_rest, rest, rest, 0, Ns); fill_plan_add(fp, a.sh_dst.obj_rest, rest, rest, Ns, P - Ns); }
+		const bool adam_sp = a.sh_dst.adam.scene_sp.p || a.sh_dst.adam.obj_sp.p;
+		if (has_lin_host(a.sh_src.f) && !adam_sp) {
+			const int row = 3 * a.sh_src.f.n_params;
+			fill_plan_add(fp, a.sh_dst.scene_sp, row, row, 0, Ns); fill_plan_add(fp, a.sh_dst.obj_sp, row, row, Ns, P - Ns);
+		}
+	} else if (a.shs) {
+		all(a.dL_dsh, a.M * 3);
+	}
+	if (a.scales) { tail(a.dL_dscale, 3); tail(a.dL_drot, 4); }
+	return fp;
 }
 
 int launch_preprocess_bwd(const PreprocessBwdArgs& a, hipStream_t stream) {
@@ -463,6 +523,8 @@
 	ADGS_HIP_CHECK(hipGetLastError());
 	if (raw && has_lin_host(a.sh_src.f)) {
 		const int No = a.P - a.sh_src.Ns;
+		if (a.prefill && a.gacc && a.published && !adam_sp)
+			return launch_lin_param_grad_rows(a.sh_src.Ns, a.sh_dst.scene_dc, a.sh_dst.scene_sp, No, a.sh_dst.obj_dc, a.sh_dst.obj_sp, 3, 3, a.sh_src.f, a.published, stream);
 		if (launch_lin_param_grad2(a.sh_src.Ns, a.sh_dst.scene_dc, a.sh_dst.scene_sp, No, a.sh_dst.obj_dc, a.sh_dst.obj_sp, 3, 3, a.sh_src.f, stream,
 		                           &a.sh_dst.adam.scene_sp, &a.sh_dst.adam.obj_sp, a.sh_dst.adam.beta1, a.sh_dst.adam.beta2, a.sh_dst.adam.eps) != 0) return -1;
 	}
diff --git a/ad-gs_amd/csrc/render_v2.hip b/ad-gs_amd/csrc/render_v2.hip
--- a/ad-gs_amd/csrc/render_v2.hip
+++ b/ad-gs_amd/csrc/render_v2.hip
@@ -415,7 +415,12 @@
 }
 
 template <int PPL, bool FULL, bool ABS>
-__global__ void __launch_bounds__(WAVE) render_bwd_v2_kernel(RenderV2BwdArgs a) {
+__global__ void __launch_bounds__(WAVE) render_bwd_v2_kernel(RenderV2BwdArgs a, FillPlan fp) {
+	uint32_t wg = blockIdx.x;
+	if (wg >= fp.start && fp.groups != 0u) {
+		if (wg - fp.start < fp.groups) { prefill_group(fp, wg - fp.start, (int)threadIdx.x); return; }
+		wg -= fp.groups;
+	}
 	constexpr int ROWS = 4 * PPL;
 	const bool do_color = FULL || a.do_color, do_flow = FULL || a.do_flow, do_sem = FULL || a.do_sem, do_depth = FULL || a.do_depth, do_opacity = FULL || a.do_opacity;
 	constexpr int BROW = PPL == 4 ? SPLAT_ROW : 4;
@@ -423,7 +428,7 @@
 	constexpr int RROWS = ABS ? RED_ROWS_ABS : RED_ROWS;
 	__shared__ __attribute__((aligned(16))) float s_red[RROWS * RED_STRIDE];
 	const int lane = threadIdx.x;
-	const uint32_t tile = a.tile_order ? a.tile_order[blockIdx.x] : blockIdx.x;
+	const uint32_t tile = a.tile_order ? a.tile_order[wg] : wg;
 	const uint32_t tx = tile % a.gx, ty = tile / a.gx;
 	const uint32_t px = tx * TILE_X + (lane & 15);
 	const uint32_t py0 = ty * ROWS + (lane >> 4);
@@ -729,26 +734,44 @@
 }
 
 namespace {
+__global__ void __launch_bounds__(WAVE) grad_prefill_kernel(FillPlan fp) {
+	prefill_group(fp, blockIdx.x, (int)threadIdx.x);
+}
 template <bool ABS>
-void launch_render_bwd_v2_t(const RenderV2BwdArgs& a, uint32_t T, bool full, hipStream_t stream) {
+void launch_render_bwd_v2_t(const RenderV2BwdArgs& a, const FillPlan& fp, uint32_t T, bool full, hipStream_t stream) {
 	if (a.ppl == 1) {
-		if (full) hipLaunchKernelGGL((render_bwd_v2_kernel<1, true, ABS>), dim3(T), dim3(WAVE), 0, stream, a);
-		else hipLaunchKernelGGL((render_bwd_v2_kernel<1, false, ABS>), dim3(T), dim3(WAVE), 0, stream, a);
+		if (full) hipLaunchKernelGGL((render_bwd_v2_kernel<1, true, ABS>), dim3(T), dim3(WAVE), 0, stream, a, fp);
+		else hipLaunchKernelGGL((render_bwd_v2_kernel<1, false, ABS>), dim3(T), dim3(WAVE), 0, stream, a, fp);
 	} else if (a.ppl == 2) {
-		if (full) hipLaunchKernelGGL((render_bwd_v2_kernel<2, true, ABS>), dim3(T), dim3(WAVE), 0, stream, a);
-		else hipLaunchKernelGGL((render_bwd_v2_kernel<2, false, ABS>), dim3(T), dim3(WAVE), 0, stream, a);
+		if (full) hipLaunchKernelGGL((render_bwd_v2_kernel<2, true, ABS>), dim3(T), dim3(WAVE), 0, stream, a, fp);
+		else hipLaunchKernelGGL((render_bwd_v2_kernel<2, false, ABS>), dim3(T), dim3(WAVE), 0, stream, a, fp);
 	} else {
-		if (full) hipLaunchKernelGGL((render_bwd_v2_kernel<4, true, ABS>), dim3(T), dim3(WAVE), 0, stream, a);
-		else hipLaunchKernelGGL((render_bwd_v2_kernel<4, false, ABS>), dim3(T), dim3(WAVE), 0, stream, a);
-	}
-}
-}
-int launch_render_bwd_v2(const RenderV2BwdArgs& a, hipStream_t stream) {
+		if (full) hipLaunchKernelGGL((render_bwd_v2_kernel<4, true, ABS>), dim3(T), dim3(WAVE), 0, stream, a, fp);
+		else hipLaunchKernelGGL((render_bwd_v2_kernel<4, false, ABS>), dim3(T), dim3(WAVE), 0, stream, a, fp);
+	}
+}
+}
+int launch_grad_prefill(const FillPlan& plan, hipStream_t stream) {
+	if (!plan.published || plan.n == 0 || plan.P <= 0) return 0;
+	hipLaunchKernelGGL(grad_prefill_kernel, dim3((unsigned)((plan.P + PREFILL_GROUP - 1) / PREFILL_GROUP)), dim3(WAVE), 0, stream, plan);
+	ADGS_HIP_CHECK(hipGetLastError());
+	return 0;
+}
+int launch_render_bwd_v2(const RenderV2BwdArgs& a, hipStream_t stream, const FillPlan* fill) {
 	const uint32_t T = (uint32_t)a.gx * a.gy;
 	const bool full = a.do_color && a.do_flow && a.do_sem && a.do_depth && a.do_opacity && a.dL_dpix_opacity != nullptr && !a.sem_src && !a.sem_dst;
 	if (a.absgrad && (a.sem_src || a.sem_dst)) { set_error("blend backward: absolute gradient sums cannot be formed by the extra semantic channel replays"); return -1; }
-	if (a.absgrad) launch_render_bwd_v2_t<true>(a, T, full, stream);
-	else launch_render_bwd_v2_t<false>(a, T, full, stream);
+	FillPlan fp;
+	if (fill) fp = *fill; else { fp.published = nullptr; fp.P = 0; fp.n = 0; }
+	fp.start = 0u; fp.groups = 0u;
+	if (fill && fp.published && fp.n > 0 && fp.P > 0) {
+		if (T == 0) return launch_grad_prefill(fp, stream);
+		fp.groups = (uint32_t)((fp.P + PREFILL_GROUP - 1) / PREFILL_GROUP);
+		fp.start = prefill_start(T);
+	}
+	if (T + fp.groups == 0) return 0;
+	if (a.absgrad) launch_render_bwd_v2_t<true>(a, fp, T + fp.groups, full, stream);
+	else launch_render_bwd_v2_t<false>(a, fp, T + fp.groups, full, stream);
 	ADGS_HIP_CHECK(hipGetLastError());
 	return 0;
 }
```
